# jammm/first_raytracer

Measured on AMD Instinct MI355X. Metric: Mrays/sec + RMSE vs CPU ref, CornellBox 1080p 512spp, 1/2/4/8 MI355X, higher is better.
Workload: dtype f32

## Files before the change

first_raytracer_amd/__init__.py:

```python
import ctypes
import os

import numpy as np

HERE = os.path.dirname(os.path.abspath(__file__))
LIB_PATH = os.environ.get("FRT_LIB_PATH") or os.path.join(HERE, "libfrt.so")

FRT_WORLD_BVH, FRT_WORLD_LIST = 0, 1
FRT_MAT_LAMBERTIAN, FRT_MAT_DIFFUSE_LIGHT = 0, 1
FRT_PRIM_SPHERE = 1 << 30
ABI_VERSION = 9
FRT_MAT_LAMBERTIAN, FRT_MAT_DIFFUSE_LIGHT, FRT_MAT_MODIFIED_PHONG, FRT_MAT_METAL, FRT_MAT_DIELECTRIC = 0, 1, 2, 3, 4
FRT_MAT_ROUGH_CONDUCTOR = 5
FRT_DIST_GGX, FRT_DIST_BECKMANN = 0, 1
FRT_TEX_CONSTANT, FRT_TEX_CHECKER, FRT_TEX_IMAGE = 0, 1, 2
FRT_IMAGE_SRGB8, FRT_IMAGE_F32 = 0, 1
FRT_FLAG_NO_LDS_SCENE = 1
FRT_FLAG_WAVES5 = 2
FRT_FLAG_WAVES6 = 4
FRT_FLAG_WAVES4 = 8
FRT_FLAG_BVH2 = 16
FRT_FLAG_NO_OCT = 256
FRT_FLAG_FP64 = 512
FRT_FLAG_FP32 = 1024
FRT_FLAG_ENV_SAMPLING = 2048
FRT_FLAG_ROULETTE = 4096
FRT_FLAG_SOBOL = 8192
FRT_PRECISION_AUTO, FRT_PRECISION_FP32, FRT_PRECISION_FP64 = 0, 1, 2
FRT_GPU_BVH_PLOC = 0
FRT_GPU_BVH_LBVH = 1
FRT_GPU_BVH_SAH = 2
FRT_INTEGRATOR_PATH, FRT_INTEGRATOR_PSSMLT, FRT_INTEGRATOR_AO, FRT_INTEGRATOR_NORMALS = 0, 1, 2, 3
FRT_INTEGRATOR_ALBEDO, FRT_INTEGRATOR_DEPTH, FRT_INTEGRATOR_DENOISE = 4, 5, 6
FRT_INTEGRATOR_ERROR = 8

ERRORS = {0: "ok", -1: "invalid", -2: "hip", -3: "no scene", -4: "unsupported", -5: "io", -6: "no gfx950 device"}


class FrtError(RuntimeError):
    pass


class Material(ctypes.Structure):
    _fields_ = [("type", ctypes.c_int32), ("distribution", ctypes.c_int32),
                ("albedo", ctypes.c_double * 3), ("emit", ctypes.c_double * 3),
                ("specular", ctypes.c_double * 3), ("exponent", ctypes.c_double), ("ior", ctypes.c_double),
                ("alpha", ctypes.c_double), ("eta", ctypes.c_double * 3), ("k", ctypes.c_double * 3),
                ("texture", ctypes.c_int32), ("image", ctypes.c_int32), ("tex_odd", ctypes.c_double * 3),
                ("tex_scale", ctypes.c_double * 2)]

    @classmethod
    def from_spec(cls, m):
        r = cls()
        r.type = MAT_TYPES[m["type"]]
        r.distribution = DISTRIBUTIONS[m.get("distribution", "ggx").lower()]
        for k in ("albedo", "emit", "specular", "eta", "k"):
            getattr(r, k)[:] = [float(x) for x in m.get(k, (0.0, 0.0, 0.0))]
        r.exponent = float(m.get("exponent", 0.0))
        r.ior = float(m.get("ior", 0.0))
        r.alpha = float(m.get("alpha", 0.0))
        tex = m.get("checker")
        if tex is not None:
            r.texture = FRT_TEX_CHECKER
            r.tex_odd[:] = [float(x) for x in tex["odd"]]
            r.tex_scale[:] = [float(x) for x in tex["scale"]]
        if m.get("image") is not None:
            r.texture = FRT_TEX_IMAGE
            r.image = int(m["image"])
        return r


class Image(ctypes.Structure):
    _fields_ = [("nx", ctypes.c_int32), ("ny", ctypes.c_int32), ("format", ctypes.c_int32),
                ("reserved", ctypes.c_int32), ("data", ctypes.c_void_p)]


def image_array(img):
    a = np.asarray(img["data"])
    if a.ndim != 3 or a.shape[2] != 3:
        raise ValueError("image data must be (ny, nx, 3)")
    if a.dtype == np.uint8:
        return np.ascontiguousarray(a), FRT_IMAGE_SRGB8
    return np.ascontiguousarray(a, np.float32), FRT_IMAGE_F32


CORNELL_CAMERA = {"lookfrom": (0.0, 1.0, float(np.float32(3.9))), "lookat": (0.0, 1.0, 0.0), "vup": (0.0, 1.0, 0.0),
                  "vfov": 40.0, "aperture": 0.0, "focus": 10.0}
MAT_TYPES = {"lambertian": 0, "diffuse_light": 1, "modified_phong": 2, "metal": 3, "dielectric": 4,
             "rough_conductor": 5}
DISTRIBUTIONS = {"ggx": 0, "beckmann": 1}
SPHERE_WHERE = {"world": 1, "lights": 2, "both": 3}


class SceneView(ctypes.Structure):
    _fields_ = [
        ("world_kind", ctypes.c_int32),
        ("n_tris", ctypes.c_int32),
        ("tri_v", ctypes.c_void_p), ("tri_n", ctypes.c_void_p), ("tri_material", ctypes.c_void_p),
        ("tri_geometry_normal", ctypes.c_void_p), ("tri_inv_area", ctypes.c_void_p),
        ("n_spheres", ctypes.c_int32), ("sphere", ctypes.c_void_p), ("sphere_material", ctypes.c_void_p),
        ("n_materials", ctypes.c_int32), ("materials", ctypes.c_void_p),
        ("n_nodes", ctypes.c_int32), ("root", ctypes.c_int32),
        ("node_box", ctypes.c_void_p), ("node_child", ctypes.c_void_p),
        ("n_list", ctypes.c_int32), ("list", ctypes.c_void_p),
        ("n_lights", ctypes.c_int32), ("lights", ctypes.c_void_p),
        ("cam_origin", ctypes.c_double * 3), ("cam_lower_left", ctypes.c_double * 3),
        ("cam_horizontal", ctypes.c_double * 3), ("cam_vertical", ctypes.c_double * 3),
        ("cam_u", ctypes.c_double * 3), ("cam_v", ctypes.c_double * 3),
        ("cam_lens_radius", ctypes.c_double),
        ("env_color", ctypes.c_double * 3),
        ("cam_w", ctypes.c_double * 3),
        ("cam_half_height", ctypes.c_double),
        ("tri_uv", ctypes.c_void_p),
        ("n_images", ctypes.c_int32), ("images", ctypes.c_void_p),
    ]


class RenderParams(ctypes.Structure):
    _fields_ = [(n, ctypes.c_int32) for n in ("nx", "ny", "spp")] + [("seed", ctypes.c_uint32)] + [
        (n, ctypes.c_int32) for n in ("max_depth", "integrator", "tile_size", "shard_index", "shard_count",
                                      "samples_per_item", "flags", "mlt_chains", "mlt_bootstrap", "sample_offset")]

    @classmethod
    def make(cls, nx, ny, spp, seed=0, max_depth=33, tile_size=32, shard_index=0, shard_count=1,
             samples_per_item=0, flags=0, integrator=0, sample_offset=0):
        return cls(nx=nx, ny=ny, spp=spp, seed=seed, max_depth=max_depth, integrator=integrator, tile_size=tile_size,
                   shard_index=shard_index, shard_count=shard_count, samples_per_item=samples_per_item, flags=flags,
                   mlt_chains=0, mlt_bootstrap=0, sample_offset=sample_offset)

    @classmethod
    def pssmlt(cls, nx, ny, mutations_per_pixel, chains, seed=0, bootstrap=10000, shard_index=0, shard_count=1,
               flags=0):
        return cls(nx=nx, ny=ny, spp=mutations_per_pixel, seed=seed, max_depth=10, integrator=FRT_INTEGRATOR_PSSMLT,
                   tile_size=32, shard_index=shard_index, shard_count=shard_count, samples_per_item=0, flags=flags,
                   mlt_chains=chains, mlt_bootstrap=bootstrap)


class Stats(ctypes.Structure):
    _fields_ = [(n, ctypes.c_uint64) for n in ("camera_rays", "extension_rays", "shadow_rays", "samples",
                                               "pixels", "work_items")] + [
        ("kernel_ms", ctypes.c_double), ("total_ms", ctypes.c_double)] + [
        (n, ctypes.c_uint32) for n in ("scene_in_lds", "waves_cap", "stack_entries", "bvh_depth")] + [
        ("scene_bytes", ctypes.c_uint64), ("fp64", ctypes.c_uint32), ("reserved", ctypes.c_uint32)]

    @property
    def rays(self):
        return self.camera_rays + self.extension_rays + self.shadow_rays

    def as_dict(self):
        d = {n: getattr(self, n) for n, _ in self._fields_}
        d["rays"] = self.rays
        return d


class TreeCost(ctypes.Structure):
    _fields_ = [("v", ctypes.c_double), ("t", ctypes.c_double), ("j", ctypes.c_double), ("w", ctypes.c_double),
                ("depth", ctypes.c_int32), ("n_nodes", ctypes.c_int32), ("n_rays", ctypes.c_int32),
                ("applies", ctypes.c_int32)]

    def as_dict(self):
        return {k: getattr(self, k) for k, _ in self._fields_}


class PlanQuery(ctypes.Structure):
    _fields_ = [(n, ctypes.c_int32) for n in ("kind", "integrator", "flags", "world_kind", "stack_needed", "has_bvh4",
                                              "depth4", "mats", "has_spec_mats", "env_image", "env_sampling",
                                              "has_f64", "precision")] + [
        ("scene_lds_bytes", ctypes.c_int64), ("scene_lds_bytes_oct", ctypes.c_int64)]


class PlanAnswer(ctypes.Structure):
    _fields_ = [(n, ctypes.c_int32) for n in ("rc", "stack", "waves", "lds_scene", "wide", "f64")] + [
        (n, ctypes.c_int64) for n in ("lds", "scene_lds", "lds_boot")] + [
        ("kernel", ctypes.c_uint64), ("kernel_boot", ctypes.c_uint64)]


class HostSceneInfo(ctypes.Structure):
    _fields_ = [(n, ctypes.c_int32) for n in ("n_tris", "n_spheres", "n_materials", "n_lights", "n_nodes",
                                              "world_kind", "n_list", "bvh_depth")] + [
        ("load_ms", ctypes.c_double), ("build_ms", ctypes.c_double)]


_lib = None

EXPORTS = ("frt_get_abi_version", "frt_create", "frt_destroy", "frt_last_error", "frt_set_precision", "frt_upload_scene",
           "frt_shard_slot_count", "frt_shard_slots", "frt_render", "frt_render_multi", "frt_render_device", "frt_trace_device",
           "frt_mlt_chain_state",
           "frt_scene_create", "frt_scene_new", "frt_scene_add_obj", "frt_scene_add_sphere", "frt_scene_set_camera",
           "frt_scene_set_env", "frt_scene_add_image", "frt_scene_finish", "frt_scene_build_bvh_gpu",
           "frt_scene_build_bvh_sah", "frt_scene_build_bvh_gpu_algo",
           "frt_scene_view_get", "frt_scene_info", "frt_scene_destroy", "frt_write_tessellated_obj",
           "frt_write_pfm", "frt_film_accumulate", "frt_tonemap_u8", "frt_write_image", "frt_selftest_path_host",
           "frt_selftest_mlt_paths_host",
           "frt_set_env_image", "frt_scene_set_env_image", "frt_scene_env_image", "frt_read_hdr",
           "frt_selftest_path_host_env")
EXPORTS_X = ("frtx_selftest_tree_refine", "frtx_selftest_trace_host", "frtx_selftest_chunk_variance",
             "frtx_selftest_plan")


def lib():
    global _lib
    if _lib is not None:
        return _lib
    if not os.path.exists(LIB_PATH):
        raise FrtError(f"{LIB_PATH} is missing: build it with `python -c 'import __graft_entry__ as g; g.build()'`")
    try:
        import torch
    except ImportError:
        pass
    L = ctypes.CDLL(LIB_PATH)
    vp = ctypes.c_void_p
    L.frt_get_abi_version.restype = ctypes.c_int
    if L.frt_get_abi_version() != ABI_VERSION:
        raise FrtError(f"{LIB_PATH}: ABI version {L.frt_get_abi_version()}, binding expects {ABI_VERSION}; rebuild")
    L.frt_create.argtypes = [ctypes.c_int, ctypes.POINTER(vp)]
    L.frt_destroy.argtypes = [vp]
    L.frt_last_error.argtypes = [vp]
    L.frt_last_error.restype = ctypes.c_char_p
    L.frt_set_precision.argtypes = [vp, ctypes.c_int]
    L.frt_upload_scene.argtypes = [vp, ctypes.POINTER(SceneView)]
    L.frt_shard_slot_count.argtypes = [ctypes.POINTER(RenderParams)]
    L.frt_shard_slot_count.restype = ctypes.c_int64
    L.frt_shard_slots.argtypes = [ctypes.POINTER(RenderParams), vp]
    L.frt_render.argtypes = [vp, ctypes.POINTER(RenderParams), vp, ctypes.POINTER(Stats)]
    L.frt_render_device.argtypes = [vp, ctypes.POINTER(RenderParams), vp, vp, ctypes.POINTER(Stats)]
    L.frt_trace_device.argtypes = [vp, vp, ctypes.c_int64, vp, ctypes.c_int, vp, ctypes.POINTER(Stats)]
    L.frt_mlt_chain_state.argtypes = [vp, ctypes.c_uint64, ctypes.c_uint64, vp, vp]
    L.frt_render_multi.argtypes = [ctypes.POINTER(vp), ctypes.c_int, ctypes.POINTER(RenderParams), vp,
                                   ctypes.POINTER(Stats)]
    L.frt_scene_create.argtypes = [ctypes.c_char_p, ctypes.c_char_p, ctypes.c_double, ctypes.POINTER(vp)]
    L.frt_scene_view_get.argtypes = [vp, ctypes.POINTER(SceneView)]
    L.frt_scene_info.argtypes = [vp, ctypes.POINTER(HostSceneInfo)]
    L.frt_scene_destroy.argtypes = [vp]
    L.frt_scene_destroy.restype = None
    dp = ctypes.POINTER(ctypes.c_double)
    L.frt_scene_new.argtypes = [ctypes.POINTER(vp)]
    L.frt_scene_add_obj.argtypes = [vp, ctypes.c_char_p, dp, ctypes.POINTER(Material), ctypes.c_int]
    L.frt_scene_add_sphere.argtypes = [vp, dp, ctypes.c_double, ctypes.POINTER(Material), ctypes.c_int]
    L.frt_scene_set_camera.argtypes = [vp, dp, dp, dp, ctypes.c_double, ctypes.c_double, ctypes.c_double,
                                       ctypes.c_double]
    L.frt_scene_set_env.argtypes = [vp, dp]
    L.frt_scene_add_image.argtypes = [vp, ctypes.POINTER(Image), ctypes.POINTER(ctypes.c_int)]
    L.frt_scene_finish.argtypes = [vp, ctypes.c_int]
    L.frt_scene_build_bvh_gpu.argtypes = [vp, vp, ctypes.POINTER(ctypes.c_double)]
    L.frt_scene_build_bvh_sah.argtypes = [vp]
    L.frt_scene_build_bvh_gpu_algo.argtypes = [vp, vp, ctypes.c_int, ctypes.POINTER(ctypes.c_double)]
    L.frt_write_tessellated_obj.argtypes = [ctypes.c_char_p, ctypes.c_int, ctypes.c_char_p]
    L.frt_write_pfm.argtypes = [ctypes.c_char_p, ctypes.c_int, ctypes.c_int, vp]
    L.frt_film_accumulate.argtypes = [vp, ctypes.c_int64, vp, ctypes.c_int64, ctypes.c_int64]
    L.frt_tonemap_u8.argtypes = [vp, ctypes.c_int, ctypes.c_int, vp]
    L.frt_write_image.argtypes = [ctypes.c_char_p, ctypes.c_int, ctypes.c_int, vp, ctypes.c_int]
    L.frt_selftest_path_host.argtypes = [ctypes.POINTER(SceneView), ctypes.POINTER(RenderParams), vp,
                                         ctypes.c_int, vp, ctypes.POINTER(Stats)]
    L.frt_selftest_mlt_paths_host.argtypes = [ctypes.POINTER(SceneView), ctypes.c_int, ctypes.c_int, ctypes.c_uint32,
                                              ctypes.c_int, vp]
    L.frt_set_env_image.argtypes = [vp, ctypes.POINTER(Image)]
    L.frt_scene_set_env_image.argtypes = [vp, ctypes.c_int]
    L.frt_scene_env_image.argtypes = [vp, ctypes.POINTER(Image)]
    L.frt_read_hdr.argtypes = [ctypes.c_char_p, ctypes.POINTER(ctypes.c_int32), ctypes.POINTER(ctypes.c_int32), vp]
    L.frt_selftest_path_host_env.argtypes = [ctypes.POINTER(SceneView), ctypes.POINTER(RenderParams), vp,
                                             ctypes.c_int, ctypes.POINTER(Image), vp, ctypes.POINTER(Stats)]
    L.frtx_selftest_tree_refine.argtypes = [ctypes.POINTER(SceneView), ctypes.POINTER(TreeCost), vp, vp, ctypes.c_int32]
    L.frtx_selftest_trace_host.argtypes = [ctypes.POINTER(SceneView), vp, ctypes.c_int64, vp]
    L.frtx_selftest_chunk_variance.argtypes = [vp, ctypes.c_int, ctypes.c_int64, ctypes.c_int, ctypes.c_int, vp]
    _lib = L
    return L


def _check(rc, what, ctx=None):
    if rc != 0:
        msg = ""
        if ctx is not None:
            msg = lib().frt_last_error(ctx).decode(errors="replace")
        raise FrtError(f"{what} failed: {ERRORS.get(rc, rc)} {msg}")


class HostScene:

    def __init__(self, kind, obj_path, aspect):
        self.ptr = ctypes.c_void_p()
        _check(lib().frt_scene_create(kind.encode(), obj_path.encode(), float(aspect), ctypes.byref(self.ptr)),
               f"frt_scene_create({kind})")
        self.info = HostSceneInfo()
        lib().frt_scene_info(self.ptr, ctypes.byref(self.info))
        self.env = None

    def set_env(self, rgb):
        self.env = tuple(float(x) for x in rgb)

    def set_env_image(self, index):
        _check(lib().frt_scene_set_env_image(self.ptr, -1 if index is None else int(index)), "frt_scene_set_env_image")

    def env_image(self):
        img = Image()
        rc = lib().frt_scene_env_image(self.ptr, ctypes.byref(img))
        if rc < 0:
            _check(rc, "frt_scene_env_image")
        return img if rc == 1 else None

    @classmethod
    def from_spec(cls, spec, aspect):
        self = cls.__new__(cls)
        self.ptr = ctypes.c_void_p()
        self.env = None
        L = lib()
        _check(L.frt_scene_new(ctypes.byref(self.ptr)), "frt_scene_new")

        def dptr(x):
            a = np.ascontiguousarray(np.asarray(x, np.float64))
            return a, a.ctypes.data_as(ctypes.POINTER(ctypes.c_double))
        for img in spec.get("images", ()):
            a, fmt = image_array(img)
            desc = Image(a.shape[1], a.shape[0], fmt, 0, a.ctypes.data)
            idx = ctypes.c_int(-1)
            _check(L.frt_scene_add_image(self.ptr, ctypes.byref(desc), ctypes.byref(idx)), "frt_scene_add_image")
        for o in spec["objects"]:
            if "obj" in o:
                tw = dptr(o["to_world"]) if o.get("to_world") is not None else (None, None)
                bs = ctypes.byref(Material.from_spec(o["bsdf"])) if o.get("bsdf") is not None else None
                _check(L.frt_scene_add_obj(self.ptr, o["obj"].encode(), tw[1], bs, int(bool(o.get("geo", False)))),
                       f"frt_scene_add_obj({o['obj']})")
            else:
                c = dptr(o["sphere"])
                _check(L.frt_scene_add_sphere(self.ptr, c[1], float(o["radius"]),
                                              ctypes.byref(Material.from_spec(o["material"])),
                                              SPHERE_WHERE[o.get("where", "world")]), "frt_scene_add_sphere")
        cam = spec["camera"]
        f, a, u = dptr(cam["lookfrom"]), dptr(cam["lookat"]), dptr(cam.get("vup", (0, 1, 0)))
        _check(L.frt_scene_set_camera(self.ptr, f[1], a[1], u[1], float(cam["vfov"]), float(aspect),
                                      float(cam.get("aperture", 0.0)), float(cam.get("focus", 10.0))),
               "frt_scene_set_camera")
        if spec.get("env") is not None:
            e = dptr(spec["env"])
            _check(L.frt_scene_set_env(self.ptr, e[1]), "frt_scene_set_env")
        if spec.get("env_image") is not None:
            _check(L.frt_scene_set_env_image(self.ptr, int(spec["env_image"])), "frt_scene_set_env_image")
        _check(L.frt_scene_finish(self.ptr, {"bvh": 0, "list": 1}[spec.get("world", "bvh")]), "frt_scene_finish")
        self.info = HostSceneInfo()
        L.frt_scene_info(self.ptr, ctypes.byref(self.info))
        return self

    def view(self):
        v = SceneView()
        _check(lib().frt_scene_view_get(self.ptr, ctypes.byref(v)), "frt_scene_view_get")
        if self.env is not None:
            v.env_color[:] = self.env
        return v

    def arrays(self):
        v = self.view()

        def arr(ptr, n, dt, w=1):
            if n == 0 or not ptr:
                return np.zeros((0, w) if w > 1 else 0, dt)
            a = np.ctypeslib.as_array(ctypes.cast(ptr, ctypes.POINTER(np.ctypeslib.as_ctypes_type(dt))),
                                      shape=(n * w,)).copy()
            return a.reshape(n, w) if w > 1 else a
        return {
            "tri_v": arr(v.tri_v, v.n_tris, np.float64, 9),
            "tri_material": arr(v.tri_material, v.n_tris, np.int32),
            "node_box": arr(v.node_box, v.n_nodes, np.float64, 6),
            "node_child": arr(v.node_child, v.n_nodes, np.int32, 2),
            "root": v.root,
            "lights": arr(v.lights, v.n_lights, np.int32),
            "list": arr(v.list, v.n_list, np.int32),
        }

    def build_bvh_sah(self):
        _check(lib().frt_scene_build_bvh_sah(self.ptr), "frt_scene_build_bvh_sah")
        lib().frt_scene_info(self.ptr, ctypes.byref(self.info))
        return self.info.build_ms

    def build_bvh_gpu(self, ctx, algo="gsah"):
        ms = ctypes.c_double()
        a = {"ploc": FRT_GPU_BVH_PLOC, "lbvh": FRT_GPU_BVH_LBVH, "gsah": FRT_GPU_BVH_SAH}[algo]
        _check(lib().frt_scene_build_bvh_gpu_algo(self.ptr, ctx.ptr, a, ctypes.byref(ms)),
               "frt_scene_build_bvh_gpu_algo", ctx.ptr)
        lib().frt_scene_info(self.ptr, ctypes.byref(self.info))
        return ms.value

    def __del__(self):
        if getattr(self, "ptr", None):
            try:
                lib().frt_scene_destroy(self.ptr)
            except Exception:
                pass
            self.ptr = None


class Context:

    def __init__(self, device=0, precision=None):
        self.ptr = ctypes.c_void_p()
        _check(lib().frt_create(int(device), ctypes.byref(self.ptr)), f"frt_create(device={device})")
        if precision is not None:
            self.set_precision(precision)

    def set_precision(self, precision):
        if isinstance(precision, str):
            precision = {"auto": FRT_PRECISION_AUTO, "fp32": FRT_PRECISION_FP32, "fp64": FRT_PRECISION_FP64}[precision]
        _check(lib().frt_set_precision(self.ptr, int(precision)), "frt_set_precision", self.ptr)

    def upload(self, scene):
        view = scene.view() if isinstance(scene, HostScene) else scene
        _check(lib().frt_upload_scene(self.ptr, ctypes.byref(view)), "frt_upload_scene", self.ptr)
        img = scene.env_image() if isinstance(scene, HostScene) else None
        if img is not None:
            _check(lib().frt_set_env_image(self.ptr, ctypes.byref(img)), "frt_set_env_image", self.ptr)
            self._env_from_scene = True
        elif isinstance(scene, HostScene) and getattr(self, "_env_from_scene", False):
            _check(lib().frt_set_env_image(self.ptr, None), "frt_set_env_image", self.ptr)
            self._env_from_scene = False

    def set_env_image(self, image):
        self._env_from_scene = False
# ... 39 lines not shown
        u = np.zeros((max(n, 1), 92), np.float32)
        fp = np.zeros((max(n, 1), 2), np.uint32)
        _check(lib().frt_mlt_chain_state(self.ptr, int(first), int(n), u.ctypes.data, fp.ctypes.data),
               "frt_mlt_chain_state", self.ptr)
        return u[:n], fp[:n]

    def trace_device(self, rays_ptr, n, hits_ptr, flags=0, stream_ptr=None):
        st = Stats()
        _check(lib().frt_trace_device(self.ptr, ctypes.c_void_p(rays_ptr), int(n), ctypes.c_void_p(hits_ptr), int(flags),
                                      ctypes.c_void_p(stream_ptr) if stream_ptr else None, ctypes.byref(st)),
               "frt_trace_device", self.ptr)
        return st

    def close(self):
        if getattr(self, "ptr", None):
            lib().frt_destroy(self.ptr)
            self.ptr = None

    def __del__(self):
        try:
            self.close()
        except Exception:
            pass


def render_multi(contexts, params, film=None):
    if film is None:
        film = np.zeros((params.ny, params.nx, 3), np.float32)
    assert film.dtype == np.float32 and film.flags.c_contiguous and film.size == params.nx * params.ny * 3
    arr = (ctypes.c_void_p * len(contexts))(*[c.ptr for c in contexts])
    st = Stats()
    _check(lib().frt_render_multi(arr, len(contexts), ctypes.byref(params), film.ctypes.data, ctypes.byref(st)),
           "frt_render_multi", contexts[0].ptr)
    return film, st


def frame_error(film, V):
    f = np.asarray(film, np.float64)
    v = np.asarray(V, np.float64)
    return float(np.sqrt(v.sum() / v.size) / (f.sum() / f.size))


def combine_variance(a, Va, b, Vb):
    a, b = float(a), float(b)
    va, vb = np.asarray(Va, np.float64), np.asarray(Vb, np.float64)
    return (((a * a) * va + (b * b) * vb) / ((a + b) * (a + b))).astype(np.float32)


def replicate_variance(films):
    assert len(films) == 4
    r = [np.asarray(f, np.float64) for f in films]
    m = (((r[0] + r[1]) + r[2]) + r[3]) * 0.25
    v = ((((r[0] - m) ** 2 + (r[1] - m) ** 2) + (r[2] - m) ** 2) + (r[3] - m) ** 2) / 12.0
    mean = np.array(films[0], np.float32, copy=True)
    for k in range(1, 4):
        mean = film_accumulate(mean, k, films[k], 1)
    return mean, v.astype(np.float32)


def render_until(render, render_error, params, target, max_spp, first_spp=16):
    first_spp, max_spp = int(first_spp), int(max_spp)
    if first_spp < 2 or first_spp & (first_spp - 1):
        raise FrtError("render_until: first_spp must be a power of two >= 2")
    if params.integrator not in (FRT_INTEGRATOR_PATH, FRT_INTEGRATOR_AO):
        raise FrtError("render_until: path and ao renders only (pssmlt has no error estimate, denoise is a filter)")
    if not target > 0:
        raise FrtError("render_until: target must be > 0")
    sobol = bool(params.flags & FRT_FLAG_SOBOL) and params.integrator == FRT_INTEGRATOR_PATH
    reps = 4 if sobol else 1
    if max_spp < reps * first_spp:
        raise FrtError("render_until: max_spp is below the first pass")
    slots = lib().frt_shard_slot_count(ctypes.byref(params))
    if slots < 0:
        raise FrtError("bad render params")
    films, V, total, passes = [None] * reps, None, 0, []
    halve = False
    while True:
        n = first_spp if total == 0 else total
        ms = 0.0
        for k in range(reps):
            p = RenderParams.from_buffer_copy(params)
            p.spp, p.sample_offset, p.seed = n, total, (params.seed + k) & 0xffffffff
            if halve:
                p.samples_per_item = n // 2
            film, st = render(p)
            if not sobol and st.work_items == slots:
                halve = True
                p.samples_per_item = n // 2
                film, st = render(p)
            ms += st.kernel_ms
            if not sobol:
                Vp = render_error(p)
                V = Vp if total == 0 else combine_variance(total, V, n, Vp)
            films[k] = film if total == 0 else film_accumulate(films[k], total, film, n)
        total += n
        if sobol:
            film, V = replicate_variance(films)
        else:
            film = films[0]
        e = frame_error(film, V)
        passes.append((reps * total, e, ms))
        if e <= target:
            return film, V, reps * total, e, True, passes
        if reps * 2 * total > max_spp:
            return film, V, reps * total, e, False, passes


def selftest_chunk_variance(partial, spp, spi):
    partial = np.ascontiguousarray(partial, dtype=np.float32)
    k, n, three = partial.shape
    assert three == 3
    out = np.zeros((n, 3), np.float32)
    _check(lib().frtx_selftest_chunk_variance(partial.ctypes.data, k, n, int(spp), int(spi), out.ctypes.data),
           "frtx_selftest_chunk_variance")
    return out


def shard_slots(params):
    n = lib().frt_shard_slot_count(ctypes.byref(params))
    if n < 0:
        raise FrtError("bad render params")
    out = np.zeros(n, np.int32)
    _check(lib().frt_shard_slots(ctypes.byref(params), out.ctypes.data), "frt_shard_slots")
    return out


def selftest_path_host(scene, params, pixels, env_image=None):
    pixels = np.ascontiguousarray(pixels, dtype=np.int32)
    out = np.zeros((len(pixels), 3), np.float32)
    st = Stats()
    view = scene.view()
    if env_image is None:
        _check(lib().frt_selftest_path_host(ctypes.byref(view), ctypes.byref(params), pixels.ctypes.data, len(pixels),
                                            out.ctypes.data, ctypes.byref(st)), "frt_selftest_path_host")
        return out, st
    a, fmt = image_array({"data": env_image})
    desc = Image(a.shape[1], a.shape[0], fmt, 0, a.ctypes.data)
    _check(lib().frt_selftest_path_host_env(ctypes.byref(view), ctypes.byref(params), pixels.ctypes.data, len(pixels),
                                            ctypes.byref(desc), out.ctypes.data, ctypes.byref(st)),
           "frt_selftest_path_host_env")
    return out, st


def selftest_tree_refine(scene):
    view = scene.view()
    cap = max(1, view.n_tris + view.n_spheres)
    nodes = [np.zeros((cap, 16), np.float32) for _ in range(2)]
    out = (TreeCost * 2)()
    _check(lib().frtx_selftest_tree_refine(ctypes.byref(view), out, nodes[0].ctypes.data, nodes[1].ctypes.data, cap),
           "frtx_selftest_tree_refine")
    return tuple((out[k].as_dict(), nodes[k][:out[k].n_nodes].copy()) for k in range(2))


def selftest_trace_host(scene, rays):
    rays = np.ascontiguousarray(rays, dtype=np.float32).reshape(-1, 8)
    hits = np.zeros((len(rays), 4), np.float32)
    view = scene.view()
    _check(lib().frtx_selftest_trace_host(ctypes.byref(view), rays.ctypes.data, len(rays), hits.ctypes.data),
           "frtx_selftest_trace_host")
    return hits


_handles = None


def kernel_handles():
    global _handles
    if _handles is None:
        import re
        import subprocess
        out = subprocess.run(["nm", "--defined-only", LIB_PATH], capture_output=True, text=True, check=True).stdout
        syms = [l.split() for l in out.splitlines()]
        stub = re.compile(r"(\d+)__device_stub__")
        kernels = {stub.sub(lambda m: str(int(m.group(1)) - 15), f[2]) for f in syms if len(f) == 3 and stub.search(f[2])}
        _handles = {int(f[0], 16): f[2] for f in syms if len(f) == 3 and f[2] in kernels}
    return _handles


def selftest_plan(**query):
    f = lib().frtx_selftest_plan
    f.argtypes = [ctypes.POINTER(PlanQuery), ctypes.POINTER(PlanAnswer)]
    a = PlanAnswer()
    _check(f(ctypes.byref(PlanQuery(**query)), ctypes.byref(a)), "frtx_selftest_plan")
    d = {n: getattr(a, n) for n, _ in a._fields_}
    for k in ("kernel", "kernel_boot"):
        d[k] = kernel_handles().get(d[k]) if d[k] else None
    return d


def selftest_mlt_paths_host(scene, nx, ny, seed, n):
    out = np.zeros((n, 6), np.float32)
    view = scene.view()
    _check(lib().frt_selftest_mlt_paths_host(ctypes.byref(view), nx, ny, seed, n, out.ctypes.data),
           "frt_selftest_mlt_paths_host")
    return out


def read_hdr(path):
    nx, ny = ctypes.c_int32(0), ctypes.c_int32(0)
    _check(lib().frt_read_hdr(os.fsencode(path), ctypes.byref(nx), ctypes.byref(ny), None), f"frt_read_hdr({path})")
    out = np.zeros((ny.value, nx.value, 3), np.float32)
    _check(lib().frt_read_hdr(os.fsencode(path), ctypes.byref(nx), ctypes.byref(ny), out.ctypes.data),
           f"frt_read_hdr({path})")
    return out


def write_pfm(path, film):
    film = np.ascontiguousarray(film, dtype=np.float32)
    ny, nx = film.shape[0], film.shape[1]
    _check(lib().frt_write_pfm(path.encode(), nx, ny, film.ctypes.data), "frt_write_pfm")


def film_accumulate(acc, acc_spp, film, spp):
    acc = np.ascontiguousarray(acc, dtype=np.float32)
    film = np.ascontiguousarray(film, dtype=np.float32)
    _check(lib().frt_film_accumulate(acc.ctypes.data, int(acc_spp), film.ctypes.data, int(spp), film.size),
           "frt_film_accumulate")
    return acc


def tonemap_u8(film):
    film = np.ascontiguousarray(film, dtype=np.float32)
    ny, nx = film.shape[0], film.shape[1]
    out = np.zeros((ny, nx, 3), np.uint8)
    _check(lib().frt_tonemap_u8(film.ctypes.data, nx, ny, out.ctypes.data), "frt_tonemap_u8")
    return out


IMAGE_FORMATS = {"png": 0, "bmp": 1, "jpg": 2}


def write_image(path, rgb_u8, fmt="png"):
    rgb_u8 = np.ascontiguousarray(rgb_u8, dtype=np.uint8)
    ny, nx = rgb_u8.shape[0], rgb_u8.shape[1]
    _check(lib().frt_write_image(path.encode(), nx, ny, rgb_u8.ctypes.data, IMAGE_FORMATS[fmt]), "frt_write_image")


def work_granule(integrator, spp, n_slots, lanes, spi_req=0):
    L = lib()
    f = L.frt_internal_work_granule
    f.argtypes = [ctypes.c_int, ctypes.c_int, ctypes.c_int64, ctypes.c_int64, ctypes.c_int,
                  ctypes.POINTER(ctypes.c_int), ctypes.POINTER(ctypes.c_int)]
    spi, k = ctypes.c_int(0), ctypes.c_int(0)
    _check(f(integrator, spp, n_slots, lanes, spi_req, ctypes.byref(spi), ctypes.byref(k)), "work_granule")
    return spi.value, k.value


def write_tessellated_obj(src_obj, k, dst_obj):
    _check(lib().frt_write_tessellated_obj(src_obj.encode(), int(k), dst_obj.encode()), "frt_write_tessellated_obj")
```

first_raytracer_amd/csrc/frt_flatten.hip:

```cpp
#include "frt_flatten.hpp"

#include <algorithm>
#include <cfloat>
#include <cmath>
#include <cstdlib>
#include <functional>

#include "frt_kernels.hpp"
#include "host/tree_refine.hpp"

using namespace frt;

static inline float round_down(double x)
{
    float f = (float)x;
    if ((double)f > x) f = std::nextafter(f, -INFINITY);
    return f;
}
static inline float round_up(double x)
{
    float f = (float)x;
    if ((double)f < x) f = std::nextafter(f, INFINITY);
    return f;
}

static int leaf_size_override()
{
    const char *e = std::getenv("FRT_LEAF_SIZE");
    return e ? std::min(std::max(std::atoi(e), 1), kLeafMax) : 0;
}

static void collapse_leaves(FlatScene &F, int leaf_max)
{
    const int nn = (int)(F.nodes.size() / 4);
    if (leaf_max <= 1 || nn == 0) return;
    auto child = [&](int i, int side) { return f2i(side ? F.nodes[4 * i + 3].y : F.nodes[4 * i + 3].x); };
    std::vector<int> cnt(nn, 0), first(nn, INT32_MAX);
    std::vector<char> sph(nn, 0);
    for (int i = nn - 1; i >= 0; --i)
        for (int side = 0; side < 2; ++side) {
            const int c = child(i, side);
            if (c >= 0) {
                cnt[i] += cnt[c]; first[i] = std::min(first[i], first[c]); sph[i] |= sph[c];
            } else if (~c & FRT_PRIM_SPHERE) {
                sph[i] = 1;
            } else {
                cnt[i] += 1; first[i] = std::min(first[i], ~c);
            }
        }
    std::vector<float4> out;
    out.reserve(F.nodes.size());
    int depth = 0;
    struct Item { int old, parent_slot, side, lvl; };
    std::vector<Item> st{{0, -1, 0, 1}};
    while (!st.empty()) {
        const Item it = st.back();
        st.pop_back();
        const int me = (int)(out.size() / 4);
        if (it.parent_slot >= 0) {
            float4 &r = out[it.parent_slot];
            (it.side ? r.y : r.x) = i2f(me);
        }
        depth = std::max(depth, it.lvl);
        for (int k = 0; k < 4; ++k) out.push_back(F.nodes[4 * it.old + k]);
        const int slot = 4 * me + 3;
        for (int side = 1; side >= 0; --side) {
            const int c = child(it.old, side);
            if (c < 0) continue;
            if (!sph[c] && cnt[c] <= leaf_max) {
                float4 &r = out[slot];
                (side ? r.y : r.x) = i2f(~(first[c] | ((cnt[c] - 1) << kLeafCountShift)));
            } else {
                st.push_back({c, slot, side, it.lvl + 1});
            }
        }
    }
    F.nodes.swap(out);
    F.depth = depth;
}

static bool build_bvh4(FlatScene &F, int root_ref)
{
    F.nodes4.clear();
    F.depth4 = 0;
    F.root4 = root_ref;
    const int nn = (int)(F.nodes.size() / 4);
    if (nn == 0 || root_ref < 0) return true;
    struct Child { float lo[3], hi[3]; int ref; };
    auto kids = [&](int i, Child *out) {
        const float4 a = F.nodes[4 * i], b = F.nodes[4 * i + 1], c = F.nodes[4 * i + 2], r = F.nodes[4 * i + 3];
        out[0] = Child{{a.x, a.y, a.z}, {a.w, b.x, b.y}, f2i(r.x)};
        out[1] = Child{{b.z, b.w, c.x}, {c.y, c.z, c.w}, f2i(r.y)};
    };
    auto area = [](const Child &c) {
        const double dx = (double)c.hi[0] - c.lo[0], dy = (double)c.hi[1] - c.lo[1], dz = (double)c.hi[2] - c.lo[2];
        return dx * dy + dy * dz + dz * dx;
    };
    const uint32_t empty_ref = (uint32_t)~(F.tris.empty() ? FRT_PRIM_SPHERE : 0);
    std::vector<double> T(nn, 0.0), D(5 * (size_t)nn, 0.0);
    std::vector<signed char> split(5 * (size_t)nn, 1);
    auto slot_cost = [&](const Child &c, int k) {
        if (c.ref < 0) return 0.0;
        return k >= 2 ? std::min(T[c.ref], D[5 * (size_t)c.ref + k]) : T[c.ref];
    };
    {
        std::vector<double> own(nn, 0.0);
        for (int i = 0; i < nn; ++i) {
            Child two[2];
            kids(i, two);
            for (int s = 0; s < 2; ++s) if (two[s].ref >= 0) own[two[s].ref] = area(two[s]);
        }
        for (int i = nn - 1; i >= 0; --i) {
            Child two[2];
            kids(i, two);
            for (int j = 2; j <= 4; ++j) {
                double best = 1e300;
                for (int k = 1; k < j; ++k) {
                    const double v = slot_cost(two[0], k) + slot_cost(two[1], j - k);
                    if (v < best) { best = v; split[5 * (size_t)i + j] = (signed char)k; }
                }
                D[5 * (size_t)i + j] = best;
            }
            T[i] = own[i] + D[5 * (size_t)i + 4];
        }
    }
    std::function<void(const Child &, int, Child *, int &)> gather = [&](const Child &c, int k, Child *out, int &n) {
        if (c.ref < 0 || k < 2 || !(D[5 * (size_t)c.ref + k] < T[c.ref])) { out[n++] = c; return; }
        Child two[2];
        kids(c.ref, two);
        const int kl = split[5 * (size_t)c.ref + k];
        gather(two[0], kl, out, n);
        gather(two[1], k - kl, out, n);
    };
    struct Item { int bin, parent, slot, lvl; };
    std::vector<Item> st{{root_ref, -1, 0, 1}};
    while (!st.empty()) {
        const Item it = st.back();
        st.pop_back();
        const int me = (int)(F.nodes4.size() / kNode4Parts);
        if (it.parent >= 0) {
            uint4 &r = F.nodes4[(size_t)kNode4Parts * it.parent + 1];
            (it.slot == 0 ? r.x : it.slot == 1 ? r.y : it.slot == 2 ? r.z : r.w) = (uint32_t)me;
        }
        F.depth4 = std::max(F.depth4, it.lvl);
        Child ch[4], two[2];
        int n = 0;
        kids(it.bin, two);
        const int kl = split[5 * (size_t)it.bin + 4];
        gather(two[0], kl, ch, n);
        gather(two[1], 4 - kl, ch, n);
        float org[3];
        int ex[3];
        uint32_t qlo[3] = {0, 0, 0}, qhi[3] = {0, 0, 0};
        for (int a = 0; a < 3; ++a) {
            float lo = ch[0].lo[a], hi = ch[0].hi[a];
            for (int k = 1; k < n; ++k) { lo = std::min(lo, ch[k].lo[a]); hi = std::max(hi, ch[k].hi[a]); }
            org[a] = lo;
            const double ext = (double)hi - (double)lo;
            int e = -126;
            if (ext > 0.0) {
                std::frexp(ext / 255.0, &e);
                e = std::max(e, -126);
                while (e > -126 && std::ldexp(255.0, e - 1) >= ext) --e;
            }
            if (e > 20) return false;
            if (e < -100) return false;
            ex[a] = e;
            for (int s = 0; s < 4; ++s) {
                double ql = 255.0, qh = 0.0;
                if (s < n) {
                    const Child &c = ch[s];
                    ql = std::floor(((double)c.lo[a] - lo) / std::ldexp(1.0, e));
                    qh = std::ceil(((double)c.hi[a] - lo) / std::ldexp(1.0, e));
                    ql = std::min(std::max(ql, 0.0), 255.0);
                    qh = std::min(std::max(qh, 0.0), 255.0);
                    while (ql > 0.0 && (double)lo + ql * std::ldexp(1.0, e) > (double)c.lo[a]) ql -= 1.0;
                    while (qh < 255.0 && (double)lo + qh * std::ldexp(1.0, e) < (double)c.hi[a]) qh += 1.0;
                }
                qlo[a] |= (uint32_t)ql << (8 * s);
                qhi[a] |= (uint32_t)qh << (8 * s);
            }
        }
        uint32_t refs[4];
        for (int s = 0; s < 4; ++s) refs[s] = s < n ? (uint32_t)ch[s].ref : empty_ref;
        F.nodes4.resize((size_t)(me + 1) * kNode4Parts);
        uint4 *out = F.nodes4.data() + (size_t)me * kNode4Parts;
        out[0] = make_uint4((uint32_t)f2i(org[0]), (uint32_t)f2i(org[1]), (uint32_t)f2i(org[2]),
                            ((uint32_t)ex[0] & 0xffu) | (((uint32_t)ex[1] & 0xffu) << 8) | (((uint32_t)ex[2] & 0xffu) << 16));
        out[1] = make_uint4(refs[0], refs[1], refs[2], refs[3]);
        out[2] = make_uint4(qlo[0], qhi[0], qlo[1], qhi[1]);
        out[3] = make_uint4(qlo[2], qhi[2], 0u, 0u);
        for (int s = n - 1; s >= 0; --s)
            if (ch[s].ref >= 0) st.push_back({ch[s].ref, me, s, it.lvl + 1});
    }
    F.root4 = 0;
    return true;
}

static void append_texels(const frt_image &im, std::vector<float4> &out)
{
    const size_t n = (size_t)im.nx * im.ny;
    auto srgb = [](double v) { return v <= 0.04045 ? v * (1.0 / 12.92) : std::pow((v + 0.055) * (1.0 / 1.055), 2.4); };
    for (size_t q = 0; q < n; ++q) {
        double c[3];
        for (int ch = 0; ch < 3; ++ch)
            c[ch] = im.format == FRT_IMAGE_F32 ? (double)static_cast<const float *>(im.data)[3 * q + ch]
                                               : srgb(static_cast<const uint8_t *>(im.data)[3 * q + ch] / 255.0);
        out.push_back(make_float4((float)c[0], (float)c[1], (float)c[2], 0.0f));
    }
}
int env_texels_of(const frt_image *img, std::vector<float4> &out, std::string &err)
{
    if (img->nx <= 0 || img->ny <= 0) { err = "environment image: nx and ny must be positive"; return FRT_E_INVALID; }
    if (!img->data) { err = "environment image: null data"; return FRT_E_INVALID; }
    if (img->format != FRT_IMAGE_SRGB8 && img->format != FRT_IMAGE_F32) {
        err = "environment image: format must be FRT_IMAGE_SRGB8 or FRT_IMAGE_F32";
        return FRT_E_INVALID;
    }
    if ((size_t)img->nx * img->ny > (size_t)INT32_MAX) { err = "environment image larger than 2^31 texels"; return FRT_E_UNSUPPORTED; }
    out.clear();
    out.reserve((size_t)img->nx * img->ny);
    append_texels(*img, out);
    for (size_t q = 0; q < out.size(); ++q) {
        const float v[3] = {out[q].x, out[q].y, out[q].z};
        for (int ch = 0; ch < 3; ++ch)
            if (!(v[ch] >= 0.0f && v[ch] <= FLT_MAX)) {
                err = "environment image: texel (" + std::to_string(q % img->nx) + ", " + std::to_string(q / img->nx) +
                      ") is negative or not finite";
                return FRT_E_INVALID;
            }
    }
    return FRT_OK;
}

static void fill_octants(FlatScene &F)
{
    for (int o = 0; o < 8 && !F.nodes_oct.empty(); ++o)
        for (size_t i = 0; i < F.nodes.size() / 4; ++i) {
            const float4 *n = &F.nodes[4 * i];
            const float b0[6] = {n[0].x, n[0].y, n[0].z, n[0].w, n[1].x, n[1].y};
            const float b1[6] = {n[1].z, n[1].w, n[2].x, n[2].y, n[2].z, n[2].w};
            float q[12];
            for (int a = 0; a < 3; ++a) {
                const bool neg = (o >> a) & 1;
                q[a] = neg ? b0[3 + a] : b0[a];
                q[3 + a] = neg ? b0[a] : b0[3 + a];
                q[6 + a] = neg ? b1[3 + a] : b1[a];
                q[9 + a] = neg ? b1[a] : b1[3 + a];
            }
            float4 *d = &F.nodes_oct[(size_t)o * F.nodes.size() + 4 * i];
            d[0] = make_float4(q[0], q[1], q[2], q[3]);
            d[1] = make_float4(q[4], q[5], q[6], q[7]);
            d[2] = make_float4(q[8], q[9], q[10], q[11]);
            d[3] = n[3];
        }
}

constexpr double kRefineW = 1.8;
constexpr int kRefineFitFrame = 24, kRefineValFrame = 40;
constexpr uint32_t kRefineFitSeed = 0x7ee5eed1u, kRefineValSeed = 0x7ee5eed2u;
constexpr int kRefineMaxDepth = 33;
constexpr int kRefineMaxEvals = 700;

static bool tree_refine_knob()
{
    const char *e = std::getenv("FRT_TREE_REFINE");
    return !(e && std::atoi(e) == 0);
}

static bool tree_in_lds(const FlatScene &F)
{
    if (F.meta.world_kind != FRT_WORLD_BVH || F.meta.root < 0 || F.depth >= kLdsMaxDepth) return false;
    const size_t bytes = sizeof(float4) * (F.nodes.size() + F.tris.size() + F.tshade.size() + F.mats.size());
    return bytes <= kLdsSceneBytes || !F.nodes_oct.empty();
}

struct RefineLeaf { float box[6]; int ref; };

static void topology_of(const std::vector<float4> &nodes, frt_refine::Topology &t, std::vector<RefineLeaf> &leaves)
{
    const int nn = (int)(nodes.size() / 4);
    leaves.clear();
    t.child.assign(2 * (size_t)nn, 0);
    t.n_leaves = nn + 1;
    t.root = t.n_leaves;
    for (int i = 0; i < nn; ++i) {
        const float4 *n = &nodes[4 * i];
        const float b[2][6] = {{n[0].x, n[0].y, n[0].z, n[0].w, n[1].x, n[1].y}, {n[1].z, n[1].w, n[2].x, n[2].y, n[2].z, n[2].w}};
        for (int side = 0; side < 2; ++side) {
            const int c = f2i(side ? n[3].y : n[3].x);
            if (c >= 0) { t.child[2 * i + side] = t.n_leaves + c; continue; }
            RefineLeaf l;
            for (int k = 0; k < 6; ++k) l.box[k] = b[side][k];
            l.ref = c;
            t.child[2 * i + side] = (int)leaves.size();
            leaves.push_back(l);
        }
    }
}

static void sample_rays(const FlatScene &F, const std::vector<RefineLeaf> &leaves, int frame, uint32_t seed,
                        frt_refine::RaySet &R)
{
    const DevScene S = host_scene(F);
    struct Ray { f3 o, d; float tmax; bool shadow; };
    std::vector<Ray> rays;
    std::vector<int> stack(std::max(F.depth + 1, 1));
    for (int pix = 0; pix < frame * frame; ++pix) {
        PathState<float> P;
        path_begin<kMatsAll>(P, S, pix % frame, pix / frame, frame, frame, seed, (uint32_t)pix, 0u);
        for (;;) {
            rays.push_back(Ray{P.ro, P.rd, P.rtmax, P.shadow});
            const Hit<float> h = trace<FRT_WORLD_BVH, 1>(S, P.ro, P.rd, P.rtmax, P.shadow, stack.data());
            uint32_t n_ext = 0, n_sh = 0;
            if (path_shade<kMatsAll>(P, S, h, kRefineMaxDepth, n_ext, n_sh)) break;
        }
    }
    const int n = (int)rays.size(), nl = (int)leaves.size();
    R = frt_refine::RaySet{};
    R.n = n;
    R.n_leaves = nl;
    R.prim_first.assign(nl + 1, 0);
    for (int l = 0; l < nl; ++l) {
        const int lref = ~leaves[l].ref;
        const bool sph = (lref & FRT_PRIM_SPHERE) != 0;
        const int first = sph ? lref : (lref & kLeafIndexMask), count = sph ? 1 : (lref >> kLeafCountShift) + 1;
        for (int k = 0; k < count; ++k) R.prim_ref.push_back(first + k);
        R.prim_first[l + 1] = (int)R.prim_ref.size();
    }
    R.n_prims = (int)R.prim_ref.size();
    R.tmin.resize(n); R.tmax.resize(n); R.anyhit.resize(n); R.live.resize(n);
    R.slab.resize((size_t)nl * n * 6);
    R.prim_t.resize((size_t)n * R.n_prims);
    int stride = (int)(0.618 * n) | 1;
    auto gcd = [](int a, int b) { while (b) { const int c = a % b; a = b; b = c; } return a; };
    while (n > 1 && gcd(stride, n) != 1) stride += 2;
    for (int i = 0; i < n; ++i) {
        const Ray &q = rays[(int)(((int64_t)i * stride) % std::max(n, 1))];
        Trav<float> T;
        R.live[i] = trav_begin(T, S, S.root, q.o, q.d, q.tmax) ? 1 : 0;
        R.tmin[i] = T.tmin;
        R.tmax[i] = q.tmax;
        R.anyhit[i] = q.shadow ? 1 : 0;
        const float inv[3] = {T.sr.invd.x, T.sr.invd.y, T.sr.invd.z}, oi[3] = {T.sr.oinv.x, T.sr.oinv.y, T.sr.oinv.z};
        for (int l = 0; l < nl; ++l) {
            float *s = &R.slab[((size_t)i * nl + l) * 6];
            for (int a = 0; a < 3; ++a) {
                const bool neg = inv[a] < 0.0f;
                s[a] = vfma(leaves[l].box[neg ? 3 + a : a], inv[a], oi[a]);
                s[3 + a] = -vfma(leaves[l].box[neg ? a : 3 + a], inv[a], oi[a]);
            }
        }
        for (int k = 0; k < R.n_prims; ++k) {
            float u, v;
            R.prim_t[(size_t)i * R.n_prims + k] = prim_t(S, R.prim_ref[k], q.o, q.d, T.tmin, q.tmax, u, v);
        }
    }
}

static void write_topology(FlatScene &F, const frt_refine::Topology &t, const std::vector<RefineLeaf> &leaves)
{
    const int L = t.n_leaves, nn = L - 1;
    std::vector<float> box(6 * (size_t)(L + nn));
    std::function<void(int)> bound = [&](int s) {
        float *b = &box[6 * (size_t)s];
        if (s < L) { for (int k = 0; k < 6; ++k) b[k] = leaves[s].box[k]; return; }
        const int c0 = t.child[2 * (s - L)], c1 = t.child[2 * (s - L) + 1];
        bound(c0);
        bound(c1);
        for (int k = 0; k < 3; ++k) {
            b[k] = std::min(box[6 * (size_t)c0 + k], box[6 * (size_t)c1 + k]);
            b[3 + k] = std::max(box[6 * (size_t)c0 + 3 + k], box[6 * (size_t)c1 + 3 + k]);
        }
    };
    bound(t.root);
    std::vector<float4> out(4 * (size_t)nn);
    int next = 0;
    std::function<int(int)> emit = [&](int s) {
        if (s < L) return leaves[s].ref;
        const int me = next++;
        const int c[2] = {t.child[2 * (s - L)], t.child[2 * (s - L) + 1]};
        const float *a = &box[6 * (size_t)c[0]], *b = &box[6 * (size_t)c[1]];
        out[4 * me + 0] = make_float4(a[0], a[1], a[2], a[3]);
        out[4 * me + 1] = make_float4(a[4], a[5], b[0], b[1]);
        out[4 * me + 2] = make_float4(b[2], b[3], b[4], b[5]);
        const int r0 = emit(c[0]), r1 = emit(c[1]);
        out[4 * me + 3] = make_float4(i2f(r0), i2f(r1), 0.0f, 0.0f);
        return me;
    };
    emit(t.root);
    F.nodes.swap(out);
}

bool tree_cost_host(const FlatScene &F, TreeCost &out)
{
    out = TreeCost{};
    out.w = kRefineW;
    if (!tree_in_lds(F) || F.nodes.empty()) return false;
    frt_refine::Topology t;
    std::vector<RefineLeaf> leaves;
    topology_of(F.nodes, t, leaves);
    frt_refine::RaySet val;
    sample_rays(F, leaves, kRefineValFrame, kRefineValSeed, val);
    const frt_refine::Cost c = frt_refine::tree_cost(t, val);
    out.V = c.V; out.T = c.T; out.J = frt_refine::cost_j(c, kRefineW);
    out.depth = t.depth();
    out.n_rays = val.n;
    return true;
}

static bool refine_tree(FlatScene &F)
{
    if (!tree_in_lds(F) || F.nodes.size() / 4 < 3) return false;
    frt_refine::Topology t;
    std::vector<RefineLeaf> leaves;
    topology_of(F.nodes, t, leaves);
    const frt_refine::Topology input = t;
    frt_refine::RaySet fit;
    sample_rays(F, leaves, kRefineFitFrame, kRefineFitSeed, fit);
    if (frt_refine::refine(t, fit, kRefineW, input.depth(), kRefineMaxEvals) == 0) return false;
    frt_refine::RaySet val;
    sample_rays(F, leaves, kRefineValFrame, kRefineValSeed, val);
    const double j0 = frt_refine::cost_j(frt_refine::tree_cost(input, val), kRefineW);
    const double j1 = frt_refine::cost_j(frt_refine::tree_cost(t, val), kRefineW);
    if (!(j1 < j0)) return false;
    write_topology(F, t, leaves);
    return true;
}

int flatten_scene(const frt_scene_view *sv, FlatScene &F, std::string &err, bool f64, int refine)
{
    auto fail = [&](int code, const std::string &m) { err = m; return code; };
    const int nt = sv->n_tris, ns = sv->n_spheres, nm = sv->n_materials;
    if (nt < 0 || ns < 0 || nm <= 0 || !sv->materials || (nt > 0 && (!sv->tri_v || !sv->tri_material || !sv->tri_inv_area)))
        return fail(FRT_E_INVALID, "scene view: missing triangle arrays or materials");
    if (ns > 0 && (!sv->sphere || !sv->sphere_material)) return fail(FRT_E_INVALID, "scene view: missing sphere arrays");
    for (int i = 0; i < nm; ++i) {
        const int t = sv->materials[i].type;
        if (t != FRT_MAT_LAMBERTIAN && t != FRT_MAT_DIFFUSE_LIGHT && t != FRT_MAT_MODIFIED_PHONG &&
            t != FRT_MAT_METAL && t != FRT_MAT_DIELECTRIC && t != FRT_MAT_ROUGH_CONDUCTOR)
            return fail(FRT_E_UNSUPPORTED, "material type " + std::to_string(t) + " is not supported");
        const int tex = sv->materials[i].texture;
        if (tex != FRT_TEX_CONSTANT && tex != FRT_TEX_CHECKER && tex != FRT_TEX_IMAGE)
            return fail(FRT_E_INVALID, "material texture must be FRT_TEX_CONSTANT, FRT_TEX_CHECKER or FRT_TEX_IMAGE");
        if (tex != FRT_TEX_CONSTANT && (t == FRT_MAT_DIFFUSE_LIGHT || t == FRT_MAT_METAL))
            return fail(FRT_E_UNSUPPORTED, "checker / image textures apply to lambertian / modified_phong / dielectric / "
                                           "rough_conductor colours");
        if (tex == FRT_TEX_IMAGE) {
            const int k = sv->materials[i].image;
            if (k < 0 || k >= sv->n_images || !sv->images)
                return fail(FRT_E_INVALID, "material image index out of range");
            const frt_image &im = sv->images[k];
            if (im.nx <= 0 || im.ny <= 0 || !im.data || (im.format != FRT_IMAGE_SRGB8 && im.format != FRT_IMAGE_F32))
                return fail(FRT_E_INVALID, "scene view: bad image");
        }
        if (t == FRT_MAT_ROUGH_CONDUCTOR &&
            (!(sv->materials[i].alpha > 0.0) || (sv->materials[i].distribution != FRT_DIST_GGX &&
                                                  sv->materials[i].distribution != FRT_DIST_BECKMANN)))
            return fail(FRT_E_INVALID, "rough_conductor needs alpha > 0 and a GGX / Beckmann distribution");
    }
    auto valid_ref = [&](int ref) {
        if (ref < 0) return false;
        if (ref & FRT_PRIM_SPHERE) return (ref & ~FRT_PRIM_SPHERE) < ns;
        return ref < nt;
    };
    auto prim_box = [&](int ref, double *lo, double *hi) {
        if (ref & FRT_PRIM_SPHERE) {
            const double *q = &sv->sphere[4 * (ref & ~FRT_PRIM_SPHERE)];
            for (int k = 0; k < 3; ++k) { lo[k] = q[k] - q[3]; hi[k] = q[k] + q[3]; }
        } else {
            const double *v = &sv->tri_v[9 * ref];
            for (int k = 0; k < 3; ++k) {
                lo[k] = std::min(std::min(v[k], v[3 + k]), v[6 + k]);
                hi[k] = std::max(std::max(v[k], v[3 + k]), v[6 + k]);
            }
        }
    };
    std::vector<int> tri_order;
    std::vector<int> tri_dev(nt, -1);
    DevScene &S = F.meta;
    S = DevScene{};
    if (sv->world_kind == FRT_WORLD_BVH) {
        const int nn = sv->n_nodes;
        if (nn < 0 || (nn > 0 && (!sv->node_box || !sv->node_child)))
            return fail(FRT_E_INVALID, "scene view: missing BVH arrays");
        if (sv->root >= nn || (sv->root >= 0 && nn == 0)) return fail(FRT_E_INVALID, "scene view: bad root");
        double rlo[3], rhi[3];
        if (sv->root < 0) {
            if (!valid_ref(~sv->root)) return fail(FRT_E_INVALID, "scene view: bad root prim");
            prim_box(~sv->root, rlo, rhi);
        } else {
            for (int k = 0; k < 3; ++k) { rlo[k] = sv->node_box[6 * sv->root + k]; rhi[k] = sv->node_box[6 * sv->root + 3 + k]; }
        }
        double scale = 1.0;
        for (int k = 0; k < 3; ++k) scale = std::max(scale, std::max(std::fabs(rlo[k]), std::fabs(rhi[k])));
        const double pad = 4e-6 * scale;
        auto padded = [&](const double *lo, const double *hi, float *flo, float *fhi) {
            for (int k = 0; k < 3; ++k) { flo[k] = round_down(lo[k] - pad); fhi[k] = round_up(hi[k] + pad); }
        };
        padded(rlo, rhi, S.root_lo, S.root_hi);
        S.ao_tmax = (float)((rhi[1] - rlo[1]) * 0.50f);
        std::vector<int> new_id(std::max(nn, 1), -1), order;
        order.reserve(nn);
        std::vector<std::pair<int, int>> st;
        st.push_back({sv->root, 1});
        while (!st.empty()) {
            const auto [x, lvl] = st.back();
            st.pop_back();
            if (x >= 0) {
                if (x >= nn || new_id[x] >= 0) return fail(FRT_E_INVALID, "scene view: BVH is not a tree");
                new_id[x] = (int)order.size();
                order.push_back(x);
                F.depth = std::max(F.depth, lvl);
                st.push_back({sv->node_child[2 * x + 1], lvl + 1});
                st.push_back({sv->node_child[2 * x], lvl + 1});
            } else {
                const int ref = ~x;
                if (!valid_ref(ref)) return fail(FRT_E_INVALID, "scene view: bad leaf prim");
                if (!(ref & FRT_PRIM_SPHERE)) {
                    if (tri_dev[ref] >= 0) return fail(FRT_E_INVALID, "scene view: triangle in two leaves");
                    tri_dev[ref] = (int)tri_order.size();
                    tri_order.push_back(ref);
                }
            }
        }
        F.nodes.resize(4 * order.size());
        for (size_t i = 0; i < order.size(); ++i) {
            const int x = order[i];
            float cb[2][6];
            int cref[2];
            for (int side = 0; side < 2; ++side) {
                const int ch = sv->node_child[2 * x + side];
                double lo[3], hi[3];
                if (ch >= 0) {
                    for (int k = 0; k < 3; ++k) { lo[k] = sv->node_box[6 * ch + k]; hi[k] = sv->node_box[6 * ch + 3 + k]; }
                    cref[side] = new_id[ch];
                } else {
                    const int ref = ~ch;
                    prim_box(ref, lo, hi);
                    cref[side] = ~((ref & FRT_PRIM_SPHERE) ? ref : tri_dev[ref]);
                }
                padded(lo, hi, &cb[side][0], &cb[side][3]);
            }
            F.nodes[4 * i + 0] = make_float4(cb[0][0], cb[0][1], cb[0][2], cb[0][3]);
            F.nodes[4 * i + 1] = make_float4(cb[0][4], cb[0][5], cb[1][0], cb[1][1]);
            F.nodes[4 * i + 2] = make_float4(cb[1][2], cb[1][3], cb[1][4], cb[1][5]);
            F.nodes[4 * i + 3] = make_float4(i2f(cref[0]), i2f(cref[1]), 0.0f, 0.0f);
        }
        if (nt >= kLeafIndexLimit) return fail(FRT_E_INVALID, "scene view: too many triangles");
        const int forced = leaf_size_override();
        if (forced) {
            collapse_leaves(F, forced);
        } else {
            const std::vector<float4> binary = F.nodes;
            const int depth = F.depth;
            collapse_leaves(F, kLeafSmallScene);
            const size_t bytes = sizeof(float4) * (F.nodes.size() + 5 * (size_t)nt + 2 * (size_t)nm);
            if (bytes > kLdsSceneBytes || F.depth >= kLdsMaxDepth) {
                F.nodes = binary;
                F.depth = depth;
                collapse_leaves(F, kLeafDefault);
            }
        }
        for (int i = 0; i < nt; ++i)
            if (tri_dev[i] < 0) { tri_dev[i] = (int)tri_order.size(); tri_order.push_back(i); }
    } else if (sv->world_kind == FRT_WORLD_LIST) {
        S.ao_spheres_only = 1;
        if (sv->n_list < 0 || (sv->n_list > 0 && !sv->list)) return fail(FRT_E_INVALID, "scene view: bad list");
        for (int i = 0; i < nt; ++i) { tri_dev[i] = i; tri_order.push_back(i); }
        for (int i = 0; i < sv->n_list; ++i)
            if (!valid_ref(sv->list[i])) return fail(FRT_E_INVALID, "scene view: bad list entry");
    } else {
        return fail(FRT_E_INVALID, "scene view: unknown world kind");
    }
    auto dev_ref = [&](int ref) { return (ref & FRT_PRIM_SPHERE) ? ref : tri_dev[ref]; };
    F.tri_view = tri_order;

    bool any_smooth = false;
    for (int i = 0; i < nt; ++i)
        if (sv->tri_geometry_normal && !sv->tri_geometry_normal[i]) any_smooth = true;
    if (any_smooth && !sv->tri_n) return fail(FRT_E_INVALID, "scene view: smooth triangles without normals");
    F.tris.resize(3 * (size_t)nt);
    F.tshade.resize(2 * (size_t)nt);
    if (any_smooth) F.tnorm.resize(3 * (size_t)nt);
    if (f64) {
        F.tris64.resize(3 * (size_t)nt);
        F.tshade64.resize(nt);
        if (any_smooth) F.tnorm64.resize(3 * (size_t)nt);
    }
    for (int d = 0; d < nt; ++d) {
        const int i = tri_order[d];
        const double *v = &sv->tri_v[9 * i];
        const double e1[3] = {v[3] - v[0], v[4] - v[1], v[5] - v[2]};
        const double e2[3] = {v[6] - v[0], v[7] - v[1], v[8] - v[2]};
        double ng[3] = {e1[1] * e2[2] - e1[2] * e2[1], e1[2] * e2[0] - e1[0] * e2[2], e1[0] * e2[1] - e1[1] * e2[0]};
        const double l = std::sqrt(ng[0] * ng[0] + ng[1] * ng[1] + ng[2] * ng[2]);
        for (int k = 0; k < 3; ++k) ng[k] = ng[k] / l;
        F.tris[3 * d + 0] = make_float4((float)v[0], (float)v[1], (float)v[2], 0.0f);
        F.tris[3 * d + 1] = make_float4((float)e1[0], (float)e1[1], (float)e1[2], 0.0f);
        F.tris[3 * d + 2] = make_float4((float)e2[0], (float)e2[1], (float)e2[2], 0.0f);
        const int mat = sv->tri_material[i];
        if (mat < 0 || mat >= nm) return fail(FRT_E_INVALID, "scene view: bad triangle material");
        const int geo = sv->tri_geometry_normal ? (sv->tri_geometry_normal[i] ? 1 : 0) : 1;
        F.tshade[2 * d + 0] = make_float4((float)ng[0], (float)ng[1], (float)ng[2], (float)sv->tri_inv_area[i]);
        F.tshade[2 * d + 1] = make_float4(i2f(mat), i2f(geo), 0.0f, 0.0f);
        if (any_smooth)
            for (int k = 0; k < 3; ++k)
                F.tnorm[3 * d + k] = make_float4((float)sv->tri_n[9 * i + 3 * k], (float)sv->tri_n[9 * i + 3 * k + 1],
                                                 (float)sv->tri_n[9 * i + 3 * k + 2], 0.0f);
        if (f64) {
            F.tris64[3 * d + 0] = make_double4(v[0], v[1], v[2], 0.0);
            F.tris64[3 * d + 1] = make_double4(e1[0], e1[1], e1[2], 0.0);
            F.tris64[3 * d + 2] = make_double4(e2[0], e2[1], e2[2], 0.0);
            F.tshade64[d] = make_double4(ng[0], ng[1], ng[2], sv->tri_inv_area[i]);
            if (any_smooth)
                for (int k = 0; k < 3; ++k)
                    F.tnorm64[3 * d + k] = make_double4(sv->tri_n[9 * i + 3 * k], sv->tri_n[9 * i + 3 * k + 1],
                                                        sv->tri_n[9 * i + 3 * k + 2], 0.0);
        }
    }
    bool any_tex = false;
    for (int i = 0; i < nm; ++i) any_tex |= sv->materials[i].texture != FRT_TEX_CONSTANT;
    if (any_tex) {
        F.tuv.assign(2 * (size_t)std::max(nt, 1), make_float4(0.0f, 0.0f, 0.0f, 0.0f));
        if (sv->tri_uv)
            for (int d = 0; d < nt; ++d) {
                const double *q = &sv->tri_uv[6 * tri_order[d]];
                F.tuv[2 * d] = make_float4((float)q[0], (float)q[1], (float)q[2], (float)q[3]);
                F.tuv[2 * d + 1] = make_float4((float)q[4], (float)q[5], 0.0f, 0.0f);
            }
    }
    F.spheres.resize(ns);
    F.smat.resize(ns);
    if (f64) F.spheres64.resize(ns);
    for (int k = 0; k < ns; ++k) {
        const double *q = &sv->sphere[4 * k];
        F.spheres[k] = make_float4((float)q[0], (float)q[1], (float)q[2], (float)q[3]);
        if (f64) F.spheres64[k] = make_double4(q[0], q[1], q[2], q[3]);
        F.smat[k] = sv->sphere_material[k];
        if (F.smat[k] < 0 || F.smat[k] >= nm) return fail(FRT_E_INVALID, "scene view: bad sphere material");
    }
    std::vector<int> image_off(std::max(sv->n_images, 0), -1);
    for (int i = 0; i < nm; ++i) {
        if (sv->materials[i].texture != FRT_TEX_IMAGE) continue;
        const int k = sv->materials[i].image;
        if (image_off[k] >= 0) continue;
        const frt_image &im = sv->images[k];
        const size_t n = (size_t)im.nx * im.ny;
        if (F.texels.size() + n > (size_t)INT32_MAX) return fail(FRT_E_UNSUPPORTED, "images larger than 2^31 texels");
        image_off[k] = (int)F.texels.size();
        append_texels(im, F.texels);
    }
    F.mats.assign(kMatStride * (size_t)nm, make_float4(0.0f, 0.0f, 0.0f, 0.0f));
    for (int i = 0; i < nm; ++i) {
        const frt_material &m = sv->materials[i];
        float4 *d = &F.mats[kMatStride * i];
        auto f4 = [](const double *v, float w) { return make_float4((float)v[0], (float)v[1], (float)v[2], w); };
        d[0] = f4(m.type == FRT_MAT_ROUGH_CONDUCTOR ? m.eta : m.albedo, i2f(m.type));
        if (m.type == FRT_MAT_DIFFUSE_LIGHT) d[1] = f4(m.emit, 0.0f);
        else d[1] = f4(m.specular, (float)(m.type == FRT_MAT_MODIFIED_PHONG ? m.exponent
                                           : m.type == FRT_MAT_DIELECTRIC ? m.ior : m.alpha));
        d[2] = f4(m.k, i2f(m.distribution));
        d[3] = f4(m.tex_odd, i2f(m.texture));
        d[4] = make_float4((float)m.tex_scale[0], (float)m.tex_scale[1], 0.0f, 0.0f);
        if (m.texture == FRT_TEX_IMAGE)
            d[4] = make_float4(i2f(sv->images[m.image].nx), i2f(sv->images[m.image].ny), i2f(image_off[m.image]), 0.0f);
    }
    if (sv->n_lights < 0 || (sv->n_lights > 0 && !sv->lights)) return fail(FRT_E_INVALID, "scene view: bad lights");
    F.lights.resize(sv->n_lights);
    for (int i = 0; i < sv->n_lights; ++i) {
        if (!valid_ref(sv->lights[i])) return fail(FRT_E_INVALID, "scene view: bad light");
        F.lights[i] = dev_ref(sv->lights[i]);
    }
    F.list.resize(sv->world_kind == FRT_WORLD_LIST ? sv->n_list : 0);
    for (size_t i = 0; i < F.list.size(); ++i) F.list[i] = dev_ref(sv->list[i]);

    const size_t oct_bytes = sizeof(float4) * (oct_lds_node_slots((int)(F.nodes.size() / 4)) + F.tris.size() +
                                               F.tshade.size() + F.mats.size());
    if (sv->world_kind == FRT_WORLD_BVH && F.depth < kLdsMaxDepth && oct_bytes <= kLdsOctBytes)
        F.nodes_oct.resize(8 * F.nodes.size());
    S.root = (sv->world_kind == FRT_WORLD_BVH) ? ((sv->root >= 0) ? 0 : ~dev_ref(~sv->root)) : 0;
    auto derive_trees = [&]() {
        fill_octants(F);
        F.has4 = sv->world_kind == FRT_WORLD_BVH && build_bvh4(F, S.root);
        if (!F.has4) F.nodes4.clear();
        S.root4 = F.has4 ? F.root4 : S.root;
        S.n_nodes4 = (int)(F.nodes4.size() / kNode4Parts);
    };
    derive_trees();
    S.n_lights = sv->n_lights;
    S.n_list = (int)F.list.size();
    S.n_nodes = (int)(F.nodes.size() / 4);
    S.n_tris = nt;
    S.n_mats = nm;
    S.n_nodes4 = (int)(F.nodes4.size() / kNode4Parts);
    S.node_es = 4; S.node_ps = 1;
    S.node4_es = kNode4Parts; S.node4_ps = 1;
    S.tri_es = 3; S.tri_ps = 1;
    S.sh_es = 2; S.sh_ps = 1;
    S.world_kind = sv->world_kind;
    auto f3d = [](const double *x) { return mk3((float)x[0], (float)x[1], (float)x[2]); };
    S.cam_o = f3d(sv->cam_origin); S.cam_llc = f3d(sv->cam_lower_left);
    S.cam_h = f3d(sv->cam_horizontal); S.cam_v = f3d(sv->cam_vertical);
    S.cam_u = f3d(sv->cam_u); S.cam_vv = f3d(sv->cam_v);
    S.lens_r = (float)sv->cam_lens_radius;
    S.cam_w = f3d(sv->cam_w);
    S.cam_half_height = (float)sv->cam_half_height;
    S.env = f3d(sv->env_color);
    auto d3d = [](const double *x) { return d3{x[0], x[1], x[2]}; };
    S.cam64_o = d3d(sv->cam_origin); S.cam64_llc = d3d(sv->cam_lower_left);
    S.cam64_h = d3d(sv->cam_horizontal); S.cam64_v = d3d(sv->cam_vertical);
    S.cam64_u = d3d(sv->cam_u); S.cam64_vv = d3d(sv->cam_v);
    S.lens_r64 = sv->cam_lens_radius;
    if ((refine < 0 ? tree_refine_knob() : refine != 0) && refine_tree(F)) derive_trees();
    return FRT_OK;
}

DevScene host_scene(const FlatScene &F)
{
    DevScene S = F.meta;
    S.nodes = F.nodes.data(); S.nodes4 = F.nodes4.data(); S.nodes_oct = F.nodes_oct.data();
    S.tris = F.tris.data(); S.tshade = F.tshade.data(); S.tnorm = F.tnorm.data();
    S.tuv = F.tuv.data(); S.texels = F.texels.data();
    S.spheres = F.spheres.data(); S.sphere_mat = F.smat.data(); S.mats = F.mats.data();
    S.lights = F.lights.data(); S.list = F.list.data(); S.tri_view = F.tri_view.data();
    S.tris64 = F.tris64.data(); S.tshade64 = F.tshade64.data(); S.tnorm64 = F.tnorm64.data();
    S.spheres64 = F.spheres64.data();
    return S;
}
```

first_raytracer_amd/csrc/frt_flatten.hpp:

```cpp
#pragma once
#include <string>
#include <vector>

#include "frt.h"
#include "frt_device.hpp"
#include "frt_path.hpp"

using frt::DevScene;

#pragma GCC visibility push(hidden)
struct FlatScene {
    std::vector<float4> nodes, tris, tshade, tnorm, spheres, mats, tuv;
    std::vector<float4> texels;
    std::vector<uint4> nodes4;
    std::vector<float4> nodes_oct;
    std::vector<double4> tris64, tshade64, tnorm64, spheres64;
    bool has4 = false;
    int root4 = 0, depth4 = 0;
    std::vector<int> smat, lights, list;
    std::vector<int> tri_view;
    DevScene meta{};
    int depth = 0;
};

int flatten_scene(const frt_scene_view *sv, FlatScene &F, std::string &err, bool f64, int refine = -1);
struct TreeCost { double V = 0.0, T = 0.0, J = 0.0, w = 0.0; int depth = 0, n_rays = 0; };
bool tree_cost_host(const FlatScene &F, TreeCost &out);
int env_texels_of(const frt_image *img, std::vector<float4> &out, std::string &err);
frt::DevScene host_scene(const FlatScene &F);
#pragma GCC visibility pop
```

first_raytracer_amd/csrc/frt_kernels.hpp:

```cpp
#pragma once
#include <hip/hip_runtime.h>

#include <stdint.h>

#include "frt.h"
#include "frt_device.hpp"
#include "frt_path.hpp"
#include "frt_mlt.hpp"

using namespace frt;

namespace {

constexpr int kBlock = 256;
constexpr size_t kLdsSceneBytes = 16 * 1024;
constexpr size_t kLdsOctBytes = 14 * 1024;
constexpr int kLdsMaxDepth = 16;
__host__ __device__ constexpr int oct_lds_node_slots(int n_nodes) { return 24 * n_nodes + (n_nodes + 1) / 2; }
#ifndef FRT_QUEUE_GRAB
#define FRT_QUEUE_GRAB 64
#endif
constexpr int kQueueGrab = FRT_QUEUE_GRAB;

struct DevWork {
// ... 76 lines not shown
constexpr int kItemWords = 10;
enum { kIsCur, kIsEnd, kIsSlot, kIsChunk, kIsPix, kIsPx, kIsPy, kIsAcc };
struct ItemState {
    int *b;
    __device__ int get(int k) const { return b[k * kBlock]; }
    __device__ void set(int k, int x) const { b[k * kBlock] = x; }
};

template <int STACK, int WORLD, bool LDS_SCENE, int WAVES = 1, int MATS = kMatsNone,
          int KIND = FRT_INTEGRATOR_PATH, typename R = float>
__global__ __launch_bounds__(kBlock) __attribute__((amdgpu_waves_per_eu(WAVES))) void path_megakernel(
    const DevScene S0, const DevWork W)
{
    extern __shared__ __attribute__((aligned(16))) int lds_mem[];
    int *stk = lds_mem + threadIdx.x;
    constexpr int kStackInts = WORLD != FRT_WORLD_LIST ? STACK * kBlock : 0;
    constexpr int kItemInts = kItemWords * kBlock;
    DevScene S = S0;
    if constexpr (LDS_SCENE) scene_to_lds<WORLD>(S, lds_mem + kStackInts + kItemInts);
    else scene_strides_hbm(S);
    const int lane = threadIdx.x & 63;
    const int T2 = W.tile * W.tile;

    bool have_item = false, exhausted = false, active = false;
    uint32_t q_cur = 0, q_end = 0;
    const ItemState I{lds_mem + kStackInts + (int)threadIdx.x};
    PathState<R> P;
    Trav<R> T;
    bool tracing = false, pending = false;
    int ovf[kOverflow<WORLD>];
    unsigned long long n_cam = 0, n_ext = 0, n_sh = 0, n_smp = 0;
    constexpr bool kLean = !LDS_SCENE && (MATS & ~kMatsFeatures) == kMatsNone && KIND == FRT_INTEGRATOR_PATH && !kIsF64<R>;
    auto flush_L = [&]() {
        I.set(kIsAcc + 0, f2i(i2f(I.get(kIsAcc + 0)) + (float)P.L.x));
        I.set(kIsAcc + 1, f2i(i2f(I.get(kIsAcc + 1)) + (float)P.L.y));
        I.set(kIsAcc + 2, f2i(i2f(I.get(kIsAcc + 2)) + (float)P.L.z));
        P.L = zero3<R>();
    };
    auto ray_tmax = [&]() -> R {
        if constexpr (kLean) return P.shadow ? R(1) - Cst<R>::shadow_eps : Cst<R>::tmax;
        else return P.rtmax;
    };

    unsigned long long diag_t0 = FRT_DIAG_CLOCK();
    for (;;) {
        FRT_DIAG_TICK(6);
        for (;;) {
            bool shadow_done = false;
            if (tracing) FRT_DIAG_TICK(3);
            if (tracing && trav_step_world<WORLD, kBlock, STACK, kPathStep<KIND>>(T, S, P.ro, P.rd, P.shadow, stk, ovf,
                                                                       LDS_SCENE && (WORLD == FRT_WORLD_BVH || WORLD == kWorldBvh2Oct)
                                                                           ? 0 : W.min_desc)) {
                if (KIND == FRT_INTEGRATOR_PATH && P.shadow) {
                    if (path_after_shadow<MATS>(P, T.h.prim < 0)) {
                        if constexpr (kLean) flush_L();
                        shadow_done = true;
                        tracing = trav_begin_world<WORLD>(T, S, P.ro, P.rd, ray_tmax());
                        pending = !tracing;
                    } else {
                        tracing = false;
                        pending = true;
                    }
                } else {
                    tracing = false;
                    pending = true;
                }
            }
            n_ext += __popcll(__ballot(shadow_done));
            if (__popcll(__ballot(tracing)) <= W.trav_min) break;
        }
        const unsigned long long diag_t1 = FRT_DIAG_CLOCK();
        FRT_DIAG_CYC(16, diag_t1 - diag_t0);
        uint32_t ne = 0, ns = 0;
        bool next_ray = false;
        if (pending) {
            FRT_DIAG_TICK(4);
            pending = false;
            if constexpr (kLean)
                P.key = smp_key<MATS>(W.seed, (uint32_t)I.get(kIsPix), (uint32_t)(I.get(kIsCur) - 1) + W.s_off);
            const bool done = shade_kind<KIND, MATS>(P, S, T.h, W.max_depth, ne, ns);
            if (done || kLean) flush_L();
            active = !done;
            next_ray = !done;
        }
        n_ext += __popcll(__ballot(ne != 0));
        n_sh += __popcll(__ballot(ns != 0));
        const unsigned long long diag_t2 = FRT_DIAG_CLOCK();
        FRT_DIAG_CYC(17, diag_t2 - diag_t1);
        if (!active && have_item && I.get(kIsCur) >= I.get(kIsEnd)) {
            float *dst = W.partial + 3ull * ((size_t)(uint32_t)I.get(kIsChunk) * W.n_slots + (uint32_t)I.get(kIsSlot));
            dst[0] = i2f(I.get(kIsAcc + 0)); dst[1] = i2f(I.get(kIsAcc + 1)); dst[2] = i2f(I.get(kIsAcc + 2));
            have_item = false;
        }
        const bool need = !active && !have_item && !exhausted;
        const uint64_t m = __ballot(need);
        if (m) {
            const uint32_t nm = (uint32_t)__popcll(m), r = lane_rank(m);
            const uint32_t left = q_end - q_cur;
            uint32_t w;
            if (nm <= left) {
                w = q_cur + r;
                q_cur += nm;
            } else {
                const uint32_t take = max(W.grab, nm - left);
                const int leader = __ffsll((unsigned long long)m) - 1;
                uint32_t base = 0;
                if (lane == leader) base = atomicAdd(W.counter, take);
                base = __shfl(base, leader);
                w = r < left ? q_cur + r : base + (r - left);
                q_cur = base + (nm - left);
                q_end = base + take;
            }
            if (need) {
                if (w >= W.n_items) {
                    exhausted = true;
                } else {
                    const uint32_t s = w % (uint32_t)T2;
                    const uint32_t q = w / (uint32_t)T2;
                    const uint32_t chunk = q % (uint32_t)W.n_chunks;
                    const uint32_t t_ord = q / (uint32_t)W.n_chunks;
                    const int tile_id = W.shard_index + (int)t_ord * W.shard_count;
                    int lx, ly;
                    slot_to_local((int)s, W.tile, lx, ly);
                    const int px = (tile_id % W.ntx) * W.tile + lx;
                    const int py = (tile_id / W.ntx) * W.tile + ly;
                    if (px < W.nx && py < W.ny) {
                        have_item = true;
                        const int s_cur = (int)chunk * W.spi;
                        I.set(kIsCur, s_cur);
                        I.set(kIsSlot, (int)(t_ord * (uint32_t)T2 + s));
                        I.set(kIsChunk, (int)chunk);
                        I.set(kIsPix, py * W.nx + px);
                        I.set(kIsEnd, min(W.spp, s_cur + W.spi));
                        I.set(kIsPx, px);
                        I.set(kIsPy, py);
                        I.set(kIsAcc + 0, 0); I.set(kIsAcc + 1, 0); I.set(kIsAcc + 2, 0);
                    }
                }
            }
        }
        const bool start = !active && have_item && I.get(kIsCur) < I.get(kIsEnd);
        if (start) {
            const int s_cur = I.get(kIsCur);
            path_begin<MATS>(P, S, I.get(kIsPx), I.get(kIsPy), W.nx, W.ny, W.seed, (uint32_t)I.get(kIsPix),
                       (uint32_t)s_cur + W.s_off);
            I.set(kIsCur, s_cur + 1);
            active = true;
            next_ray = true;
        }
        const unsigned long long started = __popcll(__ballot(start));
        n_cam += started;
        n_smp += started;
        if (next_ray) {
            tracing = trav_begin_world<WORLD>(T, S, P.ro, P.rd, ray_tmax());
            pending = !tracing;
        }
        diag_t0 = FRT_DIAG_CLOCK();
        FRT_DIAG_CYC(18, diag_t0 - diag_t2);
        if (__ballot(active || !exhausted) == 0) break;
    }
    const unsigned long long c[4] = {n_cam, n_ext, n_sh, n_smp};
    if (lane == 0) {
        const size_t wv = ((size_t)blockIdx.x * kBlock + threadIdx.x) >> 6;
        for (int k = 0; k < 4; ++k) W.wave_rays[4 * wv + k] = c[k];
    }
}


constexpr uint32_t kTraceChunk = 256;
constexpr size_t kCounterBytes = 256;
constexpr int kTraceCounterWord = 32;
struct DevRays {
    const float4 *ray;
    float4 *hit;
    uint32_t n;
    int min_desc;
    unsigned *counter;
};
template <int STACK, int WORLD, bool LDS_SCENE, int WAVES>
__global__ __launch_bounds__(kBlock) __attribute__((amdgpu_waves_per_eu(WAVES))) void trace_kernel(
    const DevScene S0, const DevRays R)
{
    extern __shared__ __attribute__((aligned(16))) int lds_mem[];
    int *stk = lds_mem + threadIdx.x;
    constexpr int kStackInts = WORLD != FRT_WORLD_LIST ? STACK * kBlock : 0;
    DevScene S = S0;
    if constexpr (LDS_SCENE) scene_to_lds<WORLD>(S, lds_mem + kStackInts);
    else scene_strides_hbm(S);
    const int lane = threadIdx.x & 63;
    Trav<float> T;
    int ovf[kOverflow<WORLD>];
    f3 o = mk3(0, 0, 0), d = mk3(0, 0, 1);
    bool anyhit = false, tracing = false, exhausted = false;
    uint32_t id = 0;
    auto finish = [&]() {
        const int p = T.h.prim;
        const int ref = (p < 0 || (p & FRT_PRIM_SPHERE)) ? p : S.tri_view[p];
        R.hit[id] = make_float4(T.h.t, T.h.u, T.h.v, i2f(ref));
    };
    uint32_t chunk_next = 0, chunk_end = 0;
    float4 na = make_float4(0, 0, 0, 0), nb = make_float4(0, 0, 0, 0);
    uint32_t nid = 0;
    bool have_next = false;
    for (;;) {
        if (!tracing && have_next) {
            id = nid;
            o = xyz(na);
            d = xyz(nb);
            anyhit = (f2i(nb.w) & 1) != 0;
            have_next = false;
            tracing = trav_begin_world<WORLD>(T, S, o, d, na.w);
            if (!tracing) finish();
        }
        const bool need = !have_next && !exhausted;
        const uint64_t m = __ballot(need);
        if (m) {
            const uint32_t want = (uint32_t)__popcll(m), left = chunk_end - chunk_next;
            uint32_t fresh = 0xffffffffu;
            if (left < want && chunk_end < R.n) {
                uint32_t b0 = 0;
                if (lane == 0) b0 = atomicAdd(R.counter, kTraceChunk);
                fresh = __builtin_amdgcn_readfirstlane(__shfl(b0, 0));
            }
            const uint32_t rank = lane_rank(m);
            const uint32_t w = rank < left ? chunk_next + rank : (fresh == 0xffffffffu ? 0xffffffffu : fresh + (rank - left));
            if (left >= want) {
                chunk_next += want;
            } else if (fresh != 0xffffffffu) {
                chunk_next = fresh + (want - left);
                chunk_end = fresh + kTraceChunk;
            } else {
                chunk_next = chunk_end;
            }
            if (need) {
                if (w >= R.n) {
                    exhausted = true;
                } else {
                    nid = w;
                    na = R.ray[2 * (size_t)w];
                    nb = R.ray[2 * (size_t)w + 1];
                    have_next = true;
                }
            }
        }
        if (__ballot(tracing || have_next) == 0) break;
        if (tracing && trav_step_world<WORLD, kBlock, STACK>(T, S, o, d, anyhit, stk, ovf,
                                                             LDS_SCENE && (WORLD == FRT_WORLD_BVH || WORLD == kWorldBvh2Oct) ? 0 : R.min_desc)) {
            tracing = false;
            finish();
        }
    }
}

constexpr int kChainWords = 9;
enum { kCsT, kCsC, kCsX, kCsY, kCsSc, kCsW, kCsCc };
struct MltWork {
    int nx, ny;
    uint32_t seed;
    int shard_index, shard_count;
    uint32_t n_local;
    uint64_t steps;
    float b, scale, s2p, logp;
    int trav_min;
    int min_desc;
    float *U;
    unsigned long long *film;
    unsigned *counter;
    unsigned long long *wave_rays;
};

template <int WORLD, int STACK>
__device__ __forceinline__ Hit<float> trace_any(const DevScene &S, const PathState<float> &P, int *stk)
{
    return trace<WORLD, kBlock, STACK>(S, P.ro, P.rd, P.rtmax, P.shadow, stk);
}

template <int STACK, int WORLD, bool MATS, bool ENV = false>
__global__ __launch_bounds__(kBlock) void mlt_bootstrap(const DevScene S0, int nx, int ny, uint32_t seed, int n_init,
                                                        float *sc)
{
    DevScene S = S0;
    scene_strides_hbm(S);
    extern __shared__ __attribute__((aligned(16))) int lds_mem[];
    int *stk = lds_mem + threadIdx.x;
    const int i = blockIdx.x * kBlock + threadIdx.x;
    if (i >= n_init) return;
    PrndSource src{nullptr, 0, 0, rng_key(seed ^ kMltBootSalt, (uint32_t)i, 0u), 0u, true, 0.0f, 0.0f};
    MltPath M;
    mlt_begin(M, S, src, nx, ny);
    uint32_t ne = 0, ns = 0;
    for (;;) {
        if (mlt_beyond(M)) { M.P.L = M.P.L + M.P.beta * env_radiance<(ENV ? kMatsEnv : kMatsNone)>(S, M.P.rd); break; }
        const Hit<float> h = trace_any<WORLD, STACK>(S, M.P, stk);
        if (mlt_shade<MATS, ENV>(M, S, h, src, ne, ns)) break;
    }
    sc[i] = fmaxf(fmaxf(M.P.L.x, M.P.L.y), M.P.L.z);
}

constexpr int kSplatFix = 36;
__device__ __forceinline__ void mlt_splat(const MltWork &W, float x, float y, f3 c, float w)
{
    const int pix = mlt_pixel(x, y, W.nx, W.ny);
    if (pix < 0) return;
    const float k = W.scale * w;
    const double q = (double)(1ull << kSplatFix), lim = 9.2233720368547758e18;
    const double v[3] = {(double)(k * c.x) * q, (double)(k * c.y) * q, (double)(k * c.z) * q};
    if (!(v[0] >= 0.0 && v[0] < lim && v[1] >= 0.0 && v[1] < lim && v[2] >= 0.0 && v[2] < lim)) return;
    unsigned long long *f = W.film + 3 * (size_t)pix;
    atomicAdd(f + 0, (unsigned long long)__double2ll_rn(v[0]));
    atomicAdd(f + 1, (unsigned long long)__double2ll_rn(v[1]));
    atomicAdd(f + 2, (unsigned long long)__double2ll_rn(v[2]));
}

#ifndef FRT_EXP_MLT_WAVES
#define FRT_EXP_MLT_WAVES 4
#endif
template <int STACK, int WORLD, bool LDS_SCENE, bool MATS, bool ENV = false>
__global__ __launch_bounds__(kBlock) __attribute__((amdgpu_waves_per_eu(FRT_EXP_MLT_WAVES))) void mlt_megakernel(
    const DevScene S0, const MltWork W)
{
    extern __shared__ __attribute__((aligned(16))) int lds_mem[];
    int *stk = lds_mem + threadIdx.x;
    constexpr int kStackInts = WORLD != FRT_WORLD_LIST ? STACK * kBlock : 0;
    DevScene S = S0;
    if constexpr (LDS_SCENE) scene_to_lds<WORLD>(S, lds_mem + kStackInts + kChainWords * kBlock);
    else scene_strides_hbm(S);
    const int lane = threadIdx.x & 63;
    bool have = false, exhausted = false, init = false, large = false;
    const ItemState C{lds_mem + kStackInts + (int)threadIdx.x};
    uint32_t j = 0;
    RngKey key{0, 0};
    MltPath M;
    uint32_t n_cam = 0, n_ext = 0, n_sh = 0, n_smp = 0;

    auto source = [&]() {
        PrndSource src{W.U, W.n_local, j, key, 2u, init || large, W.s2p, W.logp};
        return src;
    };
    Trav<float> T;
    bool tracing = false, pending = false, beyond = false;
    int ovf[kOverflow<WORLD>];
    unsigned long long diag_t0 = FRT_DIAG_CLOCK();
    for (;;) {
        FRT_DIAG_TICK(6);
        for (;;) {
            bool ext = false;
            if (tracing) FRT_DIAG_TICK(3);
            if (tracing && trav_step_world<WORLD, kBlock, STACK, FRT_EXP_MLT_STEP>(T, S, M.P.ro, M.P.rd, M.P.shadow, stk, ovf,
                                                                 LDS_SCENE ? 0 : W.min_desc)) {
                if (M.P.shadow) {
                    if (!path_after_shadow<(MATS ? kMatsAll : kMatsNone)>(M.P, T.h.prim < 0)) {
                        tracing = false;
                        pending = true;
                    } else if (mlt_beyond(M)) {
                        beyond = true;
                        tracing = false;
                        pending = true;
                    } else {
                        ext = true;
                        tracing = trav_begin_world<WORLD>(T, S, M.P.ro, M.P.rd, M.P.rtmax);
                        pending = !tracing;
                    }
                } else {
                    tracing = false;
                    pending = true;
                }
            }
            if (ext) ++n_ext;
            if (__popcll(__ballot(tracing)) <= W.trav_min) break;
        }
        bool next_ray = false, done = false;
        const unsigned long long diag_t1 = FRT_DIAG_CLOCK();
        FRT_DIAG_CYC(16, diag_t1 - diag_t0);
        if (pending) {
            FRT_DIAG_TICK(4);
            pending = false;
            if (beyond) {
                M.P.L = M.P.L + M.P.beta * env_radiance<(ENV ? kMatsEnv : kMatsNone)>(S, M.P.rd);
                beyond = false;
                done = true;
            } else {
                uint32_t ne = 0, ns = 0;
                done = mlt_shade<MATS, ENV>(M, S, T.h, source(), ne, ns);
                n_ext += ne; n_sh += ns;
                next_ray = !done;
            }
        }
        const unsigned long long diag_t2 = FRT_DIAG_CLOCK();
        FRT_DIAG_CYC(17, diag_t2 - diag_t1);
        bool mat = false, mat_fresh = false, setup_next = false;
        RngKey mat_key = key;
        if (done) {
            FRT_DIAG_TICK(5);
            const f3 L = M.P.L;
            const float sc = fmaxf(fmaxf(L.x, L.y), L.z);
            float cx = i2f(C.get(kCsX)), cy = i2f(C.get(kCsY)), csc = i2f(C.get(kCsSc)), cw = i2f(C.get(kCsW));
            f3 cc = mk3(i2f(C.get(kCsCc)), i2f(C.get(kCsCc + 1)), i2f(C.get(kCsCc + 2)));
            uint32_t t = (uint32_t)C.get(kCsT);
            bool moved = false;
            if (init) {
                mat = true; mat_fresh = true;
                cx = M.x; cy = M.y; cc = L; csc = sc;
                moved = true;
                init = false;
            } else {
                float a = 1.0f;
                if (csc > 0.0f) a = fmaxf(fminf(1.0f, sc / csc), 0.0f);
                if (sc > 0.0f) mlt_splat(W, M.x, M.y, L, (a + (large ? 1.0f : 0.0f)) / (sc / W.b + kMltLargeStep));
                if (csc > 0.0f) cw += (1.0f - a) / (csc / W.b + kMltLargeStep);
                if (rng_u(key, 1) <= a) {
                    if (csc > 0.0f && cw != 0.0f) mlt_splat(W, cx, cy, cc, cw);
                    uint2 *fp = reinterpret_cast<uint2 *>(W.U + (size_t)j * kMltRow + kMltFp);
                    uint2 f = *fp;
                    f.x += 1u; f.y += t + 1u;
                    *fp = f;
                    cw = 0.0f;
                    mat = true; mat_fresh = large;
                    cx = M.x; cy = M.y; cc = L; csc = sc;
                    moved = true;
                }
                ++t;
                ++n_smp;
            }
            if ((uint64_t)t >= W.steps) {
                if (csc > 0.0f && cw != 0.0f) mlt_splat(W, cx, cy, cc, cw);
                have = false;
            } else {
                setup_next = true;
                C.set(kCsT, (int)t);
                C.set(kCsW, f2i(cw));
                if (moved) {
                    C.set(kCsX, f2i(cx)); C.set(kCsY, f2i(cy)); C.set(kCsSc, f2i(csc));
                    C.set(kCsCc, f2i(cc.x)); C.set(kCsCc + 1, f2i(cc.y)); C.set(kCsCc + 2, f2i(cc.z));
                }
            }
        }
        const unsigned long long diag_t3 = FRT_DIAG_CLOCK();
        FRT_DIAG_CYC(19, diag_t3 - diag_t2);
        if (const uint64_t mm = __ballot(mat)) {
            const uint32_t n = (uint32_t)__popcll(mm);
            const int dst = 4 * (int)(mat ? lane_rank(mm) : n + lane_rank(~mm));
            const uint32_t rj = (uint32_t)__builtin_amdgcn_ds_permute(dst, (int)(j | (mat_fresh ? 0x80000000u : 0u)));
            const uint32_t rk0 = (uint32_t)__builtin_amdgcn_ds_permute(dst, (int)mat_key.k0);
            const uint32_t rk1 = (uint32_t)__builtin_amdgcn_ds_permute(dst, (int)mat_key.k1);
            const uint32_t total = n * (uint32_t)kMltDims;
            for (uint32_t e0 = 0; e0 < total; e0 += 64) {
                const uint32_t e = e0 + (uint32_t)lane;
                const uint32_t r = min(e / (uint32_t)kMltDims, n - 1u);
                const uint32_t jl = (uint32_t)__shfl((int)rj, (int)r);
                const RngKey kl{(uint32_t)__shfl((int)rk0, (int)r), (uint32_t)__shfl((int)rk1, (int)r)};
                if (e < total) {
                    const int d = (int)(e - r * (uint32_t)kMltDims);
                    float *row = W.U + (size_t)(jl & 0x7fffffffu) * kMltRow;
                    const float u = rng_u(kl, 2u + (uint32_t)d);
                    row[d] = (jl >> 31) ? u : mlt_mutate(row[d], u, d, W.s2p, W.logp);
                }
            }
        }
        const unsigned long long diag_t4 = FRT_DIAG_CLOCK();
        FRT_DIAG_CYC(20, diag_t4 - diag_t3);
        if (setup_next) {
            key = rng_key(W.seed ^ kMltChainSalt, (uint32_t)C.get(kCsC), (uint32_t)C.get(kCsT) + 1u);
            large = rng_u(key, 0) < kMltLargeStep;
            mlt_begin(M, S, source(), W.nx, W.ny);
            ++n_cam;
            next_ray = true;
        }
        const bool need = !have && !exhausted;
        const uint64_t m = __ballot(need);
        if (m) {
            const int leader = __ffsll((unsigned long long)m) - 1;
            uint32_t base = 0;
            if (lane == leader) base = atomicAdd(W.counter, (unsigned)__popcll(m));
            base = __shfl(base, leader);
            if (need) {
                const uint32_t w = base + lane_rank(m);
                if (w >= W.n_local) {
                    exhausted = true;
                } else {
                    have = true;
                    init = true;
                    j = w;
                    *reinterpret_cast<uint2 *>(W.U + (size_t)w * kMltRow + kMltFp) = make_uint2(0u, 0u);
                    const uint32_t c = (uint32_t)W.shard_index + w * (uint32_t)W.shard_count;
                    C.set(kCsC, (int)c);
                    C.set(kCsT, 0);
                    C.set(kCsW, 0);
                    C.set(kCsSc, 0);
                    key = rng_key(W.seed ^ kMltChainSalt, c, 0u);
                    mlt_begin(M, S, source(), W.nx, W.ny);
                    ++n_cam;
                    next_ray = true;
                }
            }
        }
        if (next_ray) {
            if (mlt_beyond(M)) {
                beyond = true;
                pending = true;
            } else {
                tracing = trav_begin_world<WORLD>(T, S, M.P.ro, M.P.rd, M.P.rtmax);
                pending = !tracing;
            }
        }
        diag_t0 = FRT_DIAG_CLOCK();
        FRT_DIAG_CYC(18, diag_t0 - diag_t4);
        if (__ballot(have || !exhausted) == 0) break;
    }
    unsigned long long cnt[4] = {n_cam, n_ext, n_sh, n_smp};
    for (int k = 0; k < 4; ++k)
        for (int off = 32; off > 0; off >>= 1) cnt[k] += __shfl_xor(cnt[k], off);
    if (lane == 0) {
        const size_t wv = ((size_t)blockIdx.x * kBlock + threadIdx.x) >> 6;
        for (int k = 0; k < 4; ++k) W.wave_rays[4 * wv + k] = cnt[k];
    }
}

}
```

first_raytracer_amd/csrc/frt_path.hpp:

```cpp
#pragma once
#include "frt.h"
#include "frt_device.hpp"

namespace frt {

FRT_HD int f2i(float f) { return __builtin_bit_cast(int, f); }
FRT_HD float i2f(int i) { return __builtin_bit_cast(float, i); }
constexpr int kMatStride = 5;
FRT_HD float u2f(uint32_t u) { return __builtin_bit_cast(float, u); }
FRT_HD bool wave_any(bool x)
{
#if defined(__HIP_DEVICE_COMPILE__)
    return __ballot(x) != 0;
#else
    return x;
#endif
}

FRT_HD int wave_count(bool x)
{
#if defined(__HIP_DEVICE_COMPILE__)
    return __popcll(__ballot(x));
#else
    return x ? 1 : 0;
#endif
}

#if defined(FRT_DIAG)
constexpr int kDiagSlots = 24;
extern __device__ unsigned long long *frt_diag;
#endif
#if defined(FRT_DIAG) && defined(__HIP_DEVICE_COMPILE__)
__device__ __forceinline__ unsigned long long *diag_slot()
{
    return frt_diag + (size_t)((blockIdx.x * blockDim.x + threadIdx.x) >> 6) * kDiagSlots;
}
#define FRT_DIAG_TICK(k)                                                                \
    do {                                                                                \
        const uint64_t m_ = __ballot(1);                                                \
        if ((int)(threadIdx.x & 63) == __ffsll((unsigned long long)m_) - 1 && frt_diag) { \
            unsigned long long *d_ = diag_slot();                                       \
            d_[2 * (k)] += 1;                                                           \
            d_[2 * (k) + 1] += __popcll(m_);                                            \
        }                                                                               \
    } while (0)
#define FRT_DIAG_CYC(k, c)                                                              \
    do {                                                                                \
        const uint64_t m_ = __ballot(1);                                                \
        if ((int)(threadIdx.x & 63) == __ffsll((unsigned long long)m_) - 1 && frt_diag) diag_slot()[k] += (c); \
    } while (0)
#define FRT_DIAG_CLOCK() ((unsigned long long)clock64())
#else
#define FRT_DIAG_TICK(k) do {} while (0)
#define FRT_DIAG_CYC(k, c) do {} while (0)
#define FRT_DIAG_CLOCK() 0ull
#endif

constexpr int kSentinel = 0x7fffffff;
constexpr int kStepBranch = 0, kStepStore = 1, kStepSelect = 2;
constexpr int kWorldBvh4 = 2;
constexpr int kWorldBvh2Oct = 4;
#ifndef FRT_EXP_BVH4_OVF
#define FRT_EXP_BVH4_OVF 44
#endif
constexpr int kBvh4Overflow = FRT_EXP_BVH4_OVF;
template <int WORLD> constexpr int kOverflow = WORLD == kWorldBvh4 ? kBvh4Overflow : 1;

struct DevScene {
    const float4 *nodes;
    const float4 *tris;
    const float4 *tshade;
    const float4 *tnorm;
    const float4 *spheres;
    const int *sphere_mat;
    const float4 *mats;
    const float4 *tuv;
    const float4 *texels;
    const int *lights;
    const int *list;
    const int *tri_view;
    const uint4 *nodes4;
    const float4 *nodes_oct;
    const int2 *node_refs;
    const double4 *tris64;
    const double4 *tshade64;
    const double4 *tnorm64;
    const double4 *spheres64;
    int root;
    int root4;
    int n_lights, n_list, world_kind;
    int n_nodes, n_tris, n_mats;
    int node_es, node_ps, tri_es, tri_ps, sh_es, sh_ps, node4_es, node4_ps;
    int n_nodes4;
    float root_lo[3], root_hi[3];
    float ao_tmax;
    int ao_spheres_only;
    f3 cam_o, cam_llc, cam_h, cam_v, cam_u, cam_vv, cam_w;
    float lens_r, cam_half_height;
    d3 cam64_o, cam64_llc, cam64_h, cam64_v, cam64_u, cam64_vv;
    double lens_r64;
    f3 env;
    const float4 *env_texels;
    int env_nx, env_ny;
};

template <typename R> struct Hit {
    int prim;
    R t, u, v;
};

constexpr int kLeafCountShift = 27, kLeafIndexMask = (1 << kLeafCountShift) - 1, kLeafIndexLimit = 1 << kLeafCountShift;
constexpr int kLeafMax = 8, kLeafDefault = 4, kLeafSmallScene = 2;
constexpr int kTravMinLds = 12, kTravMinHbm = 32;
constexpr int kTravMinLdsPath = 20, kTravMinHbmPath = 40;
constexpr int kMinDescLds = 0, kMinDescHbm = 12;

FRT_HD float4 node_part(const DevScene &S, int i, int k) { return S.nodes[i * S.node_es + k * S.node_ps]; }
FRT_HD uint4 node4_part(const DevScene &S, int i, int k) { return S.nodes4[i * S.node4_es + k * S.node4_ps]; }
constexpr int kNode4Parts = 4;
FRT_HD float4 tri_part(const DevScene &S, int i, int k) { return S.tris[i * S.tri_es + k * S.tri_ps]; }
FRT_HD float4 shade_part(const DevScene &S, int i, int k) { return S.tshade[i * S.sh_es + k * S.sh_ps]; }

template <typename R> FRT_HD V3<R> tri_vec(const DevScene &S, int i, int k)
{
    if constexpr (kIsF64<R>) return xyz(S.tris64[3 * i + k]);
    else return xyz(tri_part(S, i, k));
}
template <typename R> FRT_HD void sphere_get(const DevScene &S, int k, V3<R> &c, R &r)
{
    if constexpr (kIsF64<R>) { const double4 q = S.spheres64[k]; c = xyz(q); r = q.w; }
    else { const float4 q = S.spheres[k]; c = xyz(q); r = q.w; }
}
template <typename R> FRT_HD V3<R> geo_normal(const DevScene &S, int i)
{
    if constexpr (kIsF64<R>) return xyz(S.tshade64[i]);
    else return xyz(shade_part(S, i, 0));
}
template <typename R> FRT_HD R inv_area(const DevScene &S, int i)
{
    if constexpr (kIsF64<R>) return S.tshade64[i].w;
    else return shade_part(S, i, 0).w;
}
template <typename R> FRT_HD V3<R> vert_normal(const DevScene &S, int i, int k)
{
    if constexpr (kIsF64<R>) return xyz(S.tnorm64[3 * i + k]);
    else return xyz(S.tnorm[3 * i + k]);
}
template <typename R> FRT_HD V3<R> env_of(const DevScene &S) { return V3<R>{R(S.env.x), R(S.env.y), R(S.env.z)}; }
template <typename R> struct CamView { V3<R> o, llc, h, v, u, vv; R lens_r; };
template <typename R> FRT_HD CamView<R> cam_view(const DevScene &S)
{
    if constexpr (kIsF64<R>) return CamView<R>{S.cam64_o, S.cam64_llc, S.cam64_h, S.cam64_v, S.cam64_u, S.cam64_vv, S.lens_r64};
    else return CamView<R>{S.cam_o, S.cam_llc, S.cam_h, S.cam_v, S.cam_u, S.cam_vv, S.lens_r};
}

template <bool STRAIGHT = false, typename R>
FRT_HD R prim_t(const DevScene &S, int ref, V3<R> o, V3<R> d, R tmin, R tmax, R &u, R &v)
{
    if (ref & FRT_PRIM_SPHERE) {
        V3<R> c;
        R r;
        sphere_get(S, ref & ~FRT_PRIM_SPHERE, c, r);
        u = v = R(0);
        return sphere_intersect(o, d, c, r, tmin, tmax);
    }
    const V3<R> a = tri_vec<R>(S, ref, 0), b = tri_vec<R>(S, ref, 1), c = tri_vec<R>(S, ref, 2);
    return tri_intersect<STRAIGHT>(o, d, a, b, c, tmin, tmax, u, v);
}

template <bool STRAIGHT = false, typename R>
FRT_HD bool leaf_hit(const DevScene &S, int lref, V3<R> o, V3<R> d, R tmin, bool anyhit, Hit<R> &h)
{
    if constexpr (STRAIGHT) {
        const bool is_sph = (lref & FRT_PRIM_SPHERE) != 0;
        const int first = is_sph ? lref : (lref & kLeafIndexMask);
        const int count = is_sph ? 1 : (lref >> kLeafCountShift) + 1;
        for (int k = 0; k < count; ++k) {
            FRT_DIAG_TICK(1);
            const int ref = first + k;
            R u, v;
            const R t = prim_t<STRAIGHT>(S, ref, o, d, tmin, h.t, u, v);
            if (t > R(0) && ((t < h.t) || (h.prim >= 0 && (is_sph || ref < h.prim)))) {
                h.prim = ref; h.t = t; h.u = u; h.v = v;
                if (anyhit) return true;
            }
        }
        return false;
    }
    if (lref & FRT_PRIM_SPHERE) {
        FRT_DIAG_TICK(1);
        R u, v;
        const R t = prim_t(S, lref, o, d, tmin, h.t, u, v);
        if (t > R(0) && ((t < h.t) || h.prim >= 0)) {
            h.prim = lref; h.t = t; h.u = u; h.v = v;
            return anyhit;
        }
        return false;
    }
    const int first = lref & kLeafIndexMask;
    const int count = (lref >> kLeafCountShift) + 1;
    for (int k = 0; k < count; ++k) {
        FRT_DIAG_TICK(1);
        const int ref = first + k;
        R u, v;
        const V3<R> a = tri_vec<R>(S, ref, 0), b = tri_vec<R>(S, ref, 1), c = tri_vec<R>(S, ref, 2);
        const R t = tri_intersect<STRAIGHT>(o, d, a, b, c, tmin, h.t, u, v);
        if (t > R(0) && ((t < h.t) || ref < h.prim)) {
            h.prim = ref; h.t = t; h.u = u; h.v = v;
            if (anyhit) return true;
        }
    }
    return false;
}

template <typename R> struct Trav {
    SlabRay<R> sr;
    R tmin;
    int node, sp;
    Hit<R> h;
};

template <typename R> FRT_HD R bvh_tmin(V3<R> o)
{
    return Cst<R>::eps * vmax(R(1), vmax(vabs(o.x), vmax(vabs(o.y), vabs(o.z))));
}

template <typename R> FRT_HD bool trav_begin(Trav<R> &T, const DevScene &S, int root, V3<R> o, V3<R> d, R tmax)
{
    T.h = Hit<R>{-1, tmax, R(0), R(0)};
    T.sp = 0;
    T.node = root;
    T.sr = slab_ray(o, d);
    T.tmin = bvh_tmin(o);
    return slab_entry<R>(S.root_lo[0], S.root_lo[1], S.root_lo[2], S.root_hi[0], S.root_hi[1], S.root_hi[2], T.sr,
                         Cst<R>::eps, tmax) != R(__builtin_inff());
}

template <int STRIDE, bool OCT = false, int STEP = kStepBranch, typename R>
FRT_HD bool bvh2_step(Trav<R> &T, const DevScene &S, V3<R> o, V3<R> d, bool anyhit, int *stk, int min_desc = 0)
{
    int node = T.node, sp = T.sp;
    DevScene Sn = S;
    if constexpr (OCT) {
        const int oct = (T.sr.invd.x < R(0) ? 1 : 0) | (T.sr.invd.y < R(0) ? 2 : 0) | (T.sr.invd.z < R(0) ? 4 : 0);
        Sn.nodes = S.nodes + oct * 3 * S.n_nodes;
    }
    const R tmin = T.tmin, tbest = OCT ? vmin(T.h.t, Cst<R>::tmax) : T.h.t;
    while ((unsigned)node < (unsigned)kSentinel) {
        FRT_DIAG_TICK(2);
        R t0, t1;
        int c0, c1;
        bool h0, h1;
        if constexpr (OCT) {
            const float4 *rec = Sn.nodes + u24mul(node, 3);
            const float4 n0 = rec[0], n1 = rec[1], n2 = rec[2];
            const int2 cr = S.node_refs[node];
            R f0, f1;
            slab_nf<R>(n0.x, n0.y, n0.z, n0.w, n1.x, n1.y, T.sr, tmin, tbest, t0, f0);
            slab_nf<R>(n1.z, n1.w, n2.x, n2.y, n2.z, n2.w, T.sr, tmin, tbest, t1, f1);
            h0 = t0 <= f0; h1 = t1 <= f1;
            c0 = cr.x; c1 = cr.y;
        } else {
            const float4 n0 = node_part(Sn, node, 0), n1 = node_part(Sn, node, 1);
            const float4 n2 = node_part(Sn, node, 2), n3 = node_part(Sn, node, 3);
            t0 = slab_entry<R>(n0.x, n0.y, n0.z, n0.w, n1.x, n1.y, T.sr, tmin, tbest);
            t1 = slab_entry<R>(n1.z, n1.w, n2.x, n2.y, n2.z, n2.w, T.sr, tmin, tbest);
            h0 = t0 != R(__builtin_inff()); h1 = t1 != R(__builtin_inff());
            c0 = f2i(n3.x); c1 = f2i(n3.y);
        }
        if constexpr (OCT && STEP == kStepSelect) {
            const bool first0 = h0 && (!h1 || t0 <= t1);
            const int nr = first0 ? c0 : c1, fr = first0 ? c1 : c0;
            const int below = stk[(sp > 0 ? sp - 1 : 0) * STRIDE];
            stk[sp * STRIDE] = fr;
            const bool both = h0 && h1, any = h0 || h1;
            node = any ? nr : (sp > 0 ? below : kSentinel);
            sp += both ? 1 : (!any && sp > 0 ? -1 : 0);
        } else if constexpr (OCT && STEP == kStepStore) {
            const bool first0 = h0 && (!h1 || t0 <= t1);
            const int nr = first0 ? c0 : c1, fr = first0 ? c1 : c0;
            stk[sp * STRIDE] = fr;
            sp += (h0 && h1) ? 1 : 0;
            if (h0 || h1) node = nr;
            else node = (sp > 0) ? stk[--sp * STRIDE] : kSentinel;
        } else if (h0 && h1) {
            const bool first0 = t0 <= t1;
            stk[sp * STRIDE] = first0 ? c1 : c0;
            ++sp;
            node = first0 ? c0 : c1;
        } else if (h0) {
            node = c0;
        } else if (h1) {
            node = c1;
        } else {
            node = (sp > 0) ? stk[--sp * STRIDE] : kSentinel;
        }
        if (min_desc > 0 && wave_count((unsigned)node < (unsigned)kSentinel) < min_desc) break;
    }
    if ((unsigned)node < (unsigned)kSentinel) {
        T.node = node;
        T.sp = sp;
        return false;
    }
    bool done = node == kSentinel || leaf_hit(S, ~node, o, d, T.tmin, anyhit, T.h);
    if (!done) {
        node = (sp > 0) ? stk[--sp * STRIDE] : kSentinel;
        done = node == kSentinel;
    }
    T.node = node;
    T.sp = sp;
    return done;
}

template <int STRIDE, int LSTACK>
FRT_HD bool bvh4_step(Trav<float> &T, const DevScene &S, f3 o, f3 d, bool anyhit, int *stk, int *ovf, int min_desc = 0)
{
    int node = T.node, sp = T.sp;
    auto push = [&](int v) {
        if (!wave_any(sp >= LSTACK)) {
            stk[sp * STRIDE] = v;
        } else {
            if (sp < LSTACK) stk[sp * STRIDE] = v;
            else ovf[sp - LSTACK] = v;
        }
        ++sp;
    };
    auto pop = [&]() -> int {
        if (sp == 0) return kSentinel;
        --sp;
        if (!wave_any(sp >= LSTACK)) return stk[sp * STRIDE];
        return sp < LSTACK ? stk[sp * STRIDE] : ovf[sp - LSTACK];
    };
    while ((unsigned)node < (unsigned)kSentinel) {
        FRT_DIAG_TICK(0);
        const uint4 w0 = node4_part(S, node, 0), w1 = node4_part(S, node, 1);
        const uint4 w2 = node4_part(S, node, 2), w3 = node4_part(S, node, 3);
        const SlabRay<float> &sr = T.sr;
        const float ax = ldexpf(sr.invd.x, (int)(int8_t)(w0.w & 0xffu)), bx = fmaf(u2f(w0.x), sr.invd.x, sr.oinv.x);
        const float ay = ldexpf(sr.invd.y, (int)(int8_t)((w0.w >> 8) & 0xffu)), by = fmaf(u2f(w0.y), sr.invd.y, sr.oinv.y);
        const float az = ldexpf(sr.invd.z, (int)(int8_t)((w0.w >> 16) & 0xffu)), bz = fmaf(u2f(w0.z), sr.invd.z, sr.oinv.z);
        const bool sx = sr.invd.x < 0.0f, sy = sr.invd.y < 0.0f, sz = sr.invd.z < 0.0f;
        float t[4];
        int c[4] = {(int)w1.x, (int)w1.y, (int)w1.z, (int)w1.w};
        const uint32_t xn = sx ? w2.y : w2.x, xf = sx ? w2.x : w2.y;
        const uint32_t yn = sy ? w2.w : w2.z, yf = sy ? w2.z : w2.w;
        const uint32_t zn = sz ? w3.y : w3.x, zf = sz ? w3.x : w3.y;
#pragma unroll
        for (int i = 0; i < 4; ++i) {
            const int sh = 8 * i;
            const float txn = fmaf((float)((xn >> sh) & 0xffu), ax, bx), txf = fmaf((float)((xf >> sh) & 0xffu), ax, bx);
            const float tyn = fmaf((float)((yn >> sh) & 0xffu), ay, by), tyf = fmaf((float)((yf >> sh) & 0xffu), ay, by);
            const float tzn = fmaf((float)((zn >> sh) & 0xffu), az, bz), tzf = fmaf((float)((zf >> sh) & 0xffu), az, bz);
            const float tn = smax(smax(txn, tyn), smax(tzn, T.tmin));
            const float tf = smin(smin(txf, tyf), smin(tzf, T.h.t));
            t[i] = (tf < tn) ? __builtin_inff() : tn;
        }
        auto cx = [&](int i, int j) {
            const bool sw = t[j] < t[i];
            const float ti = sw ? t[j] : t[i], tj = sw ? t[i] : t[j];
            const int ci = sw ? c[j] : c[i], cj = sw ? c[i] : c[j];
            t[i] = ti; t[j] = tj; c[i] = ci; c[j] = cj;
        };
        cx(0, 1); cx(2, 3); cx(0, 2); cx(1, 3); cx(1, 2);
        if (!wave_any(sp > LSTACK - 3)) {
            if (t[3] != __builtin_inff()) stk[sp++ * STRIDE] = c[3];
            if (t[2] != __builtin_inff()) stk[sp++ * STRIDE] = c[2];
            if (t[1] != __builtin_inff()) stk[sp++ * STRIDE] = c[1];
        } else {
            if (t[3] != __builtin_inff()) push(c[3]);
            if (t[2] != __builtin_inff()) push(c[2]);
            if (t[1] != __builtin_inff()) push(c[1]);
        }
        node = (t[0] != __builtin_inff()) ? c[0] : pop();
        if (min_desc > 0 && wave_count((unsigned)node < (unsigned)kSentinel) < min_desc) break;
    }
    if ((unsigned)node < (unsigned)kSentinel) {
        T.node = node;
        T.sp = sp;
        return false;
    }
    bool done = node == kSentinel || leaf_hit<true>(S, ~node, o, d, T.tmin, anyhit, T.h);
    if (!done) {
        node = pop();
        done = node == kSentinel;
    }
    T.node = node;
    T.sp = sp;
    return done;
}

template <int STRIDE, typename R>
FRT_HD Hit<R> trace_bvh(const DevScene &S, V3<R> o, V3<R> d, R tmax, bool anyhit, int *stk)
{
    Trav<R> T;
    if (trav_begin(T, S, S.root, o, d, tmax))
        while (!bvh2_step<STRIDE>(T, S, o, d, anyhit, stk)) {}
    return T.h;
}

template <int STRIDE, int LSTACK, int OVF>
FRT_HD Hit<float> trace_bvh4(const DevScene &S, f3 o, f3 d, float tmax, bool anyhit, int *stk)
{
    Trav<float> T;
    int ovf[OVF];
    if (trav_begin(T, S, S.root4, o, d, tmax))
        while (!bvh4_step<STRIDE, LSTACK>(T, S, o, d, anyhit, stk, ovf)) {}
    return T.h;
}

template <typename R> FRT_HD Hit<R> trace_list(const DevScene &S, V3<R> o, V3<R> d, R tmax, bool anyhit)
{
    Hit<R> h{-1, tmax, R(0), R(0)};
    for (int i = 0; i < S.n_list; ++i) {
#if defined(__HIP_DEVICE_COMPILE__)
        const int ref = frt_uniform(((const __attribute__((address_space(4))) int *)S.list)[frt_uniform(i)]);
#else
        const int ref = S.list[i];
#endif
        R u, v;
#if defined(__HIP_DEVICE_COMPILE__)
        R t;
        if constexpr (kIsF64<R>) {
            typedef const __attribute__((address_space(4))) double4 *cptr;
            if (ref & FRT_PRIM_SPHERE) {
                const cptr sb = (cptr)S.spheres64;
                const double4 q = sb[ref & ~FRT_PRIM_SPHERE];
                u = v = R(0);
                t = sphere_intersect(o, d, xyz(q), q.w, Cst<R>::eps, h.t);
            } else {
                const cptr tb = (cptr)S.tris64;
                const double4 a = tb[3 * ref], b = tb[3 * ref + 1], c = tb[3 * ref + 2];
                t = tri_intersect(o, d, xyz(a), xyz(b), xyz(c), Cst<R>::eps, h.t, u, v);
            }
        } else {
            typedef const __attribute__((address_space(4))) float4 *cptr;
            if (ref & FRT_PRIM_SPHERE) {
                const cptr sb = (cptr)S.spheres;
                const float4 q = sb[ref & ~FRT_PRIM_SPHERE];
                u = v = R(0);
                t = sphere_intersect(o, d, xyz(q), q.w, Cst<R>::eps, h.t);
            } else {
                const cptr tb = (cptr)S.tris;
                const float4 a = tb[ref * S.tri_es], b = tb[ref * S.tri_es + S.tri_ps], c = tb[ref * S.tri_es + 2 * S.tri_ps];
                t = tri_intersect(o, d, xyz(a), xyz(b), xyz(c), Cst<R>::eps, h.t, u, v);
            }
        }
#else
        const R t = prim_t(S, ref, o, d, Cst<R>::eps, h.t, u, v);
#endif
        if (t > R(0) && ((ref & FRT_PRIM_SPHERE) || t < h.t)) {
            h.prim = ref; h.t = t; h.u = u; h.v = v;
            if (anyhit) return h;
        }
    }
    return h;
}

template <int WORLD, int STRIDE, int STACK = 0, typename R>
FRT_HD Hit<R> trace(const DevScene &S, V3<R> o, V3<R> d, R tmax, bool anyhit, int *stk)
{
    if constexpr (WORLD == FRT_WORLD_LIST) return trace_list(S, o, d, tmax, anyhit);
    else if constexpr (WORLD == kWorldBvh4) return trace_bvh4<STRIDE, STACK, kBvh4Overflow>(S, o, d, tmax, anyhit, stk);
    else return trace_bvh<STRIDE>(S, o, d, tmax, anyhit, stk);
}

template <int WORLD, typename R>
FRT_HD bool trav_begin_world(Trav<R> &T, const DevScene &S, V3<R> o, V3<R> d, R tmax)
{
    if constexpr (WORLD == FRT_WORLD_LIST) {
        T.h = Hit<R>{-1, tmax, R(0), R(0)};
        return true;
    } else {
        return trav_begin(T, S, WORLD == kWorldBvh4 ? S.root4 : S.root, o, d, tmax);
    }
}
template <int WORLD, int STRIDE, int STACK, int STEP = kStepBranch, typename R>
FRT_HD bool trav_step_world(Trav<R> &T, const DevScene &S, V3<R> o, V3<R> d, bool anyhit, int *stk, int *ovf,
                            int min_desc = 0)
{
    if constexpr (WORLD == kWorldBvh4) {
        static_assert(!kIsF64<R>, "the fp64 kernels traverse the binary tree");
        T.sr = slab_ray(o, d);
        T.tmin = bvh_tmin(o);
    }
    if constexpr (WORLD == FRT_WORLD_LIST) {
        T.h = trace_list(S, o, d, T.h.t, anyhit);
        return true;
    } else if constexpr (WORLD == kWorldBvh4) {
        return bvh4_step<STRIDE, STACK>(T, S, o, d, anyhit, stk, ovf, min_desc);
    } else {
        return bvh2_step<STRIDE, WORLD == kWorldBvh2Oct, STEP>(T, S, o, d, anyhit, stk, min_desc);
    }
}

template <typename R>
FRT_HD void prim_shade(const DevScene &S, int ref, V3<R> ro, V3<R> p, R u, R v, V3<R> &n, int &mat)
{
    if (ref & FRT_PRIM_SPHERE) {
        const int k = ref & ~FRT_PRIM_SPHERE;
        V3<R> c;
        R r;
        sphere_get(S, k, c, r);
        n = rcp(r) * (p - c);
        if (len2(ro - c) < r * r) n = -n;
        mat = S.sphere_mat[k];
        return;
    }
    const float4 s1 = shade_part(S, ref, 1);
    mat = f2i(s1.x);
    if (f2i(s1.y)) {
        n = geo_normal<R>(S, ref);
    } else {
        const V3<R> n0 = vert_normal<R>(S, ref, 0), n1 = vert_normal<R>(S, ref, 1), n2 = vert_normal<R>(S, ref, 2);
        n = normalize((R(1) - u - v) * n0 + u * n1 + v * n2);
    }
}

template <typename R>
FRT_HD R prim_pdf(const DevScene &S, int ref, V3<R> rec_p, R rec_t, V3<R> rec_n, V3<R> to_light)
{
    if (!(ref & FRT_PRIM_SPHERE)) return inv_area<R>(S, ref);
    V3<R> c;
    R r;
    sphere_get(S, ref & ~FRT_PRIM_SPHERE, c, r);
    const V3<R> o = rec_p - rec_t * to_light;
    const V3<R> dir = c - o;
    const R d2 = len2(dir);
    const R r2 = r * r;
    if (d2 <= r2) return rcp(R(4) * Cst<R>::pi * r2);
    const R cos_max = fsqrt(R(1) - fdiv(r2, d2));
    const R solid = R(2) * Cst<R>::pi * (R(1) - cos_max);
    return fdiv(rcp(solid) * vabs(dot(to_light, rec_n)), d2);
}

template <typename R>
FRT_HD V3<R> prim_sample(const DevScene &S, int ref, V3<R> o, R u0, R u1, V3<R> &ln, int &lmat)
{
    if (ref & FRT_PRIM_SPHERE) {
        const int k = ref & ~FRT_PRIM_SPHERE;
        V3<R> c;
        R r;
        sphere_get(S, k, c, r);
        lmat = S.sphere_mat[k];
        const V3<R> direction = c - o;
        const R d2 = len2(direction);
        if (d2 <= r * r) {
            const V3<R> p = c + r * uniform_sphere(u0, u1);
            ln = normalize(c - p);
            return p - o;
        }
        const Onb<R> uvw = onb_from_w(direction);
        const V3<R> p = onb_local(uvw, random_to_sphere(r, d2, u0, u1));
        ln = normalize(p);
        return p;
    }
    const V3<R> a = tri_vec<R>(S, ref, 0), b = tri_vec<R>(S, ref, 1), c = tri_vec<R>(S, ref, 2);
    const R su0 = fsqrt(u0);
    const R b0 = R(1) - su0;
    const R b1 = u1 * su0;
    const V3<R> lp = a + b0 * b + b1 * c;
    const float4 s1 = shade_part(S, ref, 1);
    lmat = f2i(s1.x);
    if (f2i(s1.y)) {
        ln = geo_normal<R>(S, ref);
    } else {
        const V3<R> n0 = vert_normal<R>(S, ref, 0), n1 = vert_normal<R>(S, ref, 1), n2 = vert_normal<R>(S, ref, 2);
        ln = normalize((R(1) - b0 - b1) * n0 + b0 * n1 + b1 * n2);
    }
    return lp - o;
}

constexpr int kMatsNone = 0, kMatsTex = 1, kMatsSpec = 2, kMatsRough = 4, kMatsAll = 7;
constexpr int kMatsEnv = 8;
constexpr int kMatsEnvNee = 16;
constexpr int kMatsRoulette = 32;
constexpr int kRouletteDepth = 3;
constexpr int kMatsSobol = 64;
constexpr int kMatsFeatures = kMatsRoulette | kMatsSobol;
constexpr int kMatsSpecAny = kMatsSpec | kMatsRough;
template <int MATS> FRT_HD RngKey smp_key(uint32_t seed, uint32_t pixel, uint32_t sample)
{
    if constexpr ((MATS & kMatsSobol) != 0) return sobol_key(seed, pixel, sample);
    else return rng_key(seed, pixel, sample);
}
template <int MATS, typename R> FRT_HD R smp_r(RngKey k, uint32_t dim)
{
    if constexpr ((MATS & kMatsSobol) != 0) return R(sobol_u(k, dim));
    else return rng_r<R>(k, dim);
}

template <typename R> FRT_HD int x86_trunc(R x)
{
    if (!(x > R(-2147483649.0f) && x < R(2147483648.0f))) return (int)0x80000000;
    return (int)x;
}
FRT_HD int imodulo2(int a) { const int r = a % 2; return r < 0 ? r + 2 : r; }
FRT_HD float vatan2(float y, float x) { return atan2f(y, x); }
FRT_HD double vatan2(double y, double x) { return atan2(y, x); }
FRT_HD float vasin(float x) { return asinf(x); }
FRT_HD double vasin(double x) { return asin(x); }
template <typename R> FRT_HD void prim_uv(const DevScene &S, int ref, V3<R> p, R u, R v, R &tu, R &tv)
{
    if (ref & FRT_PRIM_SPHERE) {
        V3<R> c;
        R r;
        sphere_get(S, ref & ~FRT_PRIM_SPHERE, c, r);
        const V3<R> q = p - c;
        const R phi = vatan2(q.z, q.x), theta = vasin(q.y);
        tu = R(1) - (phi + Cst<R>::pi) / (R(2) * Cst<R>::pi);
        tv = (theta + R(0.5f) * Cst<R>::pi) / Cst<R>::pi;
        return;
    }
    const float4 a = S.tuv[2 * ref], b = S.tuv[2 * ref + 1];
    const R w = R(1) - u - v;
    tu = (w * R(a.x) + u * R(a.z)) + v * R(b.x);
    tv = (w * R(a.y) + u * R(a.w)) + v * R(b.y);
}
FRT_HD int imodulo(int a, int b) { const int r = a % b; return r < 0 ? r + b : r; }
template <typename R> FRT_HD int image_index(int nx, int ny, R tu, R tv)
{
    int i = x86_trunc(tu * (R)nx), j = x86_trunc(tv * (R)ny);
    if (i < 0 || i > nx) i = imodulo(i, nx);
    if (j < 0 || j > ny) j = imodulo(j, ny);
    if (i == nx) i = nx - 1;
    if (j == ny) j = ny - 1;
    return j * nx + i;
}
template <typename R> FRT_HD f3 image_texel(const DevScene &S, float4 m4, R tu, R tv)
{
    return xyz(S.texels[f2i(m4.z) + image_index(f2i(m4.x), f2i(m4.y), tu, tv)]);
}
template <typename R> FRT_HD int env_index(const DevScene &S, V3<R> rd)
{
    const V3<R> d = normalize(rd);
    R dy = d.y;
    if constexpr (!kIsF64<R>) dy = vmin(vmax(dy, R(-1)), R(1));
    R phi = vatan2(d.x, -d.z), theta = vacos(dy);
    if (phi < R(0)) phi = phi + Cst<R>::pi * R(2);
    if (theta < R(0)) theta = theta + Cst<R>::pi;
    const R u = phi / (R(2) * Cst<R>::pi), v = theta / Cst<R>::pi;
    return image_index(S.env_nx, S.env_ny, u, v);
}
template <typename R> FRT_HD V3<R> env_texel(const DevScene &S, int k)
{
    const f3 c = xyz(S.env_texels[k]);
    return V3<R>{R(c.x), R(c.y), R(c.z)};
}
template <typename R> FRT_HD V3<R> env_eval(const DevScene &S, V3<R> rd) { return env_texel<R>(S, env_index(S, rd)); }

FRT_HD const float *env_marginal(const DevScene &S)
{
    return reinterpret_cast<const float *>(S.env_texels + (size_t)S.env_nx * (size_t)S.env_ny);
}
FRT_HD const float *env_conditional(const DevScene &S, int j)
{
    return env_marginal(S) + (S.env_ny + 1) + (size_t)j * (size_t)(S.env_nx + 1);
}
template <typename R> FRT_HD int env_cdf_find(const float *cdf, int n, R u)
{
    int lo = 0, hi = n;
    while (hi - lo > 1) {
        const int mid = (lo + hi) >> 1;
        if (R(cdf[mid]) <= u) lo = mid; else hi = mid;
    }
    return lo;
}
template <typename R> FRT_HD R env_row_dcos(const DevScene &S, int j, R &c0)
{
    const R half = Cst<R>::pi / (R)(2 * S.env_ny);
    c0 = vcos((R)(2 * j) * half);
    return R(2) * vsin((R)(2 * j + 1) * half) * vsin(half);
}
template <typename R> FRT_HD R env_density(const DevScene &S, R prob, R dc)
{
    return fdiv(prob * (R)S.env_nx, R(2) * Cst<R>::pi * dc);
}
template <typename R> struct EnvSample { V3<R> d, E; R pdf; };
template <typename R> FRT_HD EnvSample<R> env_sample(const DevScene &S, R u0, R u1)
{
    const R below_one = R(0x1.fffffep-1f);
    u0 = vmin(u0, below_one); u1 = vmin(u1, below_one);
    const float *marg = env_marginal(S);
    const int j = env_cdf_find(marg, S.env_ny, u0);
    const float *cond = env_conditional(S, j);
    const int i = env_cdf_find(cond, S.env_nx, u1);
    const R m0 = R(marg[j]), pm = R(marg[j + 1]) - m0, q0 = R(cond[i]), pq = R(cond[i + 1]) - q0;
    const R t0 = vmin(fdiv(u0 - m0, pm), below_one), t1 = vmin(fdiv(u1 - q0, pq), below_one);
    R c0;
    const R dc = env_row_dcos(S, j, c0);
    const R ct = vmin(vmax(c0 - t0 * dc, R(-1)), R(1)), st = fsqrt(vmax(R(1) - ct * ct, R(0)));
    const R phi = R(2) * Cst<R>::pi * fdiv((R)i + t1, (R)S.env_nx);
    EnvSample<R> e;
    e.d = V3<R>{st * vsin(phi), ct, -st * vcos(phi)};
    e.E = env_texel<R>(S, j * S.env_nx + i);
    e.pdf = env_density(S, pm * pq, dc);
    return e;
}
template <typename R> FRT_HD R env_pdf(const DevScene &S, int k)
{
    const int j = k / S.env_nx, i = k - j * S.env_nx;
    const float *m = env_marginal(S) + j, *q = env_conditional(S, j) + i;
    R c0;
    return env_density(S, (R(m[1]) - R(m[0])) * (R(q[1]) - R(q[0])), env_row_dcos(S, j, c0));
}
template <int MATS, typename R> FRT_HD V3<R> env_radiance(const DevScene &S, V3<R> rd)
{
    if constexpr ((MATS & kMatsEnv) != 0) return env_eval<R>(S, rd);
    else return env_of<R>(S);
}
template <typename R>
FRT_HD void apply_texture(const DevScene &S, int mat, int mtype, int ref, V3<R> p, R u, R v, float4 &m0, float4 &m1)
{
    const float4 m3 = S.mats[kMatStride * mat + 3];
    const int tex = f2i(m3.w);
    if (tex == FRT_TEX_CONSTANT) return;
    const float4 m4 = S.mats[kMatStride * mat + 4];
    R tu, tv;
    prim_uv(S, ref, p, u, v, tu, tv);
    f3 c;
    if (tex == FRT_TEX_IMAGE) {
        c = image_texel(S, m4, tu, tv);
    } else {
        const int x = 2 * imodulo2(x86_trunc(tu * R(m4.x) * R(2))) - 1, y = 2 * imodulo2(x86_trunc(tv * R(m4.y) * R(2))) - 1;
        if (x * y != 1) return;
        c = xyz(m3);
    }
    if (mtype == FRT_MAT_LAMBERTIAN || mtype == FRT_MAT_MODIFIED_PHONG) { m0.x = c.x; m0.y = c.y; m0.z = c.z; }
    else { m1.x = c.x; m1.y = c.y; m1.z = c.z; }
}

template <typename R> struct PathState {
    V3<R> ro, rd;
    R rtmax;
    bool shadow;
    bool term;
    V3<R> beta, L;
    V3<R> nee;
    V3<R> nxt_d;
    V3<R> nxt_o;
    V3<R> prev_p;
    R prev_pdf;
    bool prev_spec;
    int depth;
    RngKey key;
};

template <int MATS = kMatsNone, typename R>
FRT_HD void path_begin(PathState<R> &P, const DevScene &S, int px, int py, int nx, int ny, uint32_t seed,
                       uint32_t pixel, uint32_t sample)
{
    P.key = smp_key<MATS>(seed, pixel, sample);
    const CamView<R> cam = cam_view<R>(S);
    const R u = fdiv((R)px + smp_r<MATS, R>(P.key, 0), (R)nx);
    const R v = fdiv((R)py + smp_r<MATS, R>(P.key, 1), (R)ny);
    V3<R> off = zero3<R>();
    if (cam.lens_r != R(0)) {
        const R a = smp_r<MATS, R>(P.key, 2) * R(2) - R(1), b = smp_r<MATS, R>(P.key, 3) * R(2) - R(1);
        R rx = R(0), ry = R(0);
        if (a != R(0) || b != R(0)) {
            R r, phi;
            if (a * a > b * b) { r = a; phi = (Cst<R>::pi / R(4)) * (b / a); }
            else { r = b; phi = (Cst<R>::pi / R(2)) - (Cst<R>::pi / R(4)) * (a / b); }
            rx = r * vcos(phi); ry = r * vsin(phi);
        }
        off = (cam.lens_r * rx) * cam.u + (cam.lens_r * ry) * cam.vv;
    }
    P.ro = cam.o + off;
    P.rd = ((cam.llc + u * cam.h + v * cam.v) - cam.o) - off;
    P.rtmax = Cst<R>::tmax;
    P.shadow = false;
    P.term = false;
    P.depth = 0;
    P.beta = V3<R>{R(1), R(1), R(1)};
    P.L = zero3<R>();
    P.prev_pdf = R(0);
    P.prev_p = zero3<R>();
    P.prev_spec = false;
}

template <int MATS = kMatsAll, typename R>
FRT_HD bool path_after_shadow(PathState<R> &P, bool unoccluded)
{
    P.shadow = false;
    if constexpr ((MATS & kMatsRoulette) != 0) {
        if (unoccluded) P.L = P.L + P.nee;
        if (P.term) return false;
    } else {
        if (P.term) return false;
        if (unoccluded) P.L = P.L + P.nee;
    }
    if constexpr ((MATS & kMatsSpecAny) != 0) P.ro = P.nxt_o;
    P.rd = P.nxt_d; P.rtmax = Cst<R>::tmax;
    ++P.depth;
    return true;
}

struct SpecMat {
    int type;
    float4 m0, m1, m2;
};
FRT_HD SpecMat spec_mat(const DevScene &S, int mat, int type, float4 m0, float4 m1)
{
    SpecMat M{type, m0, m1, make_float4(0.0f, 0.0f, 0.0f, 0.0f)};
    if (type == FRT_MAT_ROUGH_CONDUCTOR) M.m2 = S.mats[kMatStride * mat + 2];
    return M;
}
template <int MATS = kMatsAll, typename R>
FRT_HD V3<R> spec_generate(const SpecMat &M, V3<R> n, V3<R> wi, R s0, R s1, R &sampled_pdf)
{
    sampled_pdf = R(-1);
    switch (M.type) {
    case FRT_MAT_MODIFIED_PHONG: return cosine_power_generate(n, wi, R(M.m1.w), s0, s1);
    case FRT_MAT_DIELECTRIC: return dielectric_generate(n, wi, R(M.m1.w), s0);
    case FRT_MAT_METAL: return reflect(-wi, n);
    default:
        if constexpr ((MATS & kMatsRough) != 0)
            return normalize(rough_generate(n, wi, R(M.m1.w), f2i(M.m2.w), s0, s1, sampled_pdf));
        return reflect(-wi, n);
    }
}
template <int MATS = kMatsAll, typename R>
FRT_HD R spec_value(const SpecMat &M, V3<R> n, V3<R> wi, V3<R> wo)
{
    switch (M.type) {
    case FRT_MAT_MODIFIED_PHONG: return cosine_power_value(n, wi, R(M.m1.w), wo);
    case FRT_MAT_DIELECTRIC: return dielectric_value(n, wi, R(M.m1.w), wo);
    case FRT_MAT_METAL: return R(1);
    default:
        if constexpr ((MATS & kMatsRough) != 0) return rough_value(n, wi, R(M.m1.w), f2i(M.m2.w), wo);
        return R(1);
    }
}
template <int MATS = kMatsAll, typename R>
FRT_HD V3<R> spec_eval(const SpecMat &M, V3<R> n, V3<R> wi, V3<R> wo)
{
    switch (M.type) {
    case FRT_MAT_MODIFIED_PHONG: return phong_eval(rgb<R>(M.m0), rgb<R>(M.m1), R(M.m1.w), n, wi, wo);
    case FRT_MAT_DIELECTRIC: return dielectric_eval(rgb<R>(M.m1), R(M.m1.w), n, wi, wo);
    case FRT_MAT_METAL: return rgb<R>(M.m0);
    default:
        if constexpr ((MATS & kMatsRough) != 0)
            return rough_eval(rgb<R>(M.m0), rgb<R>(M.m2), rgb<R>(M.m1), R(M.m1.w), f2i(M.m2.w), n, wi, wo);
        return rgb<R>(M.m0);
    }
}
FRT_HD bool mat_is_specular(int t)
{
    return t == FRT_MAT_MODIFIED_PHONG || t == FRT_MAT_METAL || t == FRT_MAT_DIELECTRIC || t == FRT_MAT_ROUGH_CONDUCTOR;
}
FRT_HD bool mat_no_mis(int t) { return t == FRT_MAT_MODIFIED_PHONG || t == FRT_MAT_METAL || t == FRT_MAT_DIELECTRIC; }

template <int MATS = kMatsAll, typename R>
FRT_HD bool path_shade(PathState<R> &P, const DevScene &S, const Hit<R> &h, int max_depth, uint32_t &n_ext, uint32_t &n_sh)
{
    constexpr bool kEnvNee = (MATS & kMatsEnvNee) != 0;
    constexpr bool kRoulette = (MATS & kMatsRoulette) != 0;
    if (P.shadow) {
        if (!path_after_shadow<MATS>(P, h.prim < 0)) return true;
        ++n_ext;
        return false;
    }
    if (P.term) return true;
    if (h.prim < 0) {
        if constexpr (kEnvNee) {
            if (P.depth != 0 && !P.prev_spec) {
                const int k = env_index(S, P.rd);
                P.L = P.L + mi_weight(P.prev_pdf, env_pdf<R>(S, k)) * (P.beta * env_texel<R>(S, k));
                return true;
            }
        }
        P.L = P.L + P.beta * env_radiance<MATS>(S, P.rd);
        return true;
    }
    const V3<R> p = P.ro + h.t * P.rd;
    V3<R> n;
    int mat;
    prim_shade(S, h.prim, P.ro, p, h.u, h.v, n, mat);
    float4 m0 = S.mats[kMatStride * mat], m1 = S.mats[kMatStride * mat + 1];
    const int mtype = f2i(m0.w);
    if constexpr ((MATS & kMatsTex) != 0) apply_texture(S, mat, mtype, h.prim, p, h.u, h.v, m0, m1);
    if (mtype == FRT_MAT_DIFFUSE_LIGHT && dot(n, P.rd) < R(0)) {
        const V3<R> Le = rgb<R>(m1);
        if (P.depth == 0 || P.prev_spec) {
            P.L = P.L + P.beta * Le;
        } else {
            const R cos_wo = dot(n, -normalize(P.rd));
            R d2 = len2(p - P.prev_p);
            if (d2 <= Cst<R>::eps) d2 = Cst<R>::eps;
            const R light_pdf = fdiv(prim_pdf(S, h.prim, p, h.t, n, P.rd) * d2, vabs(cos_wo));
            P.L = P.L + mi_weight(P.prev_pdf, light_pdf) * (P.beta * Le);
        }
        return true;
    }
    const bool lamb = mtype == FRT_MAT_LAMBERTIAN, spec = (MATS & kMatsSpecAny) && mat_is_specular(mtype);
    if (!(lamb || spec) || P.depth > max_depth) return true;
    const bool diel = (MATS & kMatsSpec) && mtype == FRT_MAT_DIELECTRIC;
    const uint32_t base = dim_bounce(P.depth);
    V3<R> wo, beta_next;
    R pdf;
    const V3<R> wi = -normalize(P.rd);
    SpecMat M{};
    if (!(MATS & kMatsSpecAny) || lamb) {
        const Onb<R> uvw = onb_from_w(n);
        wo = onb_local(uvw, cosine_direction(smp_r<MATS, R>(P.key, base + 6), smp_r<MATS, R>(P.key, base + 7)));
        const R cw = dot(n, normalize(wo));
        pdf = vmax(cw, R(0)) * Cst<R>::inv_pi;
        beta_next = fdiv(vabs(cw), pdf) * (P.beta * (Cst<R>::inv_pi * rgb<R>(m0)));
    } else {
        M = spec_mat(S, mat, mtype, m0, m1);
        R sampled;
        wo = spec_generate<MATS>(M, n, wi, smp_r<MATS, R>(P.key, base + 0), smp_r<MATS, R>(P.key, base + 1), sampled);
        pdf = spec_value<MATS>(M, n, wi, wo);
        if (sampled > R(0)) pdf = sampled;
        const V3<R> bsdf = spec_eval<MATS>(M, n, wi, wo);
        beta_next = P.beta * (rcp(pdf) * bsdf);
    }
    const int nl = S.n_lights;
    R pick = smp_r<MATS, R>(P.key, base + 3);
    bool env_pick = false;
    R inv_sel = R(1);
    if constexpr (kEnvNee) {
        if (lamb || mtype == FRT_MAT_ROUGH_CONDUCTOR) {
            env_pick = nl == 0 || pick < R(0.5f);
            if (nl != 0) {
                inv_sel = R(2);
                pick = env_pick ? pick * R(2) : pick * R(2) - R(1);
            }
        }
    }
    int idx = (int)(pick * (R)nl);
    if (idx == nl) idx -= 1;
// ... 187 lines not shown
```

first_raytracer_amd/csrc/frt_selftest.hip:

```cpp
#include <algorithm>
#include <cstring>
#include <string>
#include <vector>

#include "frt_ctx.hpp"
#include "frt_flatten.hpp"
#include "host/envdist.hpp"

using namespace frt;

constexpr int kSelftestStack = 8;

template <typename R, int MATS = kMatsAll>
static void selftest_pixels(const DevScene &S, const FlatScene &F, const frt_render_params *p, const int32_t *pixels,
                            int npix, bool wide, std::vector<int> &stack, float *out_rgb, uint64_t cnt[3])
{
    uint32_t n_ext = 0, n_sh = 0;
    for (int i = 0; i < npix; ++i) {
        const int pix = pixels[i];
        const int px = pix % p->nx, py = pix / p->nx;
        V3<R> acc = zero3<R>();
        for (int smp = 0; smp < p->spp; ++smp) {
            PathState<R> P;
            path_begin<MATS>(P, S, px, py, p->nx, p->ny, p->seed, (uint32_t)pix, (uint32_t)(smp + p->sample_offset));
            ++cnt[0];
            for (;;) {
                Hit<R> h;
                if (S.world_kind == FRT_WORLD_LIST) {
                    h = trace<FRT_WORLD_LIST, 1>(S, P.ro, P.rd, P.rtmax, P.shadow, stack.data());
                } else if constexpr (!kIsF64<R>) {
                    h = wide ? trace<kWorldBvh4, 1, kSelftestStack>(S, P.ro, P.rd, P.rtmax, P.shadow, stack.data())
                             : trace<FRT_WORLD_BVH, 1>(S, P.ro, P.rd, P.rtmax, P.shadow, stack.data());
                } else {
                    h = trace<FRT_WORLD_BVH, 1>(S, P.ro, P.rd, P.rtmax, P.shadow, stack.data());
                }
                n_ext = n_sh = 0;
                const bool done = p->integrator == FRT_INTEGRATOR_AO ? ao_shade<MATS>(P, S, h, n_sh)
                                  : p->integrator == FRT_INTEGRATOR_NORMALS ? normals_shade<MATS>(P, S, h)
                                  : p->integrator == FRT_INTEGRATOR_ALBEDO ? albedo_shade(P, S, h)
                                  : p->integrator == FRT_INTEGRATOR_DEPTH ? depth_shade(P, S, h)
                                  : path_shade<MATS>(P, S, h, p->max_depth, n_ext, n_sh);
                cnt[1] += n_ext; cnt[2] += n_sh;
                if (done) break;
            }
            acc = acc + P.L;
        }
        if (p->integrator == FRT_INTEGRATOR_ALBEDO || p->integrator == FRT_INTEGRATOR_DEPTH) {
            const R n = (R)p->spp;
            out_rgb[3 * i] = (float)(acc.x / n); out_rgb[3 * i + 1] = (float)(acc.y / n); out_rgb[3 * i + 2] = (float)(acc.z / n);
            if (p->integrator == FRT_INTEGRATOR_DEPTH)
                out_rgb[3 * i + 1] = depth_moment_floor(out_rgb[3 * i], out_rgb[3 * i + 1], out_rgb[3 * i + 2]);
            continue;
        }
        const R k = R(1) / (R)p->spp;
        out_rgb[3 * i] = (float)(acc.x * k); out_rgb[3 * i + 1] = (float)(acc.y * k); out_rgb[3 * i + 2] = (float)(acc.z * k);
    }
}

extern "C" int frt_selftest_path_host(const frt_scene_view *sv, const frt_render_params *p, const int32_t *pixels,
                                      int npix, float *out_rgb, frt_stats *st)
{
    return frt_selftest_path_host_env(sv, p, pixels, npix, nullptr, out_rgb, st);
}
extern "C" int frt_selftest_path_host_env(const frt_scene_view *sv, const frt_render_params *p, const int32_t *pixels,
                                          int npix, const frt_image *env, float *out_rgb, frt_stats *st)
{
    if (!sv || !p || !pixels || !out_rgb || npix < 0 || p->spp <= 0 || p->nx <= 0 || p->ny <= 0) return FRT_E_INVALID;
    for (int i = 0; i < npix; ++i)
        if (pixels[i] < 0 || pixels[i] >= p->nx * p->ny) return FRT_E_INVALID;
    if (p->integrator == FRT_INTEGRATOR_DENOISE) return FRT_E_INVALID;
    if (p->integrator == FRT_INTEGRATOR_ERROR) return FRT_E_INVALID;
    const bool feature = p->integrator == FRT_INTEGRATOR_ALBEDO || p->integrator == FRT_INTEGRATOR_DEPTH;
    if (feature) env = nullptr;
    const bool f64 = (p->flags & FRT_FLAG_FP64) != 0 && !feature;
    FlatScene F;
    std::string err;
    const int rc = flatten_scene(sv, F, err, f64);
    if (rc != FRT_OK) return rc;
    if (p->integrator == FRT_INTEGRATOR_AO)
        for (int i = 0; i < sv->n_materials; ++i)
            if (sv->materials[i].type == FRT_MAT_METAL) return FRT_E_UNSUPPORTED;
    DevScene S = host_scene(F);
    std::vector<float4> env_tex;
    bool env_sampling = false;
    if (env) {
        const int erc = env_texels_of(env, env_tex, err);
        if (erc != FRT_OK) return erc;
        if ((p->flags & FRT_FLAG_ENV_SAMPLING) && p->integrator != FRT_INTEGRATOR_AO &&
            p->integrator != FRT_INTEGRATOR_NORMALS) {
            std::vector<float> tab;
            env_sampling = env_tables_of(&env_tex[0].x, env->nx, env->ny, tab);
            const size_t n = env_tex.size();
            env_tex.resize(n + tab.size() / 4);
            memcpy(reinterpret_cast<float *>(env_tex.data() + n), tab.data(), tab.size() * sizeof(float));
        }
        S.env_texels = env_tex.data(); S.env_nx = env->nx; S.env_ny = env->ny;
    }
    std::vector<int> stack(std::max(F.depth + 1, kSelftestStack));
    const bool wide = !f64 && S.world_kind == FRT_WORLD_BVH && F.has4 && !(p->flags & FRT_FLAG_BVH2) &&
                      bvh4_stack_fits(F.depth4, kSelftestStack);
    uint64_t cnt[3] = {0, 0, 0};
    constexpr int kEnvAll = kMatsAll | kMatsEnv;
    constexpr int kEnvNee = kEnvAll | kMatsEnvNee;
    const bool path = p->integrator == FRT_INTEGRATOR_PATH;
    const bool roulette = (p->flags & FRT_FLAG_ROULETTE) && path, sobol = (p->flags & FRT_FLAG_SOBOL) && path;
    auto run_set = [&](auto extra) {
        constexpr int X = decltype(extra)::value;
        auto run = [&](auto mats) {
            constexpr int M = decltype(mats)::value;
            if (f64) selftest_pixels<double, M | X>(S, F, p, pixels, npix, wide, stack, out_rgb, cnt);
            else selftest_pixels<float, M | X>(S, F, p, pixels, npix, wide, stack, out_rgb, cnt);
        };
        if (env_sampling) run(std::integral_constant<int, kEnvNee>{});
        else if (env) run(std::integral_constant<int, kEnvAll>{});
        else run(std::integral_constant<int, kMatsAll>{});
    };
    if (sobol && roulette) run_set(std::integral_constant<int, kMatsSobol | kMatsRoulette>{});
    else if (sobol) run_set(std::integral_constant<int, kMatsSobol>{});
    else if (roulette) run_set(std::integral_constant<int, kMatsRoulette>{});
    else run_set(std::integral_constant<int, 0>{});
    if (st) {
        memset(st, 0, sizeof(*st));
        st->camera_rays = cnt[0]; st->extension_rays = cnt[1]; st->shadow_rays = cnt[2];
        st->samples = cnt[0]; st->pixels = (uint64_t)npix;
        st->stack_entries = wide ? (uint32_t)kSelftestStack : (uint32_t)stack.size();
        st->bvh_depth = (uint32_t)(wide ? F.depth4 : F.depth);
        st->fp64 = f64 ? 1u : 0u;
    }
    return FRT_OK;
}


extern "C" int frt_selftest_mlt_paths_host(const frt_scene_view *sv, int nx, int ny, uint32_t seed, int n,
                                           float *out6)
{
    if (!sv || !out6 || n < 0 || nx <= 0 || ny <= 0) return FRT_E_INVALID;
    FlatScene F;
    std::string err;
    const int rc = flatten_scene(sv, F, err, false);
    if (rc != FRT_OK) return rc;
    const DevScene S = host_scene(F);
    std::vector<int> stack(std::max(F.depth + 1, 1));
    for (int i = 0; i < n; ++i) {
        PrndSource src{nullptr, 0, 0, rng_key(seed ^ kMltBootSalt, (uint32_t)i, 0u), 0u, true, 0.0f, 0.0f};
        MltPath M;
        mlt_begin(M, S, src, nx, ny);
        uint32_t ne = 0, ns = 0;
        for (;;) {
            if (mlt_beyond(M)) { M.P.L = M.P.L + M.P.beta * env_of<float>(S); break; }
            const Hit<float> h = (S.world_kind == FRT_WORLD_LIST)
                              ? trace<FRT_WORLD_LIST, 1>(S, M.P.ro, M.P.rd, M.P.rtmax, M.P.shadow, stack.data())
                              : trace<FRT_WORLD_BVH, 1>(S, M.P.ro, M.P.rd, M.P.rtmax, M.P.shadow, stack.data());
            if (mlt_shade(M, S, h, src, ne, ns)) break;
        }
        const f3 L = M.P.L;
        float *o = &out6[6 * (size_t)i];
        o[0] = M.x; o[1] = M.y; o[2] = L.x; o[3] = L.y; o[4] = L.z; o[5] = fmaxf(fmaxf(L.x, L.y), L.z);
    }
    return FRT_OK;
}

extern "C" int frtx_selftest_tree_refine(const frt_scene_view *sv, frt_tree_cost out[2], float *nodes_off,
                                        float *nodes_on, int32_t max_nodes)
{
    if (!sv || !out) return FRT_E_INVALID;
    float *dst[2] = {nodes_off, nodes_on};
    for (int on = 0; on < 2; ++on) {
        FlatScene F;
        std::string err;
        const int rc = flatten_scene(sv, F, err, false, on);
        if (rc != FRT_OK) return rc;
        TreeCost c;
        const bool applies = tree_cost_host(F, c);
        const int nn = (int)(F.nodes.size() / 4);
        out[on] = frt_tree_cost{c.V, c.T, c.J, c.w, c.depth, nn, c.n_rays, applies ? 1 : 0};
        if (dst[on]) {
            if (nn > max_nodes) return FRT_E_INVALID;
            memcpy(dst[on], F.nodes.data(), F.nodes.size() * sizeof(float4));
        }
    }
    return FRT_OK;
}

extern "C" int frtx_selftest_trace_host(const frt_scene_view *sv, const float *rays, int64_t n, float *hits)
{
    if (!sv || n < 0 || (n > 0 && (!rays || !hits))) return FRT_E_INVALID;
    FlatScene F;
    std::string err;
    const int rc = flatten_scene(sv, F, err, false);
    if (rc != FRT_OK) return rc;
    const DevScene S = host_scene(F);
    std::vector<int> stack(std::max(F.depth + 1, 1));
    for (int64_t i = 0; i < n; ++i) {
        const float *q = rays + 8 * i;
        const f3 o = mk3(q[0], q[1], q[2]), d = mk3(q[4], q[5], q[6]);
        const bool anyhit = (f2i(q[7]) & 1) != 0;
        const Hit<float> h = S.world_kind == FRT_WORLD_LIST ? trace<FRT_WORLD_LIST, 1>(S, o, d, q[3], anyhit, stack.data())
                                                            : trace<FRT_WORLD_BVH, 1>(S, o, d, q[3], anyhit, stack.data());
        const int ref = (h.prim < 0 || (h.prim & FRT_PRIM_SPHERE)) ? h.prim : F.tri_view[h.prim];
        float *r = hits + 4 * i;
        r[0] = h.t; r[1] = h.u; r[2] = h.v;
        const float refbits = i2f(ref);
        memcpy(&r[3], &refbits, sizeof(float));
    }
    return FRT_OK;
}
```

first_raytracer_amd/csrc/host/tree_refine.cpp:

```cpp
#include "tree_refine.hpp"

#include <algorithm>
#include <cstddef>
#include <cstring>

#include "frt.h"

namespace frt_refine {
namespace {

constexpr int kMaxLevels = 64;
constexpr int kChunks = 16;
constexpr double kSlack = 0.002;

struct Tables {
    int n_slots = 0;
    std::vector<float> tab;
};

inline void unite(const float *a, const float *b, float *out)
{
    for (int k = 0; k < 6; ++k) out[k] = std::min(a[k], b[k]);
}

void count_rays(const Topology &t, const RaySet &R, const Tables &tb, const int *dirty, int n_dirty, const int *local_of,
                int r0, int r1, uint64_t &V, uint64_t &T)
{
    const int L = t.n_leaves;
    const int *child = t.child.data();
    float loc[2 * kMaxLevels][6];
    for (int r = r0; r < r1; ++r) {
        if (!R.live[r]) continue;
        const float *base = &tb.tab[(size_t)r * tb.n_slots * 6];
        auto rec = [&](int s) { return n_dirty > 0 && local_of[s] >= 0 ? loc[local_of[s]] : base + 6 * s; };
        for (int k = 0; k < n_dirty; ++k) {
            const int j = dirty[k] - L;
            unite(rec(child[2 * j]), rec(child[2 * j + 1]), loc[k]);
        }
        const float tmin = R.tmin[r];
        const bool any = R.anyhit[r] != 0;
        const float *pt = &R.prim_t[(size_t)r * R.n_prims];
        float tb_ = R.tmax[r];
        int hp = -1, sp = 0, node = t.root;
        int stk[kMaxLevels];
        for (;;) {
            while (node >= L) {
                ++V;
                const int c0 = child[2 * (node - L)], c1 = child[2 * (node - L) + 1];
                const float *a = rec(c0), *b = rec(c1);
                const float t0 = std::max(std::max(a[0], a[1]), std::max(a[2], tmin));
                const float f0 = std::min(std::min(-a[3], -a[4]), std::min(-a[5], tb_));
                const float t1 = std::max(std::max(b[0], b[1]), std::max(b[2], tmin));
                const float f1 = std::min(std::min(-b[3], -b[4]), std::min(-b[5], tb_));
                const bool h0 = t0 <= f0, h1 = t1 <= f1;
                if (h0 && h1) {
                    const bool first0 = t0 <= t1;
                    stk[sp++] = first0 ? c1 : c0;
                    node = first0 ? c0 : c1;
                } else if (h0) {
                    node = c0;
                } else if (h1) {
                    node = c1;
                } else {
                    node = sp > 0 ? stk[--sp] : -1;
                }
            }
            if (node < 0) break;
            bool done = false;
            for (int k = R.prim_first[node]; k < R.prim_first[node + 1]; ++k) {
                ++T;
                const float th = pt[k];
                const int ref = R.prim_ref[k];
                const bool sph = (ref & FRT_PRIM_SPHERE) != 0;
                if (th > 0.0f && th <= tb_ && (th < tb_ || (sph ? hp >= 0 : ref < hp))) {
                    tb_ = th;
                    hp = ref;
                    if (any) { done = true; break; }
                }
            }
            if (done || sp == 0) break;
            node = stk[--sp];
        }
    }
}

void build_tables(const Topology &t, const RaySet &R, Tables &tb)
{
    const int L = t.n_leaves, nI = std::max(L - 1, 0);
    tb.n_slots = L + nI;
    tb.tab.resize((size_t)R.n * tb.n_slots * 6);
    std::vector<int> order, st{t.root};
    while (!st.empty()) {
        const int s = st.back();
        st.pop_back();
        if (s < L) continue;
        order.push_back(s);
        st.push_back(t.child[2 * (s - L)]);
        st.push_back(t.child[2 * (s - L) + 1]);
    }
    for (int r = 0; r < R.n; ++r) {
        float *base = &tb.tab[(size_t)r * tb.n_slots * 6];
        memcpy(base, &R.slab[(size_t)r * L * 6], sizeof(float) * 6 * L);
        for (size_t k = order.size(); k-- > 0;) {
            const int s = order[k], j = s - L;
            unite(base + 6 * t.child[2 * j], base + 6 * t.child[2 * j + 1], base + 6 * s);
        }
    }
}

}

int Topology::depth() const
{
    int d = 0, sp = 0;
    int st[2 * kMaxLevels][2];
    st[sp][0] = root; st[sp++][1] = 1;
    while (sp > 0) {
        const int s = st[--sp][0], lvl = st[sp][1];
        if (s < n_leaves) continue;
        d = std::max(d, lvl);
        if (lvl >= kMaxLevels) return lvl;
        st[sp][0] = child[2 * (s - n_leaves)]; st[sp++][1] = lvl + 1;
        st[sp][0] = child[2 * (s - n_leaves) + 1]; st[sp++][1] = lvl + 1;
    }
    return d;
}

Cost tree_cost(const Topology &t, const RaySet &R)
{
    Tables tb;
    build_tables(t, R, tb);
    uint64_t V = 0, T = 0;
    count_rays(t, R, tb, nullptr, 0, nullptr, 0, R.n, V, T);
    Cost c;
    if (R.n > 0) { c.V = (double)V / R.n; c.T = (double)T / R.n; }
    return c;
}

int refine(Topology &t, const RaySet &R, double w, int max_depth, int max_evals)
{
    const int L = t.n_leaves, nI = L - 1, nS = L + nI;
    if (nI < 2 || R.n <= 0 || max_depth >= kMaxLevels) return 0;
    Tables tb;
    std::vector<int> parent(nS, -1), local_of(nS, -1);
    int bound[kChunks + 1];
    for (int c = 0; c <= kChunks; ++c) bound[c] = (int)((int64_t)R.n * c / kChunks);
    double prefix[kChunks + 1] = {0.0};
    auto keep_tree = [&]() {
        std::fill(parent.begin(), parent.end(), -1);
        for (int j = 0; j < nI; ++j) { parent[t.child[2 * j]] = L + j; parent[t.child[2 * j + 1]] = L + j; }
        build_tables(t, R, tb);
        uint64_t V = 0, T = 0;
        for (int c = 0; c < kChunks; ++c) {
            count_rays(t, R, tb, nullptr, 0, nullptr, bound[c], bound[c + 1], V, T);
            prefix[c + 1] = (double)V + w * (double)T;
        }
    };
    keep_tree();
    auto in_subtree = [&](int x, int s) {
        for (; x >= 0; x = parent[x]) if (x == s) return true;
        return false;
    };
    auto side_of = [&](int par, int c) { return 2 * (par - L) + (t.child[2 * (par - L)] == c ? 0 : 1); };
    auto move = [&](int s, int x) {
        const int p = parent[s];
        const int q = t.child[side_of(p, s) ^ 1];
        const int g = parent[p];
        if (g < 0) t.root = q;
        else t.child[side_of(g, p)] = q;
        parent[q] = g;
        const int xp = parent[x];
        if (xp < 0) t.root = p;
        else t.child[side_of(xp, x)] = p;
        parent[p] = xp;
        t.child[2 * (p - L)] = x;
        t.child[2 * (p - L) + 1] = s;
        parent[x] = p;
        parent[s] = p;
        return g;
    };
    int evals = 0, kept = 0;
    bool improved = true;
    while (improved && evals < max_evals) {
        improved = false;
        for (int s = 0; s < nS && evals < max_evals; ++s) {
            if (parent[s] < 0) continue;
            int best_x = -1;
            double best_j = prefix[kChunks];
            const Topology keep = t;
            const std::vector<int> keep_parent = parent;
            const int p = parent[s], q = t.child[side_of(p, s) ^ 1];
            for (int x = 0; x < nS && evals < max_evals; ++x) {
                if (x == p || x == q || in_subtree(x, s)) continue;
                const int g = move(s, x);
                if (t.depth() <= max_depth) {
                    ++evals;
                    std::pair<int, int> dl[2 * kMaxLevels];
                    int nd = 0;
                    for (int start : {p, g})
                        for (int y = start; y >= 0; y = parent[y]) {
                            int lvl = 0;
                            for (int z = y; z >= 0; z = parent[z]) ++lvl;
                            dl[nd++] = {-lvl, y};
                        }
                    std::sort(dl, dl + nd);
                    nd = (int)(std::unique(dl, dl + nd) - dl);
                    int dirty[2 * kMaxLevels];
                    for (int k = 0; k < nd; ++k) { dirty[k] = dl[k].second; local_of[dirty[k]] = k; }
                    uint64_t V = 0, T = 0;
                    const double slack = kSlack * prefix[kChunks];
                    double j = 0.0;
                    bool ok = true;
                    for (int c = 0; c < kChunks && ok; ++c) {
                        count_rays(t, R, tb, dirty, nd, local_of.data(), bound[c], bound[c + 1], V, T);
                        j = (double)V + w * (double)T;
                        ok = j <= prefix[c + 1] + slack;
                    }
                    for (int k = 0; k < nd; ++k) local_of[dirty[k]] = -1;
                    if (ok && j < best_j) { best_j = j; best_x = x; }
                }
                t = keep;
                parent = keep_parent;
            }
            if (best_x < 0) continue;
            move(s, best_x);
            keep_tree();
            ++kept;
            improved = true;
        }
    }
    return kept;
}

}
```

first_raytracer_amd/csrc/host/tree_refine.hpp:

```cpp
#pragma once
#include <cstdint>
#include <vector>

namespace frt_refine {

struct RaySet {
    int n = 0, n_leaves = 0, n_prims = 0;
    std::vector<float> tmin, tmax;
    std::vector<uint8_t> anyhit, live;
    std::vector<float> slab;
    std::vector<int> prim_first;
    std::vector<int> prim_ref;
    std::vector<float> prim_t;
};

struct Topology {
    int n_leaves = 0, root = 0;
    std::vector<int> child;
    int depth() const;
};

struct Cost { double V = 0.0, T = 0.0; };
inline double cost_j(const Cost &c, double w) { return c.V + w * c.T; }

Cost tree_cost(const Topology &t, const RaySet &rays);

int refine(Topology &t, const RaySet &fit, double w, int max_depth, int max_evals);

}
```

include/frt.h:

```cpp
#ifndef FRT_H
#define FRT_H

#include <stdint.h>

#ifdef __cplusplus
extern "C" {
#endif

#define FRT_ABI_VERSION 9

enum {
    FRT_OK = 0,
    FRT_E_INVALID = -1,
    FRT_E_HIP = -2,
    FRT_E_NO_SCENE = -3,
    FRT_E_UNSUPPORTED = -4,
    FRT_E_IO = -5,
    FRT_E_NO_DEVICE = -6
};

enum { FRT_WORLD_BVH = 0, FRT_WORLD_LIST = 1 };
enum { FRT_MAT_LAMBERTIAN = 0,
       FRT_MAT_DIFFUSE_LIGHT = 1,
       FRT_MAT_MODIFIED_PHONG = 2,
// ... 45 lines not shown
} frt_material;
enum { FRT_TEX_CONSTANT = 0, FRT_TEX_CHECKER = 1, FRT_TEX_IMAGE = 2 };

enum { FRT_IMAGE_SRGB8 = 0, FRT_IMAGE_F32 = 1 };
typedef struct frt_image {
    int32_t nx, ny;
    int32_t format;
    int32_t reserved;
    const void *data;
} frt_image;

typedef struct frt_scene_view {
    int32_t world_kind;
    int32_t n_tris;
    const double *tri_v;
    const double *tri_n;
    const int32_t *tri_material;
    const uint8_t *tri_geometry_normal;
    const double *tri_inv_area;
    int32_t n_spheres;
    const double *sphere;
    const int32_t *sphere_material;
    int32_t n_materials;
    const frt_material *materials;
    int32_t n_nodes;
    int32_t root;
    const double *node_box;
    const int32_t *node_child;
    int32_t n_list;
    const int32_t *list;
    int32_t n_lights;
    const int32_t *lights;
    double cam_origin[3], cam_lower_left[3], cam_horizontal[3], cam_vertical[3];
    double cam_u[3], cam_v[3];
    double cam_lens_radius;
    double env_color[3];
    double cam_w[3];
    double cam_half_height;
    const double *tri_uv;
    int32_t n_images;
    const frt_image *images;
} frt_scene_view;

typedef struct frt_render_params {
    int32_t nx, ny;
    int32_t spp;
    uint32_t seed;
    int32_t max_depth;
    int32_t integrator;
    int32_t tile_size;
    int32_t shard_index;
    int32_t shard_count;
    int32_t samples_per_item;
    int32_t flags;
    int32_t mlt_chains;
    int32_t mlt_bootstrap;
    int32_t sample_offset;
} frt_render_params;

typedef struct frt_stats {
    uint64_t camera_rays;
    uint64_t extension_rays;
    uint64_t shadow_rays;
    uint64_t samples;
    uint64_t pixels;
    uint64_t work_items;
    double kernel_ms;
    double total_ms;
    uint32_t scene_in_lds;
    uint32_t waves_cap;
    uint32_t stack_entries;
    uint32_t bvh_depth;
    uint64_t scene_bytes;
    uint32_t fp64;
    uint32_t reserved;
} frt_stats;

int frt_get_abi_version(void);

typedef struct frt_ctx frt_ctx;
int frt_create(int hip_device, frt_ctx **out);
int frt_destroy(frt_ctx *ctx);
const char *frt_last_error(const frt_ctx *ctx);
int frt_set_precision(frt_ctx *ctx, int precision);

int frt_set_env_image(frt_ctx *ctx, const frt_image *img);

int frt_upload_scene(frt_ctx *ctx, const frt_scene_view *scene);

int64_t frt_shard_slot_count(const frt_render_params *p);
int frt_shard_slots(const frt_render_params *p, int32_t *slot_pixel);

int frt_render(frt_ctx *ctx, const frt_render_params *p, float *film_rgb, frt_stats *st);

int frt_render_multi(frt_ctx **ctxs, int n, const frt_render_params *p, float *film_rgb, frt_stats *st);

int frt_render_device(frt_ctx *ctx, const frt_render_params *p, float *slots_rgb, void *hip_stream,
                      frt_stats *st);

int frt_mlt_chain_state(frt_ctx *ctx, uint64_t first, uint64_t n, float *u_out, uint32_t *fp_out);

int frt_trace_device(frt_ctx *ctx, const float *rays, int64_t n, float *hits, int flags, void *hip_stream,
                     frt_stats *st);

typedef struct frt_host_scene frt_host_scene;
typedef struct frt_host_scene_info {
    int32_t n_tris, n_spheres, n_materials, n_lights, n_nodes, world_kind, n_list, bvh_depth;
    double load_ms, build_ms;
} frt_host_scene_info;
int frt_scene_create(const char *kind, const char *obj_path, double aspect, frt_host_scene **out);
int frt_scene_view_get(const frt_host_scene *s, frt_scene_view *view);

enum { FRT_SPHERE_WORLD = 1, FRT_SPHERE_LIGHTS = 2, FRT_SPHERE_BOTH = 3 };
int frt_scene_new(frt_host_scene **out);
int frt_scene_add_obj(frt_host_scene *s, const char *obj_path, const double *to_world16, const frt_material *bsdf,
                      int use_geometry_normals);
int frt_scene_add_sphere(frt_host_scene *s, const double *center, double radius, const frt_material *m, int where);
int frt_scene_set_camera(frt_host_scene *s, const double *lookfrom, const double *lookat, const double *vup,
                         double vfov, double aspect, double aperture, double focus_dist);
int frt_scene_set_env(frt_host_scene *s, const double *rgb);
int frt_scene_add_image(frt_host_scene *s, const frt_image *img, int *index);
int frt_scene_set_env_image(frt_host_scene *s, int index);
int frt_scene_env_image(const frt_host_scene *s, frt_image *out);
int frt_scene_finish(frt_host_scene *s, int world_kind);
enum { FRT_GPU_BVH_PLOC = 0, FRT_GPU_BVH_LBVH = 1, FRT_GPU_BVH_SAH = 2 };
int frt_scene_build_bvh_gpu(frt_host_scene *s, frt_ctx *ctx, double *device_ms);
int frt_scene_build_bvh_gpu_algo(frt_host_scene *s, frt_ctx *ctx, int algo, double *device_ms);
int frt_scene_build_bvh_sah(frt_host_scene *s);
int frt_scene_info(const frt_host_scene *s, frt_host_scene_info *info);
void frt_scene_destroy(frt_host_scene *s);

int frt_write_tessellated_obj(const char *src_obj, int k, const char *dst_obj);

int frt_read_hdr(const char *path, int32_t *nx, int32_t *ny, float *rgb);

int frt_write_pfm(const char *path, int nx, int ny, const float *rgb);

int frt_film_accumulate(float *acc, int64_t acc_spp, const float *pass, int64_t pass_spp, int64_t n);
int frt_tonemap_u8(const float *rgb, int nx, int ny, uint8_t *out_u8);
enum { FRT_IMAGE_PNG = 0, FRT_IMAGE_BMP = 1, FRT_IMAGE_JPG = 2 };
int frt_write_image(const char *path, int nx, int ny, const uint8_t *rgb_u8, int format);

int frt_selftest_path_host(const frt_scene_view *scene, const frt_render_params *p, const int32_t *pixels,
                           int npix, float *out_rgb, frt_stats *st);
int frt_selftest_path_host_env(const frt_scene_view *scene, const frt_render_params *p, const int32_t *pixels,
                               int npix, const frt_image *env, float *out_rgb, frt_stats *st);
int frt_selftest_mlt_paths_host(const frt_scene_view *scene, int nx, int ny, uint32_t seed, int n, float *out6);
typedef struct frt_tree_cost {
    double v, t, j, w;
    int32_t depth, n_nodes, n_rays, applies;
} frt_tree_cost;
int frtx_selftest_tree_refine(const frt_scene_view *scene, frt_tree_cost out[2], float *nodes_off, float *nodes_on,
                             int32_t max_nodes);
int frtx_selftest_trace_host(const frt_scene_view *scene, const float *rays, int64_t n, float *hits);
int frtx_selftest_chunk_variance(const float *partial, int n_chunks, int64_t n_slots, int spp, int spi, float *out);
typedef struct frt_plan_query {
    int32_t kind, integrator, flags;
    int32_t world_kind, stack_needed, has_bvh4, depth4;
    int32_t mats, has_spec_mats, env_image, env_sampling, has_f64, precision;
    int64_t scene_lds_bytes, scene_lds_bytes_oct;
} frt_plan_query;
typedef struct frt_plan_answer {
    int32_t rc, stack, waves, lds_scene, wide, f64;
    int64_t lds, scene_lds;
    int64_t lds_boot;
    uint64_t kernel, kernel_boot;
} frt_plan_answer;
int frtx_selftest_plan(const frt_plan_query *q, frt_plan_answer *a);

#ifdef __cplusplus
}
#endif
#endif
```

Measured before the change: 35440.

## Build a separate shadow-ray BVH that omits triangles which can never occlude lights

Adds a host-side classifier that marks triangles which provably cannot block any light-sample shadow ray (geometric rules against camera and light positions), then builds a pruned BVH root that skips those primitives. Light shadow rays in the path integrator start traversal from this shadow root instead of the main root, so they visit fewer nodes and triangles. It is enabled by default through an environment knob and falls back when materials are non-Lambertian or the LDS budget changes. The risk is extra nodes in LDS and correctness that depends on the conservativeness of the classification.

New measurement: 38300 (median of 6 runs). +8.1%, better.

```diff
diff --git a/first_raytracer_amd/__init__.py b/first_raytracer_amd/__init__.py
--- a/first_raytracer_amd/__init__.py
+++ b/first_raytracer_amd/__init__.py
@@ -162,6 +162,17 @@
         return {k: getattr(self, k) for k, _ in self._fields_}
 
 
+class ShadowTreeInfo(ctypes.Structure):
+    _fields_ = [(n, ctypes.c_int32) for n in ("why", "kept_prims", "dropped_prims", "rule_a", "rule_b", "nodes_main",
+                                              "nodes_added", "nodes_shared", "root", "empty", "n_rays",
+                                              "root_stops_main", "root_stops_shadow", "n_nodes")] + [
+        (n, ctypes.c_double) for n in ("v_main", "t_main", "v_shadow", "t_shadow")] + [
+        ("segments", ctypes.c_int64), ("segment_hits", ctypes.c_int64)]
+
+    def as_dict(self):
+        return {k: getattr(self, k) for k, _ in self._fields_}
+
+
 class PlanQuery(ctypes.Structure):
     _fields_ = [(n, ctypes.c_int32) for n in ("kind", "integrator", "flags", "world_kind", "stack_needed", "has_bvh4",
                                               "depth4", "mats", "has_spec_mats", "env_image", "env_sampling",
@@ -195,7 +206,7 @@
            "frt_set_env_image", "frt_scene_set_env_image", "frt_scene_env_image", "frt_read_hdr",
            "frt_selftest_path_host_env")
 EXPORTS_X = ("frtx_selftest_tree_refine", "frtx_selftest_trace_host", "frtx_selftest_chunk_variance",
-             "frtx_selftest_plan")
+             "frtx_selftest_plan", "frtx_selftest_shadow_tree")
 
 
 def lib():
@@ -261,6 +272,8 @@
     L.frt_selftest_path_host_env.argtypes = [ctypes.POINTER(SceneView), ctypes.POINTER(RenderParams), vp,
                                              ctypes.c_int, ctypes.POINTER(Image), vp, ctypes.POINTER(Stats)]
     L.frtx_selftest_tree_refine.argtypes = [ctypes.POINTER(SceneView), ctypes.POINTER(TreeCost), vp, vp, ctypes.c_int32]
+    L.frtx_selftest_shadow_tree.argtypes = [ctypes.POINTER(SceneView), ctypes.POINTER(ShadowTreeInfo), vp, vp,
+                                            ctypes.c_int32, ctypes.c_int64, ctypes.c_uint32]
     L.frtx_selftest_trace_host.argtypes = [ctypes.POINTER(SceneView), vp, ctypes.c_int64, vp]
     L.frtx_selftest_chunk_variance.argtypes = [vp, ctypes.c_int, ctypes.c_int64, ctypes.c_int, ctypes.c_int, vp]
     _lib = L
@@ -606,6 +619,17 @@
     return tuple((out[k].as_dict(), nodes[k][:out[k].n_nodes].copy()) for k in range(2))
 
 
+def selftest_shadow_tree(scene, segments=0, seed=1):
+    view = scene.view()
+    cap = max(2 * int(view.n_nodes), 1) + 4
+    nodes = np.zeros((cap, 16), np.float32)
+    dropped = np.zeros(max(int(view.n_tris), 1), np.uint8)
+    out = ShadowTreeInfo()
+    _check(lib().frtx_selftest_shadow_tree(ctypes.byref(view), ctypes.byref(out), dropped.ctypes.data, nodes.ctypes.data,
+                                           cap, int(segments), int(seed)), "frtx_selftest_shadow_tree")
+    return out.as_dict(), dropped[:int(view.n_tris)].copy(), nodes[:out.n_nodes].copy()
+
+
 def selftest_trace_host(scene, rays):
     rays = np.ascontiguousarray(rays, dtype=np.float32).reshape(-1, 8)
     hits = np.zeros((len(rays), 4), np.float32)
diff --git a/first_raytracer_amd/csrc/frt_flatten.hip b/first_raytracer_amd/csrc/frt_flatten.hip
--- a/first_raytracer_amd/csrc/frt_flatten.hip
+++ b/first_raytracer_amd/csrc/frt_flatten.hip
@@ -4,9 +4,11 @@
 #include <cfloat>
 #include <cmath>
 #include <cstdlib>
+#include <cstring>
 #include <functional>
 
 #include "frt_kernels.hpp"
+#include "host/shadow_tree.hpp"
 #include "host/tree_refine.hpp"
 
 using namespace frt;
@@ -300,18 +302,18 @@
 }
 
 static void sample_rays(const FlatScene &F, const std::vector<RefineLeaf> &leaves, int frame, uint32_t seed,
-                        frt_refine::RaySet &R)
+                        frt_refine::RaySet &R, std::vector<uint8_t> *occl = nullptr, std::vector<float> *origins = nullptr)
 {
     const DevScene S = host_scene(F);
-    struct Ray { f3 o, d; float tmax; bool shadow; };
+    struct Ray { f3 o, d; float tmax; bool shadow, occl; };
     std::vector<Ray> rays;
     std::vector<int> stack(std::max(F.depth + 1, 1));
     for (int pix = 0; pix < frame * frame; ++pix) {
         PathState<float> P;
         path_begin<kMatsAll>(P, S, pix % frame, pix / frame, frame, frame, seed, (uint32_t)pix, 0u);
         for (;;) {
-            rays.push_back(Ray{P.ro, P.rd, P.rtmax, P.shadow});
-            const Hit<float> h = trace<FRT_WORLD_BVH, 1>(S, P.ro, P.rd, P.rtmax, P.shadow, stack.data());
+            rays.push_back(Ray{P.ro, P.rd, P.rtmax, P.shadow, light_shadow_ray(P)});
+            const Hit<float> h = trace<FRT_WORLD_BVH, 1>(S, P.ro, P.rd, P.rtmax, P.shadow, stack.data(), light_shadow_ray(P));
             uint32_t n_ext = 0, n_sh = 0;
             if (path_shade<kMatsAll>(P, S, h, kRefineMaxDepth, n_ext, n_sh)) break;
         }
@@ -330,6 +332,8 @@
     }
     R.n_prims = (int)R.prim_ref.size();
     R.tmin.resize(n); R.tmax.resize(n); R.anyhit.resize(n); R.live.resize(n);
+    if (occl) occl->assign(n, 0);
+    if (origins) origins->clear();
     R.slab.resize((size_t)nl * n * 6);
     R.prim_t.resize((size_t)n * R.n_prims);
     int stride = (int)(0.618 * n) | 1;
@@ -342,6 +346,8 @@
         R.tmin[i] = T.tmin;
         R.tmax[i] = q.tmax;
         R.anyhit[i] = q.shadow ? 1 : 0;
+        if (occl) (*occl)[i] = q.occl ? 1 : 0;
+        if (origins && q.occl) { origins->push_back(q.o.x); origins->push_back(q.o.y); origins->push_back(q.o.z); }
         const float inv[3] = {T.sr.invd.x, T.sr.invd.y, T.sr.invd.z}, oi[3] = {T.sr.oinv.x, T.sr.oinv.y, T.sr.oinv.z};
         for (int l = 0; l < nl; ++l) {
             float *s = &R.slab[((size_t)i * nl + l) * 6];
@@ -428,7 +434,178 @@
     return true;
 }
 
-int flatten_scene(const frt_scene_view *sv, FlatScene &F, std::string &err, bool f64, int refine)
+static bool shadow_tree_knob()
+{
+    const char *e = std::getenv("FRT_SHADOW_TREE");
+    return !(e && std::atoi(e) == 0);
+}
+
+static void shadow_tree(const frt_scene_view *sv, FlatScene &F)
+{
+    auto &I = F.shadow;
+    DevScene &S = F.meta;
+    I.nodes_main = (int)(F.nodes.size() / 4);
+    if (sv->n_lights <= 0) { I.why = FlatScene::kShadowNoLights; return; }
+    for (int i = 0; i < sv->n_materials; ++i)
+        if (sv->materials[i].type != FRT_MAT_LAMBERTIAN && sv->materials[i].type != FRT_MAT_DIFFUSE_LIGHT) {
+            I.why = FlatScene::kShadowMaterial;
+            return;
+        }
+    if (!tree_in_lds(F) || F.nodes.empty()) { I.why = FlatScene::kShadowNotResident; return; }
+    const int nt = sv->n_tris;
+    std::vector<double> tv(9 * (size_t)nt), tn;
+    std::vector<uint8_t> smooth(nt, 0);
+    bool any_smooth = false;
+    for (int d = 0; d < nt; ++d) {
+        const int i = F.tri_view[d];
+        std::copy(&sv->tri_v[9 * (size_t)i], &sv->tri_v[9 * (size_t)i] + 9, &tv[9 * (size_t)d]);
+        smooth[d] = sv->tri_geometry_normal && !sv->tri_geometry_normal[i];
+        any_smooth |= smooth[d] != 0;
+    }
+    if (any_smooth) {
+        tn.resize(9 * (size_t)nt);
+        for (int d = 0; d < nt; ++d) std::copy(&sv->tri_n[9 * (size_t)F.tri_view[d]], &sv->tri_n[9 * (size_t)F.tri_view[d]] + 9, &tn[9 * (size_t)d]);
+    }
+    frt_shadow::Geometry g;
+    g.n_tris = nt; g.n_spheres = sv->n_spheres;
+    g.tri_v = tv.data(); g.tri_n = any_smooth ? tn.data() : nullptr; g.tri_smooth = smooth.data();
+    g.sphere = sv->sphere;
+    g.lights = F.lights.data(); g.n_lights = (int)F.lights.size(); g.sphere_bit = FRT_PRIM_SPHERE;
+    for (int k = 0; k < 3; ++k) { g.cam_o[k] = sv->cam_origin[k]; g.cam_u[k] = sv->cam_u[k]; g.cam_v[k] = sv->cam_v[k]; }
+    g.lens_r = sv->cam_lens_radius;
+    g.eps = (double)Cst<float>::eps;
+    frt_shadow::Classified c;
+    frt_shadow::classify(g, c);
+    if (c.why != frt_shadow::kRan) {
+        I.why = c.why == frt_shadow::kNoLights ? FlatScene::kShadowNoLights : FlatScene::kShadowTooLarge;
+        return;
+    }
+    int n_dropped = 0;
+    for (int d = 0; d < nt; ++d) n_dropped += c.dropped[d];
+    if (n_dropped == 0) { I.why = FlatScene::kShadowNothing; return; }
+    std::vector<float> nodes(4 * F.nodes.size());
+    memcpy(nodes.data(), F.nodes.data(), sizeof(float4) * F.nodes.size());
+    frt_shadow::Tree t;
+    frt_shadow::build(nodes, S.root, c.dropped, FRT_PRIM_SPHERE, kLeafCountShift, t);
+    if (t.dropped_leaves == 0) { I.why = FlatScene::kShadowNothing; return; }
+    const size_t rest = F.tris.size() + F.tshade.size() + F.mats.size();
+    const int nn0 = I.nodes_main, nn1 = (int)(nodes.size() / 16);
+    const bool lds0 = sizeof(float4) * (4 * (size_t)nn0 + rest) <= kLdsSceneBytes;
+    const bool lds1 = sizeof(float4) * (4 * (size_t)nn1 + rest) <= kLdsSceneBytes;
+    const bool oct0 = !F.nodes_oct.empty();
+    const bool oct1 = sizeof(float4) * (oct_lds_node_slots(nn1) + rest) <= kLdsOctBytes;
+    if (lds0 != lds1 || oct0 != oct1) { I.why = FlatScene::kShadowBudget; return; }
+    F.nodes.resize((size_t)4 * nn1);
+    memcpy(F.nodes.data(), nodes.data(), sizeof(float) * nodes.size());
+    if (oct0) F.nodes_oct.resize(8 * F.nodes.size());
+    S.sroot = t.empty ? kSentinel : t.root;
+    I.why = FlatScene::kShadowRan;
+    I.dropped = c.dropped;
+    I.n_dropped = n_dropped; I.rule_a = c.n_rule_a; I.rule_b = c.n_rule_b;
+    I.added = t.added; I.shared = t.shared; I.empty = t.empty;
+}
+
+static void topology_all(const std::vector<float4> &nodes, frt_refine::Topology &t, std::vector<RefineLeaf> &leaves,
+                         std::vector<int> &leaf_refs)
+{
+    const int nn = (int)(nodes.size() / 4);
+    leaves.clear();
+    leaf_refs.clear();
+    for (int i = 0; i < nn; ++i)
+        for (int side = 0; side < 2; ++side) {
+            const float4 *n = &nodes[4 * i];
+            const int c = f2i(side ? n[3].y : n[3].x);
+            if (c >= 0 || std::find(leaf_refs.begin(), leaf_refs.end(), c) != leaf_refs.end()) continue;
+            const float b[2][6] = {{n[0].x, n[0].y, n[0].z, n[0].w, n[1].x, n[1].y}, {n[1].z, n[1].w, n[2].x, n[2].y, n[2].z, n[2].w}};
+            RefineLeaf l;
+            for (int k = 0; k < 6; ++k) l.box[k] = b[side][k];
+            l.ref = c;
+            leaves.push_back(l);
+            leaf_refs.push_back(c);
+        }
+    t.n_leaves = (int)leaves.size();
+    t.root = t.n_leaves;
+    t.child.assign(2 * (size_t)nn, 0);
+    for (int i = 0; i < nn; ++i)
+        for (int side = 0; side < 2; ++side) {
+            const int c = f2i(side ? nodes[4 * i + 3].y : nodes[4 * i + 3].x);
+            t.child[2 * i + side] = c >= 0 ? t.n_leaves + c
+                                           : (int)(std::find(leaf_refs.begin(), leaf_refs.end(), c) - leaf_refs.begin());
+        }
+}
+
+bool shadow_cost_host(const FlatScene &F, ShadowCost &out)
+{
+    out = ShadowCost{};
+    if (F.shadow.why != FlatScene::kShadowRan) return false;
+    frt_refine::Topology t;
+    std::vector<RefineLeaf> leaves;
+    std::vector<int> leaf_refs;
+    topology_all(F.nodes, t, leaves, leaf_refs);
+    frt_refine::RaySet R;
+    std::vector<uint8_t> occl;
+    sample_rays(F, leaves, kRefineValFrame, kRefineValSeed, R, &occl);
+    const DevScene S = host_scene(F);
+    int n_occl = 0;
+    for (int i = 0; i < R.n; ++i) n_occl += occl[i];
+    out.n_rays = n_occl;
+    if (n_occl == 0) return true;
+    auto price = [&](int which) {
+        const frt_refine::Cost c = frt_refine::tree_cost(t, R);
+        out.V[which] = c.V * R.n / n_occl;
+        out.T[which] = c.T * R.n / n_occl;
+    };
+    for (int i = 0; i < R.n; ++i) {
+        R.live[i] = R.live[i] && occl[i];
+        if (occl[i] && !R.live[i]) ++out.stops[0];
+    }
+    price(0);
+    if (F.shadow.empty) {
+        out.stops[1] = n_occl;
+        return true;
+    }
+    const int sroot = S.sroot >= 0 ? t.n_leaves + S.sroot
+                                   : (int)(std::find(leaf_refs.begin(), leaf_refs.end(), S.sroot) - leaf_refs.begin());
+    std::vector<int> under, st{sroot};
+    while (!st.empty()) {
+        const int s = st.back();
+        st.pop_back();
+        if (s < t.n_leaves) { under.push_back(s); continue; }
+        st.push_back(t.child[2 * (s - t.n_leaves)]);
+        st.push_back(t.child[2 * (s - t.n_leaves) + 1]);
+    }
+    auto misses_box = [&](int i) {
+        float u[6];
+        for (int k = 0; k < 6; ++k) u[k] = __builtin_inff();
+        for (int l : under)
+            for (int k = 0; k < 6; ++k) u[k] = std::min(u[k], R.slab[((size_t)i * R.n_leaves + l) * 6 + k]);
+        const float tn = std::max(std::max(u[0], u[1]), std::max(u[2], Cst<float>::eps));
+        const float tf = std::min(std::min(-u[3], -u[4]), std::min(-u[5], R.tmax[i]));
+        return !(tn <= tf);
+    };
+    R.root.assign(R.n, sroot);
+    for (int i = 0; i < R.n; ++i) {
+        R.live[i] = occl[i];
+        if (occl[i] && misses_box(i)) ++out.stops[1];
+    }
+    price(1);
+    return true;
+}
+
+void shadow_origins_host(const FlatScene &F, std::vector<float> &origins)
+{
+    origins.clear();
+    if (F.meta.world_kind != FRT_WORLD_BVH || F.nodes.empty()) return;
+    frt_refine::Topology t;
+    std::vector<RefineLeaf> leaves;
+    std::vector<int> leaf_refs;
+    topology_all(F.nodes, t, leaves, leaf_refs);
+    frt_refine::RaySet R;
+    std::vector<uint8_t> occl;
+    sample_rays(F, leaves, kRefineValFrame, kRefineValSeed, R, &occl, &origins);
+}
+
+int flatten_scene(const frt_scene_view *sv, FlatScene &F, std::string &err, bool f64, int refine, int shadow)
 {
     auto fail = [&](int code, const std::string &m) { err = m; return code; };
     const int nt = sv->n_tris, ns = sv->n_spheres, nm = sv->n_materials;
@@ -680,6 +857,7 @@
     if (sv->world_kind == FRT_WORLD_BVH && F.depth < kLdsMaxDepth && oct_bytes <= kLdsOctBytes)
         F.nodes_oct.resize(8 * F.nodes.size());
     S.root = (sv->world_kind == FRT_WORLD_BVH) ? ((sv->root >= 0) ? 0 : ~dev_ref(~sv->root)) : 0;
+    S.sroot = S.root;
     auto derive_trees = [&]() {
         fill_octants(F);
         F.has4 = sv->world_kind == FRT_WORLD_BVH && build_bvh4(F, S.root);
@@ -712,7 +890,13 @@
     S.cam64_h = d3d(sv->cam_horizontal); S.cam64_v = d3d(sv->cam_vertical);
     S.cam64_u = d3d(sv->cam_u); S.cam64_vv = d3d(sv->cam_v);
     S.lens_r64 = sv->cam_lens_radius;
-    if ((refine < 0 ? tree_refine_knob() : refine != 0) && refine_tree(F)) derive_trees();
+    bool again = (refine < 0 ? tree_refine_knob() : refine != 0) && refine_tree(F);
+    if (shadow < 0 ? shadow_tree_knob() : shadow != 0) {
+        shadow_tree(sv, F);
+        again |= F.shadow.why == FlatScene::kShadowRan;
+    }
+    if (again) derive_trees();
+    S.n_nodes = (int)(F.nodes.size() / 4);
     return FRT_OK;
 }
 
diff --git a/first_raytracer_amd/csrc/frt_flatten.hpp b/first_raytracer_amd/csrc/frt_flatten.hpp
--- a/first_raytracer_amd/csrc/frt_flatten.hpp
+++ b/first_raytracer_amd/csrc/frt_flatten.hpp
@@ -21,9 +21,20 @@
     std::vector<int> tri_view;
     DevScene meta{};
     int depth = 0;
+    enum { kShadowRan = 0, kShadowOff, kShadowNoLights, kShadowTooLarge, kShadowMaterial, kShadowNotResident,
+           kShadowNothing, kShadowBudget };
+    struct {
+        int why = kShadowOff;
+        std::vector<uint8_t> dropped;
+        int n_dropped = 0, rule_a = 0, rule_b = 0, nodes_main = 0, added = 0, shared = 0;
+        bool empty = false;
+    } shadow;
 };
 
-int flatten_scene(const frt_scene_view *sv, FlatScene &F, std::string &err, bool f64, int refine = -1);
+int flatten_scene(const frt_scene_view *sv, FlatScene &F, std::string &err, bool f64, int refine = -1, int shadow = -1);
+struct ShadowCost { double V[2] = {0, 0}, T[2] = {0, 0}; int n_rays = 0, stops[2] = {0, 0}; };
+bool shadow_cost_host(const FlatScene &F, ShadowCost &out);
+void shadow_origins_host(const FlatScene &F, std::vector<float> &origins);
 struct TreeCost { double V = 0.0, T = 0.0, J = 0.0, w = 0.0; int depth = 0, n_rays = 0; };
 bool tree_cost_host(const FlatScene &F, TreeCost &out);
 int env_texels_of(const frt_image *img, std::vector<float4> &out, std::string &err);
diff --git a/first_raytracer_amd/csrc/frt_kernels.hpp b/first_raytracer_amd/csrc/frt_kernels.hpp
--- a/first_raytracer_amd/csrc/frt_kernels.hpp
+++ b/first_raytracer_amd/csrc/frt_kernels.hpp
@@ -252,7 +252,9 @@
         n_cam += started;
         n_smp += started;
         if (next_ray) {
-            tracing = trav_begin_world<WORLD>(T, S, P.ro, P.rd, ray_tmax());
+            const R tm = ray_tmax();
+            const bool occl = KIND == FRT_INTEGRATOR_PATH && P.shadow && ((MATS & kMatsEnvNee) == 0 || tm < R(1));
+            tracing = trav_begin_world<WORLD>(T, S, P.ro, P.rd, tm, occl);
             pending = !tracing;
         }
         diag_t0 = FRT_DIAG_CLOCK();
@@ -372,7 +374,7 @@
 template <int WORLD, int STACK>
 __device__ __forceinline__ Hit<float> trace_any(const DevScene &S, const PathState<float> &P, int *stk)
 {
-    return trace<WORLD, kBlock, STACK>(S, P.ro, P.rd, P.rtmax, P.shadow, stk);
+    return trace<WORLD, kBlock, STACK>(S, P.ro, P.rd, P.rtmax, P.shadow, stk, P.shadow);
 }
 
 template <int STACK, int WORLD, bool MATS, bool ENV = false>
@@ -458,7 +460,7 @@
                         pending = true;
                     } else {
                         ext = true;
-                        tracing = trav_begin_world<WORLD>(T, S, M.P.ro, M.P.rd, M.P.rtmax);
+                        tracing = trav_begin_world<WORLD>(T, S, M.P.ro, M.P.rd, M.P.rtmax, M.P.shadow);
                         pending = !tracing;
                     }
                 } else {
@@ -599,7 +601,7 @@
                 beyond = true;
                 pending = true;
             } else {
-                tracing = trav_begin_world<WORLD>(T, S, M.P.ro, M.P.rd, M.P.rtmax);
+                tracing = trav_begin_world<WORLD>(T, S, M.P.ro, M.P.rd, M.P.rtmax, M.P.shadow);
                 pending = !tracing;
             }
         }
diff --git a/first_raytracer_amd/csrc/frt_path.hpp b/first_raytracer_amd/csrc/frt_path.hpp
--- a/first_raytracer_amd/csrc/frt_path.hpp
+++ b/first_raytracer_amd/csrc/frt_path.hpp
@@ -93,6 +93,7 @@
     int node_es, node_ps, tri_es, tri_ps, sh_es, sh_ps, node4_es, node4_ps;
     int n_nodes4;
     float root_lo[3], root_hi[3];
+    int sroot;
     float ao_tmax;
     int ao_spheres_only;
     f3 cam_o, cam_llc, cam_h, cam_v, cam_u, cam_vv, cam_w;
@@ -225,15 +226,17 @@
     return Cst<R>::eps * vmax(R(1), vmax(vabs(o.x), vmax(vabs(o.y), vabs(o.z))));
 }
 
-template <typename R> FRT_HD bool trav_begin(Trav<R> &T, const DevScene &S, int root, V3<R> o, V3<R> d, R tmax)
+template <typename R>
+FRT_HD bool trav_begin(Trav<R> &T, const DevScene &S, int root, V3<R> o, V3<R> d, R tmax, bool occl = false)
 {
     T.h = Hit<R>{-1, tmax, R(0), R(0)};
     T.sp = 0;
-    T.node = root;
+    T.node = occl ? S.sroot : root;
     T.sr = slab_ray(o, d);
     T.tmin = bvh_tmin(o);
-    return slab_entry<R>(S.root_lo[0], S.root_lo[1], S.root_lo[2], S.root_hi[0], S.root_hi[1], S.root_hi[2], T.sr,
-                         Cst<R>::eps, tmax) != R(__builtin_inff());
+    const bool in = slab_entry<R>(S.root_lo[0], S.root_lo[1], S.root_lo[2], S.root_hi[0], S.root_hi[1], S.root_hi[2], T.sr,
+                                  Cst<R>::eps, tmax) != R(__builtin_inff());
+    return occl || in;
 }
 
 template <int STRIDE, bool OCT = false, int STEP = kStepBranch, typename R>
@@ -390,10 +393,10 @@
 }
 
 template <int STRIDE, typename R>
-FRT_HD Hit<R> trace_bvh(const DevScene &S, V3<R> o, V3<R> d, R tmax, bool anyhit, int *stk)
+FRT_HD Hit<R> trace_bvh(const DevScene &S, V3<R> o, V3<R> d, R tmax, bool anyhit, int *stk, bool occl = false)
 {
     Trav<R> T;
-    if (trav_begin(T, S, S.root, o, d, tmax))
+    if (trav_begin(T, S, S.root, o, d, tmax, occl))
         while (!bvh2_step<STRIDE>(T, S, o, d, anyhit, stk)) {}
     return T.h;
 }
@@ -457,21 +460,23 @@
 }
 
 template <int WORLD, int STRIDE, int STACK = 0, typename R>
-FRT_HD Hit<R> trace(const DevScene &S, V3<R> o, V3<R> d, R tmax, bool anyhit, int *stk)
+FRT_HD Hit<R> trace(const DevScene &S, V3<R> o, V3<R> d, R tmax, bool anyhit, int *stk, bool occl = false)
 {
     if constexpr (WORLD == FRT_WORLD_LIST) return trace_list(S, o, d, tmax, anyhit);
     else if constexpr (WORLD == kWorldBvh4) return trace_bvh4<STRIDE, STACK, kBvh4Overflow>(S, o, d, tmax, anyhit, stk);
-    else return trace_bvh<STRIDE>(S, o, d, tmax, anyhit, stk);
+    else return trace_bvh<STRIDE>(S, o, d, tmax, anyhit, stk, occl);
 }
 
 template <int WORLD, typename R>
-FRT_HD bool trav_begin_world(Trav<R> &T, const DevScene &S, V3<R> o, V3<R> d, R tmax)
+FRT_HD bool trav_begin_world(Trav<R> &T, const DevScene &S, V3<R> o, V3<R> d, R tmax, bool occl = false)
 {
     if constexpr (WORLD == FRT_WORLD_LIST) {
         T.h = Hit<R>{-1, tmax, R(0), R(0)};
         return true;
+    } else if constexpr (WORLD == kWorldBvh4) {
+        return trav_begin(T, S, S.root4, o, d, tmax);
     } else {
-        return trav_begin(T, S, WORLD == kWorldBvh4 ? S.root4 : S.root, o, d, tmax);
+        return trav_begin(T, S, S.root, o, d, tmax, occl);
     }
 }
 template <int WORLD, int STRIDE, int STACK, int STEP = kStepBranch, typename R>
@@ -777,6 +782,8 @@
     P.prev_p = zero3<R>();
     P.prev_spec = false;
 }
+
+template <typename R> FRT_HD bool light_shadow_ray(const PathState<R> &P) { return P.shadow && P.rtmax < R(1); }
 
 template <int MATS = kMatsAll, typename R>
 FRT_HD bool path_after_shadow(PathState<R> &P, bool unoccluded)
diff --git a/first_raytracer_amd/csrc/frt_selftest.hip b/first_raytracer_amd/csrc/frt_selftest.hip
--- a/first_raytracer_amd/csrc/frt_selftest.hip
+++ b/first_raytracer_amd/csrc/frt_selftest.hip
@@ -26,13 +26,14 @@
             ++cnt[0];
             for (;;) {
                 Hit<R> h;
+                const bool occl = p->integrator != FRT_INTEGRATOR_AO && light_shadow_ray(P);
                 if (S.world_kind == FRT_WORLD_LIST) {
                     h = trace<FRT_WORLD_LIST, 1>(S, P.ro, P.rd, P.rtmax, P.shadow, stack.data());
                 } else if constexpr (!kIsF64<R>) {
                     h = wide ? trace<kWorldBvh4, 1, kSelftestStack>(S, P.ro, P.rd, P.rtmax, P.shadow, stack.data())
-                             : trace<FRT_WORLD_BVH, 1>(S, P.ro, P.rd, P.rtmax, P.shadow, stack.data());
+                             : trace<FRT_WORLD_BVH, 1>(S, P.ro, P.rd, P.rtmax, P.shadow, stack.data(), occl);
                 } else {
-                    h = trace<FRT_WORLD_BVH, 1>(S, P.ro, P.rd, P.rtmax, P.shadow, stack.data());
+                    h = trace<FRT_WORLD_BVH, 1>(S, P.ro, P.rd, P.rtmax, P.shadow, stack.data(), occl);
                 }
                 n_ext = n_sh = 0;
                 const bool done = p->integrator == FRT_INTEGRATOR_AO ? ao_shade<MATS>(P, S, h, n_sh)
@@ -150,7 +151,7 @@
             if (mlt_beyond(M)) { M.P.L = M.P.L + M.P.beta * env_of<float>(S); break; }
             const Hit<float> h = (S.world_kind == FRT_WORLD_LIST)
                               ? trace<FRT_WORLD_LIST, 1>(S, M.P.ro, M.P.rd, M.P.rtmax, M.P.shadow, stack.data())
-                              : trace<FRT_WORLD_BVH, 1>(S, M.P.ro, M.P.rd, M.P.rtmax, M.P.shadow, stack.data());
+                              : trace<FRT_WORLD_BVH, 1>(S, M.P.ro, M.P.rd, M.P.rtmax, M.P.shadow, stack.data(), M.P.shadow);
             if (mlt_shade(M, S, h, src, ne, ns)) break;
         }
         const f3 L = M.P.L;
@@ -168,7 +169,7 @@
     for (int on = 0; on < 2; ++on) {
         FlatScene F;
         std::string err;
-        const int rc = flatten_scene(sv, F, err, false, on);
+        const int rc = flatten_scene(sv, F, err, false, on, 0);
         if (rc != FRT_OK) return rc;
         TreeCost c;
         const bool applies = tree_cost_host(F, c);
@@ -177,6 +178,62 @@
         if (dst[on]) {
             if (nn > max_nodes) return FRT_E_INVALID;
             memcpy(dst[on], F.nodes.data(), F.nodes.size() * sizeof(float4));
+        }
+    }
+    return FRT_OK;
+}
+
+extern "C" int frtx_selftest_shadow_tree(const frt_scene_view *sv, frt_shadow_tree_info *out, uint8_t *dropped,
+                                         float *nodes, int32_t max_nodes, int64_t segments, uint32_t seed)
+{
+    if (!sv || !out || segments < 0) return FRT_E_INVALID;
+    FlatScene F;
+    std::string err;
+    const int rc = flatten_scene(sv, F, err, false, -1, 1);
+    if (rc != FRT_OK) return rc;
+    const auto &I = F.shadow;
+    memset(out, 0, sizeof(*out));
+    out->why = I.why;
+    out->n_nodes = (int)(F.nodes.size() / 4);
+    out->nodes_main = I.nodes_main;
+    out->root = F.meta.sroot;
+    if (nodes) {
+        if (out->n_nodes > max_nodes) return FRT_E_INVALID;
+        memcpy(nodes, F.nodes.data(), F.nodes.size() * sizeof(float4));
+    }
+    if (dropped) memset(dropped, 0, (size_t)std::max(sv->n_tris, 0));
+    if (I.why != FlatScene::kShadowRan) return FRT_OK;
+    out->dropped_prims = I.n_dropped;
+    out->kept_prims = sv->n_tris + sv->n_spheres - I.n_dropped;
+    out->rule_a = I.rule_a; out->rule_b = I.rule_b;
+    out->nodes_added = I.added; out->nodes_shared = I.shared; out->empty = I.empty ? 1 : 0;
+    if (dropped)
+        for (int d = 0; d < sv->n_tris; ++d) dropped[F.tri_view[d]] = I.dropped[d];
+    ShadowCost c;
+    shadow_cost_host(F, c);
+    out->n_rays = c.n_rays;
+    out->v_main = c.V[0]; out->t_main = c.T[0]; out->v_shadow = c.V[1]; out->t_shadow = c.T[1];
+    out->root_stops_main = c.stops[0]; out->root_stops_shadow = c.stops[1];
+    if (segments > 0) {
+        std::vector<float> org;
+        shadow_origins_host(F, org);
+        const DevScene S = host_scene(F);
+        const int64_t no = (int64_t)(org.size() / 3);
+        for (int64_t i = 0; i < segments && no > 0 && S.n_lights > 0; ++i) {
+            const RngKey key = rng_key(seed, (uint32_t)i, (uint32_t)(i >> 32));
+            const float *q = &org[3 * (size_t)(i % no)];
+            const f3 o = mk3(q[0], q[1], q[2]);
+            int idx = (int)(rng_u(key, 0) * (float)S.n_lights);
+            if (idx == S.n_lights) idx -= 1;
+            f3 ln;
+            int lmat;
+            const f3 d = prim_sample(S, S.lights[idx], o, rng_u(key, 1), rng_u(key, 2), ln, lmat);
+            ++out->segments;
+            for (int t = 0; t < S.n_tris; ++t) {
+                if (!I.dropped[t]) continue;
+                float u, v;
+                if (prim_t(S, t, o, d, bvh_tmin(o), 1.0f - Cst<float>::shadow_eps, u, v) > 0.0f) ++out->segment_hits;
+            }
         }
     }
     return FRT_OK;
diff --git a/first_raytracer_amd/csrc/host/shadow_tree.cpp b/first_raytracer_amd/csrc/host/shadow_tree.cpp
--- /dev/null
+++ b/first_raytracer_amd/csrc/host/shadow_tree.cpp
@@ -0,0 +1,176 @@
+#include "shadow_tree.hpp"
+
+#include <algorithm>
+#include <cmath>
+
+namespace frt_shadow {
+namespace {
+
+constexpr double kU = 1.0 / 16777216.0;
+constexpr double kNoise = 32.0, kOnPlane = 8.0, kMaxAspect = 8.0;
+
+struct V { double x, y, z; };
+inline V sub(V a, V b) { return V{a.x - b.x, a.y - b.y, a.z - b.z}; }
+inline double dot(V a, V b) { return a.x * b.x + a.y * b.y + a.z * b.z; }
+inline V cross(V a, V b) { return V{a.y * b.z - a.z * b.y, a.z * b.x - a.x * b.z, a.x * b.y - a.y * b.x}; }
+inline double len(V a) { return std::sqrt(dot(a, a)); }
+inline V at(const double *p) { return V{p[0], p[1], p[2]}; }
+
+}
+
+void classify(const Geometry &g, Classified &out)
+{
+    out = Classified{};
+    out.dropped.assign((size_t)std::max(g.n_tris, 0), 0);
+    if (g.n_lights <= 0) { out.why = kNoLights; return; }
+    double lo[3] = {1e300, 1e300, 1e300}, hi[3] = {-1e300, -1e300, -1e300};
+    auto grow = [&](const double *p, double r) {
+        for (int k = 0; k < 3; ++k) { lo[k] = std::min(lo[k], p[k] - r); hi[k] = std::max(hi[k], p[k] + r); }
+    };
+    for (int i = 0; i < 3 * g.n_tris; ++i) grow(&g.tri_v[3 * i], 0.0);
+    for (int i = 0; i < g.n_spheres; ++i) grow(&g.sphere[4 * i], g.sphere[4 * i + 3]);
+    grow(g.cam_o, std::fabs(g.lens_r));
+    double M = 0.0, Dm = 0.0;
+    for (int k = 0; k < 3; ++k) {
+        M = std::max(M, std::max(std::fabs(lo[k]), std::fabs(hi[k])));
+        Dm += (hi[k] - lo[k]) * (hi[k] - lo[k]);
+    }
+    Dm = std::sqrt(Dm);
+    if (!(kNoise * kU * Dm <= 0.25 * g.eps) || !(M < 1e30)) { out.why = kTooLarge; return; }
+    const double tol = kOnPlane * kU * M;
+    const double lens = std::fabs(g.lens_r);
+
+    std::vector<V> ng((size_t)g.n_tris);
+    std::vector<uint8_t> flat((size_t)g.n_tris, 0);
+    for (int i = 0; i < g.n_tris; ++i) {
+        const double *v = &g.tri_v[9 * i];
+        const V c = cross(sub(at(v + 3), at(v)), sub(at(v + 6), at(v)));
+        const double l = len(c);
+        if (l > 0.0) ng[i] = V{c.x / l, c.y / l, c.z / l};
+        else { ng[i] = V{0, 0, 0}; flat[i] = 1; }
+    }
+    auto smooth = [&](int i) { return g.tri_smooth && g.tri_smooth[i]; };
+    auto light_is_sphere = [&](int ref) { return (ref & g.sphere_bit) != 0; };
+
+    for (int p = 0; p < g.n_tris; ++p) {
+        if (flat[p]) continue;
+        const double *pv = &g.tri_v[9 * p];
+        const V v0 = at(pv), e1 = sub(at(pv + 3), v0), e2 = sub(at(pv + 6), v0), m = ng[p];
+        const double rho = len(e1) * len(e2) / len(cross(e1, e2));
+        if (!(rho <= kMaxAspect)) continue;
+        const double E = kNoise * kU * rho * Dm, D = 4.0 * E / g.eps;
+        auto s = [&](const double *x) { return dot(m, sub(at(x), v0)); };
+
+        bool rule_b = false;
+        for (int k = 0; k < 3 && !rule_b; ++k) {
+            const double c = pv[k];
+            bool ok = pv[3 + k] == c && pv[6 + k] == c;
+            for (int l = 0; l < g.n_lights && ok; ++l) {
+                const int ref = g.lights[l];
+                if (light_is_sphere(ref)) { ok = false; break; }
+                const double *lv = &g.tri_v[9 * ref];
+                ok = lv[k] == c && lv[3 + k] == c && lv[6 + k] == c;
+            }
+            rule_b = ok;
+        }
+        if (rule_b) { out.dropped[p] = 1; ++out.n_rule_b; continue; }
+
+        for (int side = 1; side >= -1 && !out.dropped[p]; side -= 2) {
+            const double sg = (double)side;
+            bool ok = true;
+            for (int i = 0; i < 3 * g.n_tris && ok; ++i) ok = sg * s(&g.tri_v[3 * i]) >= -tol;
+            for (int i = 0; i < g.n_spheres && ok; ++i) ok = sg * s(&g.sphere[4 * i]) - g.sphere[4 * i + 3] >= -tol;
+            if (ok) {
+                const double a = dot(m, at(g.cam_u)), b = dot(m, at(g.cam_v));
+                ok = sg * s(g.cam_o) - lens * std::sqrt(a * a + b * b) >= -tol;
+            }
+            for (int q = 0; q < g.n_tris && ok; ++q) {
+                const double *qv = &g.tri_v[9 * q];
+                bool leans;
+                if (smooth(q)) {
+                    leans = false;
+                    for (int j = 0; j < 3; ++j) leans |= !(sg * dot(m, at(&g.tri_n[9 * q + 3 * j])) >= 0.0);
+                } else {
+                    leans = flat[q] || !(-sg * dot(m, ng[q]) * g.eps <= E);
+                }
+                if (leans) ok = std::min(std::min(sg * s(qv), sg * s(qv + 3)), sg * s(qv + 6)) >= 2.0 * g.eps;
+            }
+            for (int i = 0; i < g.n_spheres && ok; ++i)
+                ok = sg * s(&g.sphere[4 * i]) - g.sphere[4 * i + 3] >= 2.0 * g.eps;
+            for (int l = 0; l < g.n_lights && ok; ++l) {
+                const int ref = g.lights[l];
+                if (light_is_sphere(ref)) {
+                    const double *q = &g.sphere[4 * (ref & ~g.sphere_bit)];
+                    ok = sg * s(q) - q[3] >= D;
+                } else {
+                    const double *lv = &g.tri_v[9 * ref];
+                    ok = std::min(std::min(sg * s(lv), sg * s(lv + 3)), sg * s(lv + 6)) >= D;
+                }
+            }
+            if (ok) { out.dropped[p] = 1; ++out.n_rule_a; }
+        }
+    }
+}
+
+void build(std::vector<float> &nodes, int main_root, const std::vector<uint8_t> &dropped, int sphere_bit,
+           int count_shift, Tree &out)
+{
+    out = Tree{};
+    auto ref_of = [&](int i, int side) {
+        int r;
+        const float f = nodes[16 * (size_t)i + 12 + side];
+        static_assert(sizeof(r) == sizeof(f), "refs are stored as int bits");
+        std::copy(reinterpret_cast<const char *>(&f), reinterpret_cast<const char *>(&f) + sizeof(f), reinterpret_cast<char *>(&r));
+        return r;
+    };
+    auto leaf_kept = [&](int lref) {
+        if (lref & sphere_bit) return true;
+        const int first = lref & ((1 << count_shift) - 1), count = (lref >> count_shift) + 1;
+        for (int k = 0; k < count; ++k)
+            if (first + k >= (int)dropped.size() || !dropped[first + k]) return true;
+        return false;
+    };
+    struct Sub { bool empty, same; int ref; float box[6]; int n_nodes; };
+    struct Rec {
+        std::vector<float> &nodes;
+        decltype(ref_of) &ref;
+        decltype(leaf_kept) &kept;
+        Tree &out;
+        Sub visit(int r, const float *box)
+        {
+            Sub s{};
+            for (int k = 0; k < 6; ++k) s.box[k] = box[k];
+            s.ref = r;
+            if (r < 0) {
+                s.same = true;
+                s.empty = !kept(~r);
+                ++(s.empty ? out.dropped_leaves : out.kept_leaves);
+                return s;
+            }
+            float b0[6], b1[6];
+            for (int k = 0; k < 6; ++k) { b0[k] = nodes[16 * (size_t)r + k]; b1[k] = nodes[16 * (size_t)r + 6 + k]; }
+            const Sub a = visit(ref(r, 0), b0), b = visit(ref(r, 1), b1);
+            if (a.empty && b.empty) { s.empty = true; return s; }
+            if (a.empty || b.empty) { Sub c = a.empty ? b : a; c.same = false; return c; }
+            if (a.same && b.same) { s.same = true; s.n_nodes = 1 + a.n_nodes + b.n_nodes; return s; }
+            out.shared += a.n_nodes + b.n_nodes;
+            s.ref = (int)(nodes.size() / 16);
+            float rec[16] = {0};
+            for (int k = 0; k < 6; ++k) { rec[k] = a.box[k]; rec[6 + k] = b.box[k]; }
+            const int refs[2] = {a.ref, b.ref};
+            std::copy(reinterpret_cast<const char *>(refs), reinterpret_cast<const char *>(refs) + sizeof(refs),
+                      reinterpret_cast<char *>(&rec[12]));
+            nodes.insert(nodes.end(), rec, rec + 16);
+            ++out.added;
+            for (int k = 0; k < 3; ++k) { s.box[k] = std::min(a.box[k], b.box[k]); s.box[3 + k] = std::max(a.box[3 + k], b.box[3 + k]); }
+            return s;
+        }
+    } rec{nodes, ref_of, leaf_kept, out};
+    const float no_box[6] = {0, 0, 0, 0, 0, 0};
+    const Sub r = rec.visit(main_root, no_box);
+    out.shared += r.n_nodes;
+    out.empty = r.empty;
+    out.root = r.empty ? main_root : r.ref;
+}
+
+}
diff --git a/first_raytracer_amd/csrc/host/shadow_tree.hpp b/first_raytracer_amd/csrc/host/shadow_tree.hpp
--- /dev/null
+++ b/first_raytracer_amd/csrc/host/shadow_tree.hpp
@@ -0,0 +1,36 @@
+#pragma once
+#include <cstdint>
+#include <vector>
+
+namespace frt_shadow {
+
+struct Geometry {
+    int n_tris = 0, n_spheres = 0;
+    const double *tri_v = nullptr;
+    const double *tri_n = nullptr;
+    const uint8_t *tri_smooth = nullptr;
+    const double *sphere = nullptr;
+    const int *lights = nullptr;
+    int n_lights = 0, sphere_bit = 0;
+    double cam_o[3] = {0, 0, 0}, cam_u[3] = {0, 0, 0}, cam_v[3] = {0, 0, 0}, lens_r = 0.0;
+    double eps = 0.0;
+};
+
+enum Why { kRan = 0, kNoLights, kTooLarge };
+struct Classified {
+    int why = kRan;
+    std::vector<uint8_t> dropped;
+    int n_rule_a = 0, n_rule_b = 0;
+};
+void classify(const Geometry &g, Classified &out);
+
+struct Tree {
+    int root = 0;
+    bool empty = false;
+    int added = 0, shared = 0;
+    int kept_leaves = 0, dropped_leaves = 0;
+};
+void build(std::vector<float> &nodes, int main_root, const std::vector<uint8_t> &dropped, int sphere_bit,
+           int count_shift, Tree &out);
+
+}
diff --git a/first_raytracer_amd/csrc/host/tree_refine.cpp b/first_raytracer_amd/csrc/host/tree_refine.cpp
--- a/first_raytracer_amd/csrc/host/tree_refine.cpp
+++ b/first_raytracer_amd/csrc/host/tree_refine.cpp
@@ -3,6 +3,8 @@
 #include <algorithm>
 #include <cstddef>
 #include <cstring>
+#include <utility>
+#include <vector>
 
 #include "frt.h"
 
@@ -41,7 +43,7 @@
         const bool any = R.anyhit[r] != 0;
         const float *pt = &R.prim_t[(size_t)r * R.n_prims];
         float tb_ = R.tmax[r];
-        int hp = -1, sp = 0, node = t.root;
+        int hp = -1, sp = 0, node = R.root.empty() ? t.root : R.root[r];
         int stk[kMaxLevels];
         for (;;) {
             while (node >= L) {
@@ -86,22 +88,31 @@
 
 void build_tables(const Topology &t, const RaySet &R, Tables &tb)
 {
-    const int L = t.n_leaves, nI = std::max(L - 1, 0);
+    const int L = t.n_leaves, nI = (int)(t.child.size() / 2);
     tb.n_slots = L + nI;
     tb.tab.resize((size_t)R.n * tb.n_slots * 6);
-    std::vector<int> order, st{t.root};
+    std::vector<int> order, roots{t.root};
+    roots.insert(roots.end(), R.root.begin(), R.root.end());
+    std::sort(roots.begin(), roots.end());
+    roots.erase(std::unique(roots.begin(), roots.end()), roots.end());
+    std::vector<char> seen(tb.n_slots, 0);
+    std::vector<std::pair<int, bool>> st;
+    for (int root : roots) st.push_back({root, false});
     while (!st.empty()) {
-        const int s = st.back();
+        const auto [s, done] = st.back();
         st.pop_back();
         if (s < L) continue;
-        order.push_back(s);
-        st.push_back(t.child[2 * (s - L)]);
-        st.push_back(t.child[2 * (s - L) + 1]);
+        if (done) { order.push_back(s); continue; }
+        if (seen[s]) continue;
+        seen[s] = 1;
+        st.push_back({s, true});
+        st.push_back({t.child[2 * (s - L)], false});
+        st.push_back({t.child[2 * (s - L) + 1], false});
     }
     for (int r = 0; r < R.n; ++r) {
         float *base = &tb.tab[(size_t)r * tb.n_slots * 6];
         memcpy(base, &R.slab[(size_t)r * L * 6], sizeof(float) * 6 * L);
-        for (size_t k = order.size(); k-- > 0;) {
+        for (size_t k = 0; k < order.size(); ++k) {
             const int s = order[k], j = s - L;
             unite(base + 6 * t.child[2 * j], base + 6 * t.child[2 * j + 1], base + 6 * s);
         }
diff --git a/first_raytracer_amd/csrc/host/tree_refine.hpp b/first_raytracer_amd/csrc/host/tree_refine.hpp
--- a/first_raytracer_amd/csrc/host/tree_refine.hpp
+++ b/first_raytracer_amd/csrc/host/tree_refine.hpp
@@ -12,6 +12,7 @@
     std::vector<int> prim_first;
     std::vector<int> prim_ref;
     std::vector<float> prim_t;
+    std::vector<int> root;
 };
 
 struct Topology {
diff --git a/include/frt.h b/include/frt.h
--- a/include/frt.h
+++ b/include/frt.h
@@ -221,6 +221,15 @@
 } frt_tree_cost;
 int frtx_selftest_tree_refine(const frt_scene_view *scene, frt_tree_cost out[2], float *nodes_off, float *nodes_on,
                              int32_t max_nodes);
+typedef struct frt_shadow_tree_info {
+    int32_t why, kept_prims, dropped_prims, rule_a, rule_b;
+    int32_t nodes_main, nodes_added, nodes_shared, root, empty;
+    int32_t n_rays, root_stops_main, root_stops_shadow, n_nodes;
+    double v_main, t_main, v_shadow, t_shadow;
+    int64_t segments, segment_hits;
+} frt_shadow_tree_info;
+int frtx_selftest_shadow_tree(const frt_scene_view *scene, frt_shadow_tree_info *out, uint8_t *dropped, float *nodes,
+                              int32_t max_nodes, int64_t segments, uint32_t seed);
 int frtx_selftest_trace_host(const frt_scene_view *scene, const float *rays, int64_t n, float *hits);
 int frtx_selftest_chunk_variance(const float *partial, int n_chunks, int64_t n_slots, int spp, int spi, float *out);
 typedef struct frt_plan_query {
```
